# lightec-xyz/bls-verify-gadget

Measured on NVIDIA B200. Metric: bls12_381_verifies_per_sec, higher is better.
Workload: dtype u32 limbs (381-bit modular integer)

## Files before the change

bls_verify_gadget_b200/csrc/blsgpu.cu:

```cuda
#include <cuda_runtime.h>
#include <cstdio>
#include <cstring>
#include <cstdarg>
#include <new>
#include <vector>
#include "stages.cuh"
#include "coop.cuh"
#include "../../include/blsgpu.h"

using namespace bls;

#ifndef BLS_TPB
#define BLS_TPB 128
#endif
#define TPB BLS_TPB
#define VERIFY_CHUNK_DEFAULT ((size_t)1 << 20)
#ifndef VERIFY_COOP_BELOW
#define VERIFY_COOP_BELOW 4096
#endif
#ifndef BLS_MINB
#define BLS_MINB 2
#endif
static inline unsigned nblk(size_t n, unsigned tpb = TPB) { return (unsigned)((n + tpb - 1) / tpb); }

#ifndef BLS_MINB_DG1
#define BLS_MINB_DG1 4
#endif
#ifndef BLS_MINB_DG2
#define BLS_MINB_DG2 4
#endif
#ifndef BLS_MINB_HASH
#define BLS_MINB_HASH BLS_MINB
#endif
#ifndef BLS_MINB_SQR
#define BLS_MINB_SQR 3
#endif
#ifndef BLS_MINB_HFIELD
#define BLS_MINB_HFIELD 4
#endif
#ifndef BLS_MINB_HMAP
#define BLS_MINB_HMAP 3
#endif
#ifndef BLS_MINB_LINES
#define BLS_MINB_LINES BLS_MINB
#endif
#ifndef BLS_MINB_HCLEAR
#define BLS_MINB_HCLEAR BLS_MINB
#endif
#ifndef BLS_MINB_ACCUM
#define BLS_MINB_ACCUM BLS_MINB
#endif
#ifndef MILLER_LINE_ITERS
#define MILLER_LINE_ITERS 8
#define MILLER_LINE_STEPS 11
#endif

#ifndef BLS_F_IN_SMEM
#define BLS_F_IN_SMEM 0
#endif
#ifndef BLS_SKEW
#define BLS_SKEW 0
#endif
__device__ __forceinline__ void phase_skew() {
#if BLS_SKEW > 0
    if ((threadIdx.x >> 5) & 4) { long long t0 = clock64(); while (clock64() - t0 < BLS_SKEW) { } }
#endif
}
__global__ void __launch_bounds__(TPB, BLS_MINB) k_fp_mul_raw(const fp* a, const fp* b, fp* out, size_t n, int reps) {
    size_t i = blockIdx.x * (size_t)blockDim.x + threadIdx.x; if (i >= n) return;
    fp x = a[i], y = b[i];
    fp r = fp_mul(x, y);
    for (int k = 1; k < reps; k++) r = fp_mul(r, y);
    out[i] = r;
}
__global__ void __launch_bounds__(256) k_imad_peak(uint32_t* sink, int iters, int mode) {
    uint32_t a = threadIdx.x * 2654435761u + 12345u, b = blockIdx.x * 40503u + 977u;
    if (mode == 0) {
        unsigned long long acc[16];
#pragma unroll
        for (int j = 0; j < 16; j++) acc[j] = (unsigned long long)j * 0x9e3779b97f4a7c15ull + a;
        for (int it = 0; it < iters; it++) {
#pragma unroll
            for (int j = 0; j < 16; j++)
                asm volatile("mad.wide.u32 %0, %1, %2, %0;" : "+l"(acc[j]) : "r"((uint32_t)acc[(j + 5) & 15]), "r"(b));
        }
        unsigned long long s = 0;
#pragma unroll
        for (int j = 0; j < 16; j++) s ^= acc[j];
        if (s == 0x1234567ull) sink[0] = (uint32_t)s;
    } else {
        uint32_t e[16], o[16];
#pragma unroll
        for (int j = 0; j < 16; j++) { e[j] = a + j; o[j] = b + j; }
        for (int it = 0; it < iters; it++) {
            asm volatile(
                "mad.lo.cc.u32 %0, %16, %24, %0;\n\tmadc.hi.cc.u32 %1, %16, %24, %1;\n\tmadc.lo.cc.u32 %2, %17, %24, %2;\n\tmadc.hi.cc.u32 %3, %17, %24, %3;\n\t"
                "madc.lo.cc.u32 %4, %18, %24, %4;\n\tmadc.hi.cc.u32 %5, %18, %24, %5;\n\tmadc.lo.cc.u32 %6, %19, %24, %6;\n\tmadc.hi.cc.u32 %7, %19, %24, %7;\n\t"
                "madc.lo.cc.u32 %8, %20, %24, %8;\n\tmadc.hi.cc.u32 %9, %20, %24, %9;\n\tmadc.lo.cc.u32 %10, %21, %24, %10;\n\tmadc.hi.cc.u32 %11, %21, %24, %11;\n\t"
                "madc.lo.cc.u32 %12, %22, %24, %12;\n\tmadc.hi.cc.u32 %13, %22, %24, %13;\n\tmadc.lo.cc.u32 %14, %23, %24, %14;\n\tmadc.hi.u32 %15, %23, %24, %15;"
                : "+r"(e[0]), "+r"(e[1]), "+r"(e[2]), "+r"(e[3]), "+r"(e[4]), "+r"(e[5]), "+r"(e[6]), "+r"(e[7]), "+r"(e[8]), "+r"(e[9]), "+r"(e[10]), "+r"(e[11]), "+r"(e[12]), "+r"(e[13]), "+r"(e[14]), "+r"(e[15])
                : "r"(a), "r"(a + 1), "r"(a + 2), "r"(a + 3), "r"(a + 4), "r"(a + 5), "r"(a + 6), "r"(a + 7), "r"(o[3]));
            asm volatile(
                "mad.lo.cc.u32 %0, %16, %24, %0;\n\tmadc.hi.cc.u32 %1, %16, %24, %1;\n\tmadc.lo.cc.u32 %2, %17, %24, %2;\n\tmadc.hi.cc.u32 %3, %17, %24, %3;\n\t"
                "madc.lo.cc.u32 %4, %18, %24, %4;\n\tmadc.hi.cc.u32 %5, %18, %24, %5;\n\tmadc.lo.cc.u32 %6, %19, %24, %6;\n\tmadc.hi.cc.u32 %7, %19, %24, %7;\n\t"
                "madc.lo.cc.u32 %8, %20, %24, %8;\n\tmadc.hi.cc.u32 %9, %20, %24, %9;\n\tmadc.lo.cc.u32 %10, %21, %24, %10;\n\tmadc.hi.cc.u32 %11, %21, %24, %11;\n\t"
                "madc.lo.cc.u32 %12, %22, %24, %12;\n\tmadc.hi.cc.u32 %13, %22, %24, %13;\n\tmadc.lo.cc.u32 %14, %23, %24, %14;\n\tmadc.hi.u32 %15, %23, %24, %15;"
                : "+r"(o[0]), "+r"(o[1]), "+r"(o[2]), "+r"(o[3]), "+r"(o[4]), "+r"(o[5]), "+r"(o[6]), "+r"(o[7]), "+r"(o[8]), "+r"(o[9]), "+r"(o[10]), "+r"(o[11]), "+r"(o[12]), "+r"(o[13]), "+r"(o[14]), "+r"(o[15])
                : "r"(b), "r"(b + 1), "r"(b + 2), "r"(b + 3), "r"(b + 4), "r"(b + 5), "r"(b + 6), "r"(b + 7), "r"(e[5]));
        }
        uint32_t s = 0;
#pragma unroll
        for (int j = 0; j < 16; j++) s ^= e[j] ^ o[j];
        if (s == 0x12345u) sink[0] = s;
    }
}

__global__ void __launch_bounds__(TPB, BLS_MINB_DG1) k_decode_g1(const uint8_t* in48, size_t n, u32x4* soa, uint8_t* code) {
    phase_skew();
    size_t i = blockIdx.x * (size_t)blockDim.x + threadIdx.x; if (i >= n) return;
    g1_aff p; int rc = g1_decode(p, in48 + 48 * i);
    if (soa) soa_store_g1(soa, n, i, p);
    code[i] = (uint8_t)rc;
}
__global__ void __launch_bounds__(TPB, BLS_MINB_DG2) k_decode_g2(const uint8_t* in96, size_t n, u32x4* soa, uint8_t* code) {
    phase_skew();
    size_t i = blockIdx.x * (size_t)blockDim.x + threadIdx.x; if (i >= n) return;
    g2_aff p; int rc = g2_decode(p, in96 + 96 * i);
    if (soa) soa_store_g2(soa, n, i, p);
    code[i] = (uint8_t)rc;
}
__global__ void __launch_bounds__(TPB, BLS_MINB_HASH) k_hash_to_g2(const uint8_t* msg, const uint32_t* off, size_t n, const uint8_t* code_pk, const uint8_t* code_sig,
                                                    u32x4* hm_soa, uint8_t* flags, uint8_t* status) {
    phase_skew();
    size_t i = blockIdx.x * (size_t)blockDim.x + threadIdx.x; if (i >= n) return;
    uint8_t st = ST_OK, fl = 0;
    if (code_pk) {
        if (code_pk[i] != DEC_OK) st = ST_BAD_PK;
        else if (code_sig[i] != DEC_OK && code_sig[i] != DEC_INF) st = ST_BAD_SIG;
        else if (code_sig[i] == DEC_INF) fl = FL_SIG_INF;
    }
    if (st == ST_OK) {
        const uint8_t* m; uint32_t len;
        if (off) { m = msg + off[i]; len = off[i + 1] - off[i]; } else { m = msg + 32 * i; len = 32; }
        g2_aff hm; uint8_t f2; stage_hash(hm, f2, m, len);
        soa_store_g2(hm_soa, n, i, hm); fl |= f2;
    }
    flags[i] = fl; if (status) status[i] = st;
}
__global__ void __launch_bounds__(TPB, BLS_MINB_HFIELD) k_hash_field(const uint8_t* msg, const uint32_t* off, size_t n, const uint8_t* code_pk, const uint8_t* code_sig,
                                                               u32x4* u_soa, uint8_t* flags, uint8_t* status) {
    size_t i = blockIdx.x * (size_t)blockDim.x + threadIdx.x; if (i >= n) return;
    uint8_t st = ST_OK, fl = 0;
    if (code_pk) {
        if (code_pk[i] != DEC_OK) st = ST_BAD_PK;
        else if (code_sig[i] != DEC_OK && code_sig[i] != DEC_INF) st = ST_BAD_SIG;
        else if (code_sig[i] == DEC_INF) fl = FL_SIG_INF;
    }
    if (st == ST_OK) {
        const uint8_t* m; uint32_t len;
        if (off) { m = msg + off[i]; len = off[i + 1] - off[i]; } else { m = msg + 32 * i; len = 32; }
        fp2 u0, u1; hash_to_field(u0, u1, m, len);
        soa_store_fp2(u_soa, n, i, 0, u0); soa_store_fp2(u_soa, n, i, 1, u1);
    }
    flags[i] = fl; if (status) status[i] = st;
}
__global__ void k_status_merge(const uint8_t* code_pk, const uint8_t* code_sig, size_t n, uint8_t* flags, uint8_t* status) {
    size_t i = blockIdx.x * (size_t)blockDim.x + threadIdx.x; if (i >= n) return;
    uint8_t st = ST_OK, fl = 0;
    if (code_pk[i] != DEC_OK) st = ST_BAD_PK;
    else if (code_sig[i] != DEC_OK && code_sig[i] != DEC_INF) st = ST_BAD_SIG;
    else if (code_sig[i] == DEC_INF) fl = FL_SIG_INF;
    flags[i] = (uint8_t)((flags[i] & FL_HM_INF) | fl); status[i] = st;
}
__global__ void __launch_bounds__(TPB, BLS_MINB_HMAP) k_hash_map(const u32x4* u_soa, const uint8_t* status, size_t n, u32x4* q_soa) {
    size_t t = blockIdx.x * (size_t)blockDim.x + threadIdx.x; if (t >= 2 * n) return;
    int j = t >= n; size_t i = t - (j ? n : 0);
    if (status && status[i] != ST_OK) return;
    fp2 u = soa_load_fp2(u_soa, n, i, j), xn, xd, y; g2_jac q;
    sswu_map(xn, xd, y, u); iso3_map(q, xn, xd, y);
    soa_store_fp2(q_soa, n, i, 3 * j, q.X); soa_store_fp2(q_soa, n, i, 3 * j + 1, q.Y); soa_store_fp2(q_soa, n, i, 3 * j + 2, q.Z);
}
__global__ void __launch_bounds__(TPB, BLS_MINB_HCLEAR) k_hash_clear(const u32x4* q_soa, const uint8_t* status, size_t n, u32x4* hm_soa, uint8_t* flags) {
    size_t i = blockIdx.x * (size_t)blockDim.x + threadIdx.x; if (i >= n) return;
    if (status && status[i] != ST_OK) return;
    g2_jac q0, q1, h; g2_aff hm;
    q0.X = soa_load_fp2(q_soa, n, i, 0); q0.Y = soa_load_fp2(q_soa, n, i, 1); q0.Z = soa_load_fp2(q_soa, n, i, 2);
    q1.X = soa_load_fp2(q_soa, n, i, 3); q1.Y = soa_load_fp2(q_soa, n, i, 4); q1.Z = soa_load_fp2(q_soa, n, i, 5);
    jac_add(q0, q0, q1); g2_clear_cofactor(h, q0);
    if (!jac_to_aff(hm, h)) flags[i] |= FL_HM_INF;
    soa_store_g2(hm_soa, n, i, hm);
}
__global__ void __launch_bounds__(TPB, BLS_MINB) k_miller(const u32x4* pk_soa, const u32x4* hm_soa, const u32x4* sig_soa, const uint8_t* flags,
                                                const uint8_t* status, size_t n, u32x4* f_soa) {
    phase_skew();
    size_t i = blockIdx.x * (size_t)blockDim.x + threadIdx.x; if (i >= n) return;
    if (status[i] != ST_OK) return;
    g1_aff pk; g2_aff hm, sig;
    soa_load_g1(pk, pk_soa, n, i); soa_load_g2(hm, hm_soa, n, i); soa_load_g2(sig, sig_soa, n, i);
#if BLS_F_IN_SMEM
    extern __shared__ uint4 f_smem[];
    fp12& f = *reinterpret_cast<fp12*>(f_smem + threadIdx.x * 37);
#else
    fp12 f;
#endif
    stage_miller(f, pk, hm, sig, flags[i]);
    soa_store_fp12(f_soa, n, i, f);
}
__global__ void __launch_bounds__(TPB, BLS_MINB_LINES) k_miller_lines(const u32x4* pk_soa, const u32x4* hm_soa, const u32x4* sig_soa, const uint8_t* flags, const uint8_t* status,
                                                                size_t n, u32x4* t_soa, u32x4* lines, int i_hi, int i_lo) {
    size_t t = blockIdx.x * (size_t)blockDim.x + threadIdx.x; if (t >= 2 * n) return;
    int j = t >= n; size_t i = t - (j ? n : 0);
    if (status[i] != ST_OK) return;
    if (flags[i] & (j ? FL_HM_INF : FL_SIG_INF)) return;
    g1_aff p; g2_aff q; g2_proj r;
    if (j) { soa_load_g1(p, pk_soa, n, i); soa_load_g2(q, hm_soa, n, i); } else { p.x = fp_const(C_G1X); p.y = fp_const(C_G1Y_NEG); soa_load_g2(q, sig_soa, n, i); }
    if (i_hi == 62) { r.x = q.x; r.y = q.y; r.z = fp2_one(); }
    else { r.x = soa_load_fp2(t_soa, n, i, 3 * j); r.y = soa_load_fp2(t_soa, n, i, 3 * j + 1); r.z = soa_load_fp2(t_soa, n, i, 3 * j + 2); }
    const uint64_t x = BLS_X_ABS; int s = 0; fp2 c0, c1, c2;
    for (int it = i_hi; it >= i_lo; it--) {
        miller_dbl(r, c0, c1, c2);
        { u32x4* L = lines + (size_t)(2 * s + j) * 18 * n; soa_store_fp2(L, n, i, 0, c0); soa_store_fp2(L, n, i, 1, fp2_mul_fp(c1, p.x)); soa_store_fp2(L, n, i, 2, fp2_mul_fp(c2, p.y)); s++; }
        if ((x >> it) & 1) {
            miller_add(r, q, c0, c1, c2);
            u32x4* L = lines + (size_t)(2 * s + j) * 18 * n; soa_store_fp2(L, n, i, 0, c0); soa_store_fp2(L, n, i, 1, fp2_mul_fp(c1, p.x)); soa_store_fp2(L, n, i, 2, fp2_mul_fp(c2, p.y)); s++;
        }
    }
    if (i_lo != 0) { soa_store_fp2(t_soa, n, i, 3 * j, r.x); soa_store_fp2(t_soa, n, i, 3 * j + 1, r.y); soa_store_fp2(t_soa, n, i, 3 * j + 2, r.z); }
}
__global__ void __launch_bounds__(TPB, BLS_MINB_ACCUM) k_miller_accum(const uint8_t* flags, const uint8_t* status, size_t n, u32x4* f_soa, const u32x4* lines, int i_hi, int i_lo) {
    size_t i = blockIdx.x * (size_t)blockDim.x + threadIdx.x; if (i >= n) return;
    if (status[i] != ST_OK) return;
    uint8_t fl = flags[i]; bool use0 = !(fl & FL_SIG_INF), use1 = !(fl & FL_HM_INF);
    fp12 f; if (i_hi == 62) fp12_one(f); else soa_load_fp12(f, f_soa, n, i);
    const uint64_t x = BLS_X_ABS; int s = 0;
    for (int it = i_hi; it >= i_lo; it--) {
        if (it != 62) fp12_sqr(f, f);
        int steps = 1 + (int)((x >> it) & 1);
        for (int a = 0; a < steps; a++, s++) {
            if (use0) { const u32x4* L = lines + (size_t)(2 * s) * 18 * n; fp12_mul_by_014(f, soa_load_fp2(L, n, i, 0), soa_load_fp2(L, n, i, 1), soa_load_fp2(L, n, i, 2)); }
            if (use1) { const u32x4* L = lines + (size_t)(2 * s + 1) * 18 * n; fp12_mul_by_014(f, soa_load_fp2(L, n, i, 0), soa_load_fp2(L, n, i, 1), soa_load_fp2(L, n, i, 2)); }
        }
    }
    if (i_lo == 0) fp12_conj(f, f);
    soa_store_fp12(f_soa, n, i, f);
}
__global__ void __launch_bounds__(TPB, BLS_MINB_SQR) k_final_squarings(const u32x4* in_soa, u32x4* snap_soa, const uint8_t* status, size_t n) {
    size_t i = blockIdx.x * (size_t)blockDim.x + threadIdx.x; if (i >= n) return;
    if (status[i] != ST_OK) return;
    fp12c c;
    c.g2 = soa_load_fp2(in_soa, n, i, 3); c.g3 = soa_load_fp2(in_soa, n, i, 2); c.g4 = soa_load_fp2(in_soa, n, i, 1); c.g5 = soa_load_fp2(in_soa, n, i, 5);
    const uint64_t x = BLS_X_ABS; int k = 0;
    for (int j = 1; j <= 63; j++) {
        fp12c_sqr(c, c);
        if ((x >> j) & 1) {
            soa_store_fp2(snap_soa, n, i, 4 * k, c.g2); soa_store_fp2(snap_soa, n, i, 4 * k + 1, c.g3); soa_store_fp2(snap_soa, n, i, 4 * k + 2, c.g4); soa_store_fp2(snap_soa, n, i, 4 * k + 3, c.g5);
            k++;
        }
    }
}
template <int STEP> __global__ void __launch_bounds__(TPB, BLS_MINB) k_final_step(u32x4* f_soa, u32x4* y1_soa, u32x4* y2_soa, const u32x4* snap_soa, const uint8_t* status_in, uint8_t* status_out, size_t n) {
    size_t i = blockIdx.x * (size_t)blockDim.x + threadIdx.x; if (i >= n) return;
    if (status_in[i] != ST_OK) { if (STEP == 5) status_out[i] = status_in[i]; return; }
    fp12 r, y1, y2, e;
    if (STEP >= 1) {
        fp12_decompress_product_from(e, [&](int k) { fp12c c; c.g2 = soa_load_fp2(snap_soa, n, i, 4 * k); c.g3 = soa_load_fp2(snap_soa, n, i, 4 * k + 1);
                                                     c.g4 = soa_load_fp2(snap_soa, n, i, 4 * k + 2); c.g5 = soa_load_fp2(snap_soa, n, i, 4 * k + 3); return c; }, 6);
        fp12_conj(e, e);
    }
    if (STEP == 0 || STEP == 1 || STEP == 3 || STEP == 5) soa_load_fp12(r, f_soa, n, i);
    if (STEP == 2 || STEP == 3 || STEP == 5) soa_load_fp12(y1, y1_soa, n, i);
    final_exponentiation_step<STEP>(r, y1, y2, e);
    if (STEP == 0 || STEP == 3 || STEP == 5) soa_store_fp12(f_soa, n, i, r);
    if (STEP >= 1 && STEP <= 3) soa_store_fp12(y1_soa, n, i, y1);
    if (STEP == 4) soa_store_fp12(y2_soa, n, i, y2);
    if (STEP == 5) status_out[i] = fp12_is_one(r) ? ST_OK : ST_FALSE;
}
__global__ void __launch_bounds__(TPB, BLS_MINB) k_miller_pairs(const u32x4* g1_soa, const u32x4* g2_soa, const uint8_t* c1, const uint8_t* c2, size_t npairs, size_t nprod,
                                                      u32x4* f_soa, uint8_t* status) {
    size_t i = blockIdx.x * (size_t)blockDim.x + threadIdx.x; if (i >= nprod) return;
    size_t tot = npairs * nprod;
    g1_aff p[2]; g2_aff q[2]; bool use[2] = {false, false}; uint8_t st = ST_OK;
    for (size_t k = 0; k < npairs; k++) {
        size_t j = i * npairs + k;
        soa_load_g1(p[k], g1_soa, tot, j); soa_load_g2(q[k], g2_soa, tot, j);
        if (c1[j] > DEC_INF) st = ST_BAD_PK; else if (c2[j] > DEC_INF && st == ST_OK) st = ST_BAD_SIG;
        use[k] = c1[j] == DEC_OK && c2[j] == DEC_OK;
    }
    if (npairs < 2) { p[1] = p[0]; q[1] = q[0]; }
    status[i] = st;
    if (st != ST_OK) return;
    fp12 f; miller_loop2(f, p[0], q[0], use[0], p[1], q[1], use[1]);
    soa_store_fp12(f_soa, nprod, i, f);
}
__global__ void __launch_bounds__(TPB, BLS_MINB) k_final_exp(u32x4* f_soa, const uint8_t* status_in, uint8_t* status_out, size_t n) {
    phase_skew();
    size_t i = blockIdx.x * (size_t)blockDim.x + threadIdx.x; if (i >= n) return;
    if (status_in[i] != ST_OK) { status_out[i] = status_in[i]; return; }
    fp12 f, gt; soa_load_fp12(f, f_soa, n, i);
    status_out[i] = stage_final(gt, f);
    soa_store_fp12(f_soa, n, i, gt);
}
__global__ void __launch_bounds__(TPB, BLS_MINB) k_final_easy(u32x4* f_soa, const uint8_t* status, size_t n) {
    size_t i = blockIdx.x * (size_t)blockDim.x + threadIdx.x; if (i >= n) return;
    if (status[i] != ST_OK) return;
    fp12 f, t, r; soa_load_fp12(f, f_soa, n, i);
    fp12_conj(t, f); fp12_inv(r, f); fp12_mul(r, t, r);
    fp12_frob2(t, r); fp12_mul(r, t, r);
    soa_store_fp12(f_soa, n, i, r);
}
__global__ void __launch_bounds__(128, 2) k_final_hard_coop(u32x4* f_soa, const uint8_t* status_in, uint8_t* status_out, size_t n) {
    __shared__ coop_smem sm[4];
    int warp = threadIdx.x >> 5, lane = threadIdx.x & 31, g = lane / 6;
    coop_lane c = coop_init(&sm[warp]);
    size_t item = (blockIdx.x * (size_t)4 + warp) * 5 + g;
    bool in_range = g < 5 && item < n;
    uint8_t st = in_range ? status_in[item] : (uint8_t)ST_BAD_PK;
    bool active = in_range && st == ST_OK;
    fp2 r = c.k == 0 ? fp2_one() : fp2_zero();
    if (active) r = soa_load_fp2(f_soa, n, item, COOP_TOWER_POS[c.k]);
    r = coop_final_exp_hard(c, r);
    bool mine = c.k == 0 ? fp2_eq(r, fp2_one()) : fp2_is_zero(r);
    unsigned ball = __ballot_sync(0xffffffffu, mine);
    if (active) soa_store_fp2(f_soa, n, item, COOP_TOWER_POS[c.k], r);
    if (in_range && c.k == 0) status_out[item] = active ? ((((ball >> (6 * g)) & 63u) == 63u) ? (uint8_t)ST_OK : (uint8_t)ST_FALSE) : st;
}
__global__ void __launch_bounds__(128, 2) k_miller_accum_coop(const uint8_t* flags, const uint8_t* status, size_t n, u32x4* f_soa, const u32x4* lines, int i_hi, int i_lo) {
    __shared__ coop_smem sm[4];
    int warp = threadIdx.x >> 5, lane = threadIdx.x & 31, g = lane / 6;
    coop_lane c = coop_init(&sm[warp]);
    size_t item = (blockIdx.x * (size_t)4 + warp) * 5 + g;
    bool active = g < 5 && item < n && status[item] == ST_OK;
    uint8_t fl = active ? flags[item] : (uint8_t)(FL_SIG_INF | FL_HM_INF);
    bool use[2] = {!(fl & FL_SIG_INF), !(fl & FL_HM_INF)};
    fp2 unit = c.k == 0 ? fp2_one() : fp2_zero();
    fp2 f = (active && i_hi != 62) ? soa_load_fp2(f_soa, n, item, COOP_TOWER_POS[c.k]) : unit;
    int slot = c.k == 0 ? 0 : c.k == 2 ? 1 : c.k == 3 ? 2 : -1;
    const uint64_t x = BLS_X_ABS; int s = 0;
    for (int it = i_hi; it >= i_lo; it--) {
        if (it != 62) f = coop_mul(c, f, f);
        int steps = 1 + (int)((x >> it) & 1);
        for (int a = 0; a < steps; a++, s++)
            for (int j = 0; j < 2; j++) {
                const u32x4* L = lines + (size_t)(2 * s + j) * 18 * n;
                fp2 b = !use[j] ? unit : slot >= 0 ? soa_load_fp2(L, n, item, slot) : fp2_zero();
                f = coop_mul(c, f, b);
            }
    }
    if (i_lo == 0) f = coop_conj(c, f);
    if (active) soa_store_fp2(f_soa, n, item, COOP_TOWER_POS[c.k], f);
}
__global__ void __launch_bounds__(TPB, BLS_MINB) k_gt_reduce(const u32x4* in_soa, const uint8_t* status, size_t n, u32x4* out_soa, size_t T) {
    size_t t = blockIdx.x * (size_t)blockDim.x + threadIdx.x; if (t >= T) return;
    fp12 acc, x; fp12_one(acc);
    for (size_t i = t; i < n; i += T) {
        if (status && status[i] > ST_FALSE) continue;
        soa_load_fp12(x, in_soa, n, i); fp12_mul(acc, acc, x);
    }
    soa_store_fp12(out_soa, T, t, acc);
}
__global__ void k_gt_mul_into(u32x4* acc_soa, const u32x4* x_soa) {
    if (threadIdx.x || blockIdx.x) return;
    fp12 a, x; soa_load_fp12(a, acc_soa, 1, 0); soa_load_fp12(x, x_soa, 1, 0); fp12_mul(a, a, x); soa_store_fp12(acc_soa, 1, 0, a);
}
__global__ void k_gt_set_one(u32x4* acc_soa) { if (threadIdx.x || blockIdx.x) return; fp12 a; fp12_one(a); soa_store_fp12(acc_soa, 1, 0, a); }
__global__ void __launch_bounds__(TPB, BLS_MINB) k_gt_to_bytes(const u32x4* soa, size_t n, uint8_t* out576, const uint8_t* status) {
    size_t i = blockIdx.x * (size_t)blockDim.x + threadIdx.x; if (i >= n) return;
    if (status && status[i] != ST_OK) { for (int k = 0; k < 576; k++) out576[576 * i + k] = 0; return; }
    fp12 a; soa_load_fp12(a, soa, n, i); fp12_to_bytes(out576 + 576 * i, a);
}
__global__ void __launch_bounds__(TPB, BLS_MINB) k_gt_from_bytes(const uint8_t* in576, size_t n, u32x4* soa) {
    size_t i = blockIdx.x * (size_t)blockDim.x + threadIdx.x; if (i >= n) return;
    fp12 a; fp2* c[6] = {&a.c0.c0, &a.c0.c1, &a.c0.c2, &a.c1.c0, &a.c1.c1, &a.c1.c2};
    const uint8_t* b = in576 + 576 * i;
    for (int k = 0; k < 12; k++) {
        fp v;
        for (int w = 0; w < 12; w++) { const uint8_t* q = b + 48 * k + 4 * w; v.l[w] = q[0] | ((uint32_t)q[1] << 8) | ((uint32_t)q[2] << 16) | ((uint32_t)q[3] << 24); }
        v = fp_to_mont(v);
        if (k & 1) c[k >> 1]->c1 = v; else c[k >> 1]->c0 = v;
    }
    soa_store_fp12(soa, n, i, a);
}
__global__ void k_status_bitmap(const uint8_t* status, size_t n, uint32_t* bitmap32) {
    size_t i = blockIdx.x * (size_t)blockDim.x + threadIdx.x;
    bool ok = i < n && status[i] == ST_OK;
    unsigned m = __ballot_sync(0xffffffffu, ok);
    if ((threadIdx.x & 31) == 0 && i < ((n + 31) / 32) * 32) bitmap32[i >> 5] = m;
}
__global__ void __launch_bounds__(TPB, BLS_MINB) k_encode_g1(const u32x4* soa, const uint8_t* inf, size_t n, uint8_t* out48) {
    size_t i = blockIdx.x * (size_t)blockDim.x + threadIdx.x; if (i >= n) return;
    g1_aff p; soa_load_g1(p, soa, n, i); g1_encode(out48 + 48 * i, p, inf && inf[i]);
}
__global__ void __launch_bounds__(TPB, BLS_MINB) k_encode_g2(const u32x4* soa, const uint8_t* flags, uint8_t mask, size_t n, uint8_t* out96) {
    size_t i = blockIdx.x * (size_t)blockDim.x + threadIdx.x; if (i >= n) return;
    g2_aff p; soa_load_g2(p, soa, n, i); g2_encode(out96 + 96 * i, p, flags && (flags[i] & mask));
}
__device__ __forceinline__ bool load_scalar(uint32_t* k, const uint8_t* sk) {
    const uint32_t R[8] = BLS_C_R_ORDER;
    for (int w = 0; w < 8; w++) k[w] = sk[4 * w] | ((uint32_t)sk[4 * w + 1] << 8) | ((uint32_t)sk[4 * w + 2] << 16) | ((uint32_t)sk[4 * w + 3] << 24);
    for (int w = 7; w >= 0; w--) { if (k[w] != R[w]) return k[w] < R[w]; }
    return false;
}
__global__ void __launch_bounds__(TPB, BLS_MINB) k_scalar_mul_g1(const uint8_t* sk32, size_t n, uint8_t* pk48, uint8_t* status) {
    size_t i = blockIdx.x * (size_t)blockDim.x + threadIdx.x; if (i >= n) return;
    uint32_t k[8]; bool canon = load_scalar(k, sk32 + 32 * i);
    if (status) status[i] = canon ? ST_OK : ST_BAD_SK;
    g1_aff g; g.x = fp_const(C_G1X); g.y = fp_const(C_G1Y);
    g1_jac r; jac_mul_scalar(r, g, k);
    g1_aff a; bool ok = jac_to_aff(a, r); g1_encode(pk48 + 48 * i, a, !ok || !canon);
}
__global__ void __launch_bounds__(TPB, BLS_MINB) k_scalar_mul_g2(const uint8_t* sk32, const u32x4* hm_soa, const uint8_t* flags, size_t n, uint8_t* sig96, uint8_t* status) {
    size_t i = blockIdx.x * (size_t)blockDim.x + threadIdx.x; if (i >= n) return;
    uint32_t k[8]; bool canon = load_scalar(k, sk32 + 32 * i);
    uint32_t nz = 0; for (int w = 0; w < 8; w++) nz |= k[w];
    if (!canon || !nz) { status[i] = ST_BAD_SK; for (int b = 0; b < 96; b++) sig96[96 * i + b] = 0; return; }
    status[i] = ST_OK;
    g2_aff hm; soa_load_g2(hm, hm_soa, n, i);
    g2_jac r;
    if (flags[i] & FL_HM_INF) jac_set_identity(r); else jac_mul_scalar(r, hm, k);
    g2_aff a; bool ok = jac_to_aff(a, r); g2_encode(sig96 + 96 * i, a, !ok);
}

template <class F> struct segsum_traits;
template <> struct segsum_traits<fp>  { enum { K = 2 }; static __device__ __forceinline__ void load(aff<fp>& p, const u32x4* s, size_t n, size_t i) { soa_load_g1(p, s, n, i); }
                                        static __device__ __forceinline__ void store(u32x4* s, size_t n, size_t i, const aff<fp>& p) { soa_store_g1(s, n, i, p); }
                                        static __device__ __forceinline__ void storej(u32x4* s, size_t n, size_t i, const jac<fp>& p) { soa_store_fp(s, n, i, 0, p.X); soa_store_fp(s, n, i, 1, p.Y); soa_store_fp(s, n, i, 2, p.Z); }
                                        static __device__ __forceinline__ void loadj(jac<fp>& p, const u32x4* s, size_t n, size_t i) { p.X = soa_load_fp(s, n, i, 0); p.Y = soa_load_fp(s, n, i, 1); p.Z = soa_load_fp(s, n, i, 2); } };
template <> struct segsum_traits<fp2> { enum { K = 4 }; static __device__ __forceinline__ void load(aff<fp2>& p, const u32x4* s, size_t n, size_t i) { soa_load_g2(p, s, n, i); }
                                        static __device__ __forceinline__ void store(u32x4* s, size_t n, size_t i, const aff<fp2>& p) { soa_store_g2(s, n, i, p); }
                                        static __device__ __forceinline__ void storej(u32x4* s, size_t n, size_t i, const jac<fp2>& p) { soa_store_fp2(s, n, i, 0, p.X); soa_store_fp2(s, n, i, 1, p.Y); soa_store_fp2(s, n, i, 2, p.Z); }
                                        static __device__ __forceinline__ void loadj(jac<fp2>& p, const u32x4* s, size_t n, size_t i) { p.X = soa_load_fp2(s, n, i, 0); p.Y = soa_load_fp2(s, n, i, 1); p.Z = soa_load_fp2(s, n, i, 2); } };
#define SEG_WARPS 4
template <class F> __global__ void __launch_bounds__(32 * SEG_WARPS) k_segsum(const u32x4* pts_soa, const uint8_t* code, size_t npts, const uint32_t* seg_off, size_t seg_stride,
                                                                            const uint64_t* bitmap, size_t nseg, u32x4* out_jac, uint8_t* status, uint8_t bad_code,
                                                                            const uint32_t* idx , int L) {
    __shared__ jac<F> sm[SEG_WARPS][32];
    int warp = threadIdx.x >> 5, lane = threadIdx.x & 31, sub = lane / L, sl = lane % L, per_warp = 32 / L;
    size_t s = (blockIdx.x * (size_t)SEG_WARPS + warp) * per_warp + sub;
    bool active = s < nseg;
    size_t lo = 0, hi = 0;
    if (active) { if (seg_off) { lo = seg_off[s]; hi = seg_off[s + 1]; } else { lo = s * seg_stride; hi = lo + seg_stride; } }
    jac<F> acc; jac_set_identity(acc);
    unsigned bad = 0, cnt = 0;
    for (size_t i = lo + sl; i < hi; i += L) {
        if (bitmap && !((bitmap[i >> 6] >> (i & 63)) & 1)) continue;
        cnt++;
        size_t pi = idx ? (size_t)idx[i] : i;
        if (pi >= npts) { bad = 1; continue; }
        uint8_t c = code[pi];
        if (c > DEC_INF) { bad = 1; continue; }
        if (c == DEC_INF) continue;
        aff<F> p; segsum_traits<F>::load(p, pts_soa, npts, pi);
        jac_add_mixed(acc, acc, p);
    }
    sm[warp][lane] = acc;
    __syncwarp();
    for (int w = L >> 1; w >= 1; w >>= 1) {
        if (sl < w) { jac<F> o = sm[warp][lane + w]; jac_add(acc, acc, o); sm[warp][lane] = acc; }
        __syncwarp();
        bad |= __shfl_down_sync(0xffffffffu, bad, w); cnt += __shfl_down_sync(0xffffffffu, cnt, w);
    }
    if (active && sl == 0) {
        segsum_traits<F>::storej(out_jac, nseg, s, acc);
        status[s] = bad ? bad_code : (cnt == 0 ? ST_EMPTY : ST_OK);
    }
}
template <class F> __global__ void __launch_bounds__(TPB, BLS_MINB) k_jac_to_aff(const u32x4* jac_soa, size_t n, u32x4* aff_soa, uint8_t* inf) {
    size_t i = blockIdx.x * (size_t)blockDim.x + threadIdx.x; if (i >= n) return;
    jac<F> p; segsum_traits<F>::loadj(p, jac_soa, n, i);
    aff<F> a; bool ok = jac_to_aff(a, p);
    segsum_traits<F>::store(aff_soa, n, i, a); inf[i] = ok ? 0 : 1;
}
static int seg_lanes(size_t avg_len) { int L = 32; while (L > 1 && avg_len / L < 64) L >>= 1; return L; }
__global__ void k_fav_status(const uint8_t* agg_status, const uint8_t* agg_inf, const uint8_t* code_sig, size_t n, uint8_t* code_pk_out) {
    size_t i = blockIdx.x * (size_t)blockDim.x + threadIdx.x; if (i >= n) return;
    code_pk_out[i] = (agg_status[i] != ST_OK || agg_inf[i]) ? DEC_BAD_FLAGS : DEC_OK;
}

__device__ __forceinline__ uint64_t rlc_scalar(const uint8_t* seed16, uint64_t idx) {
    sha256_ctx c; sha256_init(c);
    for (int i = 0; i < 16; i++) sha256_put(c, seed16[i]);
    for (int i = 0; i < 8; i++) sha256_put(c, (uint32_t)(idx >> (8 * i)) & 0xffu);
    uint32_t d[8]; sha256_final(c, d);
    uint64_t r = ((uint64_t)d[0] << 32) | d[1];
    return r ? r : 1;
}
template <class F> __device__ __forceinline__ void jac_mul_u64(jac<F>& r, const aff<F>& p, uint64_t k) {
    jac_set_identity(r);
    for (int i = 63; i >= 0; i--) { jac_dbl(r, r); if ((k >> i) & 1) jac_add_mixed(r, r, p); }
}
__global__ void __launch_bounds__(TPB, BLS_MINB) k_rlc_scale(u32x4* pk_soa, const u32x4* sig_soa, uint8_t* flags, const uint8_t* status, size_t n, size_t idx0,
                                                              const uint8_t* seed16, u32x4* rsig_jac) {
    size_t i = blockIdx.x * (size_t)blockDim.x + threadIdx.x; if (i >= n) return;
    g2_jac rs; jac_set_identity(rs);
    if (status[i] == ST_OK) {
        uint64_t r = rlc_scalar(seed16, idx0 + i);
        g1_aff pk; soa_load_g1(pk, pk_soa, n, i);
        g1_jac rp; jac_mul_u64(rp, pk, r);
        g1_aff a; jac_to_aff(a, rp); soa_store_g1(pk_soa, n, i, a);
        if (!(flags[i] & FL_SIG_INF)) { g2_aff sg; soa_load_g2(sg, sig_soa, n, i); jac_mul_u64(rs, sg, r); }
        flags[i] |= FL_SIG_INF;
    }
    segsum_traits<fp2>::storej(rsig_jac, n, i, rs);
}
__global__ void __launch_bounds__(TPB, BLS_MINB) k_g2_jac_reduce(const u32x4* in_jac, size_t n, u32x4* out_jac, size_t T) {
    size_t t = blockIdx.x * (size_t)blockDim.x + threadIdx.x; if (t >= T) return;
    g2_jac acc, x; jac_set_identity(acc);
    for (size_t i = t; i < n; i += T) { segsum_traits<fp2>::loadj(x, in_jac, n, i); jac_add(acc, acc, x); }
    segsum_traits<fp2>::storej(out_jac, T, t, acc);
}
__global__ void k_g2_jac_add_into(u32x4* acc_jac, const u32x4* x_jac) {
    if (threadIdx.x || blockIdx.x) return;
    g2_jac a, x; segsum_traits<fp2>::loadj(a, acc_jac, 1, 0); segsum_traits<fp2>::loadj(x, x_jac, 1, 0); jac_add(a, a, x); segsum_traits<fp2>::storej(acc_jac, 1, 0, a);
}
__global__ void k_g2_jac_set_identity(u32x4* acc_jac) { if (threadIdx.x || blockIdx.x) return; g2_jac a; jac_set_identity(a); segsum_traits<fp2>::storej(acc_jac, 1, 0, a); }
__global__ void k_any_bad(const uint8_t* status, size_t n, uint32_t* bad) {
    size_t i = blockIdx.x * (size_t)blockDim.x + threadIdx.x;
    bool b = i < n && status[i] != ST_OK;
    if (__any_sync(0xffffffffu, b) && (threadIdx.x & 31) == 0) atomicOr(bad, 1u);
}
__global__ void __launch_bounds__(32, 1) k_rlc_finish(const u32x4* f_acc, const u32x4* s_jac, const uint32_t* bad, uint8_t* all_ok) {
    if (threadIdx.x || blockIdx.x) return;
    fp12 F, f2, gt; soa_load_fp12(F, f_acc, 1, 0);
    g2_jac S; segsum_traits<fp2>::loadj(S, s_jac, 1, 0);
    g2_aff sa; bool have = jac_to_aff(sa, S);
    g1_aff ng; ng.x = fp_const(C_G1X); ng.y = fp_const(C_G1Y_NEG);
    miller_loop2(f2, ng, sa, have, ng, sa, false);
    fp12_mul(F, F, f2);
    final_exponentiation(gt, F);
    all_ok[0] = (fp12_is_one(gt) && !bad[0]) ? 1 : 0;
}

__global__ void __launch_bounds__(TPB, BLS_MINB) k_gt_reduce_seg(const u32x4* in_soa, const uint8_t* status, size_t n, size_t L, u32x4* out_soa, size_t T, size_t P) {
    size_t t = blockIdx.x * (size_t)blockDim.x + threadIdx.x, p = blockIdx.y; if (t >= T) return;
    size_t lo = p * L, hi = lo + L < n ? lo + L : n;
    fp12 acc, x; fp12_one(acc);
    for (size_t i = lo + t; i < hi; i += T) {
        if (status && status[i] > ST_FALSE) continue;
        soa_load_fp12(x, in_soa, n, i); fp12_mul(acc, acc, x);
    }
    soa_store_fp12(out_soa, P * T, p * T + t, acc);
}
__global__ void __launch_bounds__(TPB, BLS_MINB) k_g2_jac_reduce_seg(const u32x4* in_jac, size_t n, size_t L, u32x4* out_jac, size_t T, size_t P) {
    size_t t = blockIdx.x * (size_t)blockDim.x + threadIdx.x, p = blockIdx.y; if (t >= T) return;
    size_t lo = p * L, hi = lo + L < n ? lo + L : n;
    g2_jac acc, x; jac_set_identity(acc);
    for (size_t i = lo + t; i < hi; i += T) { segsum_traits<fp2>::loadj(x, in_jac, n, i); jac_add(acc, acc, x); }
    segsum_traits<fp2>::storej(out_jac, P * T, p * T + t, acc);
}
__global__ void __launch_bounds__(32, 1) k_rlc_finish_seg(const u32x4* f_piece, const u32x4* s_piece, size_t P, uint8_t* ok) {
    size_t p = blockIdx.x; if (threadIdx.x || p >= P) return;
    fp12 F, f2, gt; soa_load_fp12(F, f_piece, P, p);
    g2_jac S; segsum_traits<fp2>::loadj(S, s_piece, P, p);
    g2_aff sa; bool have = jac_to_aff(sa, S);
    g1_aff ng; ng.x = fp_const(C_G1X); ng.y = fp_const(C_G1Y_NEG);
    miller_loop2(f2, ng, sa, have, ng, sa, false);
    fp12_mul(F, F, f2);
    final_exponentiation(gt, F);
    ok[p] = fp12_is_one(gt) ? 1 : 0;
}

__global__ void __launch_bounds__(TPB, BLS_MINB) k_g1_recode(const uint8_t* in, size_t n, uint8_t* out, uint8_t* code, int to_uncompressed) {
    size_t i = blockIdx.x * (size_t)blockDim.x + threadIdx.x; if (i >= n) return;
    g1_aff p; int rc = to_uncompressed ? g1_decode(p, in + 48 * i) : g1_decode_uncompressed(p, in + 96 * i);
    uint8_t* o = out + (to_uncompressed ? 96 : 48) * i;
    if (rc > DEC_INF) { for (int k = 0; k < (to_uncompressed ? 96 : 48); k++) o[k] = 0; }
    else if (to_uncompressed) g1_encode_uncompressed(o, p, rc == DEC_INF); else g1_encode(o, p, rc == DEC_INF);
    if (code) code[i] = (uint8_t)rc;
}
__global__ void __launch_bounds__(TPB, BLS_MINB) k_g2_recode(const uint8_t* in, size_t n, uint8_t* out, uint8_t* code, int to_uncompressed) {
    size_t i = blockIdx.x * (size_t)blockDim.x + threadIdx.x; if (i >= n) return;
    g2_aff p; int rc = to_uncompressed ? g2_decode(p, in + 96 * i) : g2_decode_uncompressed(p, in + 192 * i);
    uint8_t* o = out + (to_uncompressed ? 192 : 96) * i;
    if (rc > DEC_INF) { for (int k = 0; k < (to_uncompressed ? 192 : 96); k++) o[k] = 0; }
    else if (to_uncompressed) g2_encode_uncompressed(o, p, rc == DEC_INF); else g2_encode(o, p, rc == DEC_INF);
    if (code) code[i] = (uint8_t)rc;
}
__global__ void k_aggv_sig_status(const uint8_t* code_sig, size_t nsig, uint8_t* st, uint8_t* flags) {
    size_t s = blockIdx.x * (size_t)blockDim.x + threadIdx.x; if (s >= nsig) return;
    st[s] = (code_sig[s] == DEC_OK || code_sig[s] == DEC_INF) ? ST_OK : ST_BAD_SIG;
    flags[s] = FL_HM_INF | (code_sig[s] == DEC_INF ? FL_SIG_INF : 0);
}
__global__ void __launch_bounds__(TPB, BLS_MINB) k_aggv_combine(const u32x4* f_pair, const uint8_t* pair_status, size_t npairs, const uint32_t* pair_off,
                                                                 u32x4* f_sig, const uint8_t* sig_status, size_t nsig, uint8_t* status) {
    size_t s = blockIdx.x * (size_t)blockDim.x + threadIdx.x; if (s >= nsig) return;
    uint32_t lo = pair_off[s], hi = pair_off[s + 1];
    uint8_t st = sig_status[s];
    for (uint32_t j = lo; j < hi; j++) if (pair_status[j] != ST_OK) { st = ST_BAD_PK; break; }
    if (st == ST_OK && lo == hi) st = ST_EMPTY;
    status[s] = st;
    if (st != ST_OK) return;
    fp12 acc, x; soa_load_fp12(acc, f_sig, nsig, s);
    for (uint32_t j = lo; j < hi; j++) { soa_load_fp12(x, f_pair, npairs, j); fp12_mul(acc, acc, x); }
    soa_store_fp12(f_sig, nsig, s, acc);
}

struct blsgpu_ctx {
    int device; cudaStream_t own_stream, stream; int ptr_mode; char err[512];
    uint8_t* ws; size_t ws_bytes, ws_used; unsigned long long launches;
    struct r1cs_sys* r1cs[16]; struct wit_prog* wit[4];
    uint8_t* rlc_acc;
    struct { u32x4* soa; uint8_t* code; size_t n; } pool[16];
    int coop;
    int wit_cluster;
    int lanes; cudaStream_t lane_stream[4]; cudaEvent_t lane_done[4], fork;
    int split;
    size_t chunk;
    int prof; cudaEvent_t ev[8];
};
struct dev_guard { int prev; dev_guard() : prev(-1) { if (cudaGetDevice(&prev) != cudaSuccess) { cudaGetLastError(); prev = -1; } } ~dev_guard() { if (prev >= 0) cudaSetDevice(prev); } };
#define STAGE_MARK(k) do { if (ctx->prof) CU(cudaEventRecord(ctx->ev[k], ctx->stream)); } while (0)
static int fail(blsgpu_ctx* c, int code, const char* fmt, ...) {
    if (c) { va_list ap; va_start(ap, fmt); vsnprintf(c->err, sizeof c->err, fmt, ap); va_end(ap); }
    return code;
}
#define CU(call) do { cudaError_t e_ = (call); if (e_ != cudaSuccess) return fail(ctx, BLSGPU_ERR_CUDA, "%s failed: %s (%s:%d)", #call, cudaGetErrorString(e_), __FILE__, __LINE__); } while (0)
#define LAUNCH(kern, grid, block, ...) do { kern<<<(grid), (block), 0, ctx->stream>>>(__VA_ARGS__); ctx->launches++; CU(cudaGetLastError()); } while (0)

static int ws_reserve(blsgpu_ctx* ctx, size_t bytes) {
    if (bytes <= ctx->ws_bytes) { ctx->ws_used = 0; return 0; }
    CU(cudaStreamSynchronize(ctx->stream));
    if (ctx->ws) { cudaFree(ctx->ws); ctx->ws = nullptr; ctx->ws_bytes = 0; }
    size_t want = bytes + (bytes >> 3);
    if (cudaMalloc(&ctx->ws, want) != cudaSuccess) { cudaGetLastError(); return fail(ctx, BLSGPU_ERR_ALLOC, "cudaMalloc of %zu workspace bytes failed", want); }
    ctx->ws_bytes = want; ctx->ws_used = 0; return 0;
}
template <class T> static T* ws_take(blsgpu_ctx* ctx, size_t count) {
    size_t off = (ctx->ws_used + 255) & ~(size_t)255; ctx->ws_used = off + count * sizeof(T);
    return reinterpret_cast<T*>(ctx->ws + off);
}
static inline size_t al(size_t b) { return (b + 255) & ~(size_t)255; }
template <class T> static int stage_in(blsgpu_ctx* ctx, const T*& dev, const T* user, size_t count) {
    if (!user) { dev = nullptr; return 0; }
    if (ctx->ptr_mode == BLSGPU_DEVICE) { dev = user; return 0; }
    T* d = ws_take<T>(ctx, count ? count : 1);
    if (count) CU(cudaMemcpyAsync(d, user, count * sizeof(T), cudaMemcpyHostToDevice, ctx->stream));
    dev = d; return 0;
}
template <class T> static T* stage_out(blsgpu_ctx* ctx, T* user, size_t count) {
    if (!user) return nullptr;
    return ctx->ptr_mode == BLSGPU_DEVICE ? user : ws_take<T>(ctx, count ? count : 1);
}
template <class T> static int finish_out(blsgpu_ctx* ctx, T* user, const T* dev, size_t count) {
    if (!user || ctx->ptr_mode == BLSGPU_DEVICE || !count) return 0;
    CU(cudaMemcpyAsync(user, dev, count * sizeof(T), cudaMemcpyDeviceToHost, ctx->stream));
    return 0;
}
static int finish_call(blsgpu_ctx* ctx) {
    if (ctx->ptr_mode == BLSGPU_HOST) CU(cudaStreamSynchronize(ctx->stream));
    return 0;
}
static size_t msg_bytes_total(blsgpu_ctx* ctx, const uint32_t* off, size_t n, int& rc) {
    rc = 0;
    if (!off) return 32 * n;
    if (ctx->ptr_mode == BLSGPU_HOST) return off[n];
    uint32_t last = 0;
    if (cudaMemcpyAsync(&last, off + n, 4, cudaMemcpyDeviceToHost, ctx->stream) != cudaSuccess || cudaStreamSynchronize(ctx->stream) != cudaSuccess) rc = BLSGPU_ERR_CUDA;
    return last;
}

static int gt_product(blsgpu_ctx* ctx, const u32x4* in_soa, const uint8_t* status, size_t n, u32x4* tmp_a, u32x4* tmp_b, u32x4* dst) {
    const u32x4* cur = in_soa; size_t cnt = n; const uint8_t* st = status; u32x4* bufs[2] = {tmp_a, tmp_b}; int which = 0;
    while (true) {
        size_t T = (cnt + 7) / 8;
        u32x4* out = T == 1 ? dst : bufs[which];
        LAUNCH(k_gt_reduce, nblk(T), TPB, cur, st, cnt, out, T);
        if (T == 1) break;
        cur = out; cnt = T; st = nullptr; which ^= 1;
    }
    return 0;
}

extern "C" {

int blsgpu_create(blsgpu_ctx** out, int device) {
    if (!out) return BLSGPU_ERR_ARG;
    *out = nullptr;
    int ndev = 0;
    if (cudaGetDeviceCount(&ndev) != cudaSuccess || ndev == 0) { cudaGetLastError(); return BLSGPU_ERR_CUDA; }
    if (device < 0) { if (cudaGetDevice(&device) != cudaSuccess) return BLSGPU_ERR_CUDA; }
    if (device >= ndev) return BLSGPU_ERR_ARG;
    dev_guard guard_;
    cudaDeviceProp prop;
    if (cudaGetDeviceProperties(&prop, device) != cudaSuccess) return BLSGPU_ERR_CUDA;
    if (prop.major != 10) return BLSGPU_ERR_CUDA;
    if (cudaSetDevice(device) != cudaSuccess) return BLSGPU_ERR_CUDA;
    blsgpu_ctx* c = new (std::nothrow) blsgpu_ctx(); if (!c) return BLSGPU_ERR_ALLOC;
    memset(c, 0, sizeof *c); c->device = device; c->ptr_mode = BLSGPU_HOST; c->chunk = VERIFY_CHUNK_DEFAULT; c->lanes = 2; c->wit_cluster = 0; c->split = 1; c->coop = 2;
    if (cudaStreamCreateWithFlags(&c->own_stream, cudaStreamNonBlocking) != cudaSuccess) { delete c; return BLSGPU_ERR_CUDA; }
    c->stream = c->own_stream;
    *out = c; return 0;
}
void blsgpu_destroy(blsgpu_ctx* ctx) {
    if (!ctx) return;
    dev_guard guard_; cudaSetDevice(ctx->device);
    cudaStreamSynchronize(ctx->stream);
    for (int i = 0; i < 16; i++) if (ctx->r1cs[i]) blsgpu_r1cs_free(ctx, i);
    for (int i = 0; i < 4; i++) if (ctx->wit[i]) blsgpu_witness_free(ctx, i);
    for (int i = 0; i < 16; i++) if (ctx->pool[i].soa) { cudaFree(ctx->pool[i].soa); cudaFree(ctx->pool[i].code); }
    if (ctx->ws) cudaFree(ctx->ws);
    if (ctx->rlc_acc) cudaFree(ctx->rlc_acc);
    if (ctx->ev[0]) for (int i = 0; i < 8; i++) cudaEventDestroy(ctx->ev[i]);
    if (ctx->lane_stream[0]) { for (int l = 0; l < 4; l++) { cudaStreamDestroy(ctx->lane_stream[l]); cudaEventDestroy(ctx->lane_done[l]); } cudaEventDestroy(ctx->fork); }
    cudaStreamDestroy(ctx->own_stream);
    delete ctx;
}
const char* blsgpu_last_error(blsgpu_ctx* ctx) { return ctx ? ctx->err : "no context (no usable sm_100 CUDA device, or bad device ordinal)"; }
int blsgpu_set_stream(blsgpu_ctx* ctx, void* s, int use_own) { if (!ctx) return BLSGPU_ERR_ARG; ctx->stream = use_own ? ctx->own_stream : (cudaStream_t)s; return 0; }
int blsgpu_set_pointer_mode(blsgpu_ctx* ctx, int mode) { if (!ctx || (mode != BLSGPU_HOST && mode != BLSGPU_DEVICE)) return BLSGPU_ERR_ARG; ctx->ptr_mode = mode; return 0; }
int blsgpu_synchronize(blsgpu_ctx* ctx) { if (!ctx) return BLSGPU_ERR_ARG; dev_guard guard_; CU(cudaSetDevice(ctx->device)); CU(cudaStreamSynchronize(ctx->stream)); return 0; }
uint64_t blsgpu_launch_count(blsgpu_ctx* ctx) { return ctx ? ctx->launches : 0; }
int blsgpu_set_coop(blsgpu_ctx* ctx, int on) { if (!ctx || on < 0 || on > 2) return BLSGPU_ERR_ARG; ctx->coop = on; return 0; }
int blsgpu_set_witness_mode(blsgpu_ctx* ctx, int cluster) { if (!ctx) return BLSGPU_ERR_ARG; ctx->wit_cluster = cluster ? 1 : 0; return 0; }
int blsgpu_set_split(blsgpu_ctx* ctx, int on) { if (!ctx) return BLSGPU_ERR_ARG; ctx->split = on ? 1 : 0; return 0; }
int blsgpu_set_lanes(blsgpu_ctx* ctx, int lanes) { if (!ctx || lanes < 1 || lanes > 4) return BLSGPU_ERR_ARG; ctx->lanes = lanes; return 0; }
int blsgpu_set_chunk(blsgpu_ctx* ctx, size_t items) { if (!ctx || items < 64 || (items & 63)) return BLSGPU_ERR_ARG; ctx->chunk = items; return 0; }
int blsgpu_set_profiling(blsgpu_ctx* ctx, int on) {
    if (!ctx) return BLSGPU_ERR_ARG;
    dev_guard guard_; CU(cudaSetDevice(ctx->device));
    if (on && !ctx->ev[0]) for (int i = 0; i < 8; i++) CU(cudaEventCreate(&ctx->ev[i]));
    ctx->prof = on ? 1 : 0; return 0;
}
int blsgpu_stage_times(blsgpu_ctx* ctx, float* ms6) {
    if (!ctx || !ms6 || !ctx->ev[0]) return BLSGPU_ERR_ARG;
    dev_guard guard_; CU(cudaSetDevice(ctx->device)); CU(cudaStreamSynchronize(ctx->stream));
    for (int i = 0; i < 6; i++) CU(cudaEventElapsedTime(&ms6[i], ctx->ev[i], ctx->ev[i + 1]));
    return 0;
}

#define ENTER() if (!ctx) return BLSGPU_ERR_ARG; dev_guard guard_; CU(cudaSetDevice(ctx->device))

int blsgpu_fp_mul_raw(blsgpu_ctx* ctx, const uint8_t* a48, const uint8_t* b48, size_t n, uint8_t* out48, int reps) {
    ENTER(); if (!a48 || !b48 || !out48) return fail(ctx, BLSGPU_ERR_ARG, "null pointer");
    if (!n) return 0;
    if (int rc = ws_reserve(ctx, 3 * al(48 * n) + 4096)) return rc;
    const uint8_t *da, *db; if (int rc = stage_in(ctx, da, a48, 48 * n)) return rc; if (int rc = stage_in(ctx, db, b48, 48 * n)) return rc;
    uint8_t* dout = stage_out(ctx, out48, 48 * n);
    LAUNCH(k_fp_mul_raw, nblk(n), TPB, (const fp*)da, (const fp*)db, (fp*)dout, n, reps < 1 ? 1 : reps);
    if (int rc = finish_out(ctx, out48, dout, 48 * n)) return rc;
    return finish_call(ctx);
}
int blsgpu_imad_peak(blsgpu_ctx* ctx, int mode, double* mac32_per_sec, double* ms_out) {
    ENTER(); if (!mac32_per_sec) return fail(ctx, BLSGPU_ERR_ARG, "null pointer");
    if (int rc = ws_reserve(ctx, 4096)) return rc;
    uint32_t* sink = ws_take<uint32_t>(ctx, 16);
    int sms = 0; CU(cudaDeviceGetAttribute(&sms, cudaDevAttrMultiProcessorCount, ctx->device));
    const int iters = 8192, blocks = sms * 8, threads = 256;
    cudaEvent_t e0, e1; CU(cudaEventCreate(&e0)); CU(cudaEventCreate(&e1));
    double best = 1e30;
    if (mode == 2) {
        size_t n = (size_t)sms * 128 * 8; const int reps = 2000;
        if (int rc = ws_reserve(ctx, 3 * al(48 * n) + 4096)) return rc;
        fp* a = ws_take<fp>(ctx, n); fp* b = ws_take<fp>(ctx, n); fp* o = ws_take<fp>(ctx, n);
        CU(cudaMemsetAsync(a, 0x5a, 48 * n, ctx->stream)); CU(cudaMemsetAsync(b, 0x13, 48 * n, ctx->stream));
        for (int rep = 0; rep < 4; rep++) {
            CU(cudaEventRecord(e0, ctx->stream));
            LAUNCH(k_fp_mul_raw, nblk(n), TPB, (const fp*)a, (const fp*)b, o, n, reps);
            CU(cudaEventRecord(e1, ctx->stream)); CU(cudaEventSynchronize(e1));
            float ms = 0; CU(cudaEventElapsedTime(&ms, e0, e1));
            if (rep && ms < best) best = ms;
        }
        cudaEventDestroy(e0); cudaEventDestroy(e1);
        *mac32_per_sec = (double)n * reps * 300.0 / (best * 1e-3); if (ms_out) *ms_out = best;
        return 0;
    }
    for (int rep = 0; rep < 6; rep++) {
        CU(cudaEventRecord(e0, ctx->stream));
        LAUNCH(k_imad_peak, blocks, threads, sink, iters, mode);
        CU(cudaEventRecord(e1, ctx->stream)); CU(cudaEventSynchronize(e1));
        float ms = 0; CU(cudaEventElapsedTime(&ms, e0, e1));
        if (rep && ms < best) best = ms;
    }
    cudaEventDestroy(e0); cudaEventDestroy(e1);
    double macs = (double)blocks * threads * (double)iters * 16.0;
    *mac32_per_sec = macs / (best * 1e-3); if (ms_out) *ms_out = best;
    return 0;
}

int blsgpu_deserialize_g1(blsgpu_ctx* ctx, const uint8_t* in48, size_t n, uint8_t* status) {
    ENTER(); if (!in48 || !status) return fail(ctx, BLSGPU_ERR_ARG, "null pointer");
    if (!n) return 0;
    if (int rc = ws_reserve(ctx, al(48 * n) + al(n) + 4096)) return rc;
    const uint8_t* din; if (int rc = stage_in(ctx, din, in48, 48 * n)) return rc;
    uint8_t* dst = stage_out(ctx, status, n);
    LAUNCH(k_decode_g1, nblk(n), TPB, din, n, (u32x4*)nullptr, dst);
    if (int rc = finish_out(ctx, status, dst, n)) return rc;
    return finish_call(ctx);
}
int blsgpu_deserialize_g2(blsgpu_ctx* ctx, const uint8_t* in96, size_t n, uint8_t* status) {
    ENTER(); if (!in96 || !status) return fail(ctx, BLSGPU_ERR_ARG, "null pointer");
    if (!n) return 0;
    if (int rc = ws_reserve(ctx, al(96 * n) + al(n) + 4096)) return rc;
    const uint8_t* din; if (int rc = stage_in(ctx, din, in96, 96 * n)) return rc;
    uint8_t* dst = stage_out(ctx, status, n);
    LAUNCH(k_decode_g2, nblk(n), TPB, din, n, (u32x4*)nullptr, dst);
    if (int rc = finish_out(ctx, status, dst, n)) return rc;
    return finish_call(ctx);
}

static int hash_stage(blsgpu_ctx* ctx, const uint8_t* dmsg, const uint32_t* doff, size_t n, const uint8_t* code_pk, const uint8_t* code_sig, u32x4* hm_soa, u32x4* scratch36,
                      uint8_t* flags, uint8_t* dstatus);
int blsgpu_hash_to_g2_batch(blsgpu_ctx* ctx, const uint8_t* msg, const uint32_t* msg_off, size_t n, uint8_t* out96) {
    ENTER(); if (!msg || !out96) return fail(ctx, BLSGPU_ERR_ARG, "null pointer");
    if (!n) return 0;
    int rc; size_t mb = msg_bytes_total(ctx, msg_off, n, rc); if (rc) return fail(ctx, rc, "reading msg_off failed");
    if ((rc = ws_reserve(ctx, al(mb + 1) + al(4 * (n + 1)) + al(192 * n) + al(96 * n) + al(n) + (ctx->split ? al(576 * n) : 0) + 8192))) return rc;
    const uint8_t* dmsg; const uint32_t* doff;
    if ((rc = stage_in(ctx, dmsg, msg, mb ? mb : 1))) return rc; if ((rc = stage_in(ctx, doff, msg_off, n + 1))) return rc;
    u32x4* hm = ws_take<u32x4>(ctx, 12 * n); uint8_t* flags = ws_take<uint8_t>(ctx, n);
    uint8_t* dout = stage_out(ctx, out96, 96 * n);
    u32x4* scratch = ctx->split ? ws_take<u32x4>(ctx, 36 * n) : nullptr;
    if ((rc = hash_stage(ctx, dmsg, doff, n, nullptr, nullptr, hm, scratch, flags, nullptr))) return rc;
    LAUNCH(k_encode_g2, nblk(n), TPB, hm, flags, (uint8_t)FL_HM_INF, n, dout);
    if ((rc = finish_out(ctx, out96, dout, 96 * n))) return rc;
    return finish_call(ctx);
}

static int hash_stage(blsgpu_ctx* ctx, const uint8_t* dmsg, const uint32_t* doff, size_t n, const uint8_t* code_pk, const uint8_t* code_sig, u32x4* hm_soa, u32x4* scratch36,
                      uint8_t* flags, uint8_t* dstatus) {
    if (ctx->split) {
        LAUNCH(k_hash_field, nblk(n), TPB, dmsg, doff, n, code_pk, code_sig, hm_soa, flags, dstatus);
        LAUNCH(k_hash_map, nblk(2 * n), TPB, (const u32x4*)hm_soa, (const uint8_t*)dstatus, n, scratch36);
        LAUNCH(k_hash_clear, nblk(n), TPB, (const u32x4*)scratch36, (const uint8_t*)dstatus, n, hm_soa, flags);
    } else LAUNCH(k_hash_to_g2, nblk(n), TPB, dmsg, doff, n, code_pk, code_sig, hm_soa, flags, dstatus);
    return 0;
}
static int miller_stage_split(blsgpu_ctx* ctx, const u32x4* pk_soa, const u32x4* hm_soa, const u32x4* sig_soa, const uint8_t* flags, const uint8_t* dstatus, size_t n,
                              u32x4* f_soa, u32x4* t_soa , u32x4* lines , bool coop = false) {
    for (int hi = 62; hi >= 0; hi -= MILLER_LINE_ITERS) {
        int lo = hi - MILLER_LINE_ITERS + 1 < 0 ? 0 : hi - MILLER_LINE_ITERS + 1;
        LAUNCH(k_miller_lines, nblk(2 * n), TPB, pk_soa, hm_soa, sig_soa, flags, dstatus, n, t_soa, lines, hi, lo);
        if (coop) LAUNCH(k_miller_accum_coop, nblk(n, 20), 128, flags, dstatus, n, f_soa, (const u32x4*)lines, hi, lo);
        else LAUNCH(k_miller_accum, nblk(n), TPB, flags, dstatus, n, f_soa, (const u32x4*)lines, hi, lo);
    }
    return 0;
}
static int verify_core(blsgpu_ctx* ctx, const u32x4* pk_soa, const uint8_t* code_pk, const uint8_t* dmsg, const uint32_t* doff, const uint8_t* dsig, size_t n,
                       uint8_t* dstatus, uint32_t* dbitmap, u32x4* gt_acc , bool forked = false) {
    u32x4* sig_soa = ws_take<u32x4>(ctx, 12 * n); u32x4* hm_soa = ws_take<u32x4>(ctx, 12 * n); u32x4* f_soa = ws_take<u32x4>(ctx, 36 * n);
    uint8_t* code_sig = ws_take<uint8_t>(ctx, n); uint8_t* flags = ws_take<uint8_t>(ctx, n);
    if (forked) {
        cudaStream_t main_stream = ctx->stream; int rc = 0;
        ctx->stream = ctx->lane_stream[0]; cudaStreamWaitEvent(ctx->stream, ctx->fork, 0);
        k_decode_g2<<<nblk(n), TPB, 0, ctx->stream>>>(dsig, n, sig_soa, code_sig); ctx->launches++; cudaEventRecord(ctx->lane_done[0], ctx->stream);
        ctx->stream = ctx->lane_stream[1]; cudaStreamWaitEvent(ctx->stream, ctx->fork, 0);
        rc = hash_stage(ctx, dmsg, doff, n, nullptr, nullptr, hm_soa, f_soa, flags, nullptr); cudaEventRecord(ctx->lane_done[1], ctx->stream);
        ctx->stream = main_stream;
        CU(cudaStreamWaitEvent(main_stream, ctx->lane_done[0], 0)); CU(cudaStreamWaitEvent(main_stream, ctx->lane_done[1], 0));
        if (rc) return rc;
        CU(cudaGetLastError());
        LAUNCH(k_status_merge, nblk(n, 256), 256, code_pk, (const uint8_t*)code_sig, n, flags, dstatus);
    } else {
    STAGE_MARK(1);
    LAUNCH(k_decode_g2, nblk(n), TPB, dsig, n, sig_soa, code_sig);
    STAGE_MARK(2);
    if (int rc = hash_stage(ctx, dmsg, doff, n, code_pk, code_sig, hm_soa, f_soa, flags, dstatus)) return rc;
    }
    STAGE_MARK(3);
    bool coop = ctx->coop == 1 || (ctx->coop == 2 && n <= VERIFY_COOP_BELOW);
    u32x4 *y1_soa = nullptr, *y2_soa = nullptr, *snap_soa = nullptr;
    if (ctx->split) {
        u32x4* t_soa = ws_take<u32x4>(ctx, 36 * n); y1_soa = t_soa; y2_soa = ws_take<u32x4>(ctx, 36 * n);
        u32x4* lines = ws_take<u32x4>(ctx, (size_t)MILLER_LINE_STEPS * 2 * 18 * n);
        if (int rc = miller_stage_split(ctx, pk_soa, hm_soa, sig_soa, flags, dstatus, n, f_soa, t_soa, lines, coop)) return rc;
        snap_soa = lines;
    } else {
#if BLS_F_IN_SMEM
    { static bool attr_set = false; if (!attr_set) { cudaFuncSetAttribute(k_miller, cudaFuncAttributeMaxDynamicSharedMemorySize, TPB * 592); attr_set = true; }
      k_miller<<<nblk(n), TPB, TPB * 592, ctx->stream>>>(pk_soa, (const u32x4*)hm_soa, (const u32x4*)sig_soa, (const uint8_t*)flags, (const uint8_t*)dstatus, n, f_soa); ctx->launches++; CU(cudaGetLastError()); }
#else
    LAUNCH(k_miller, nblk(n), TPB, pk_soa, (const u32x4*)hm_soa, (const u32x4*)sig_soa, (const uint8_t*)flags, (const uint8_t*)dstatus, n, f_soa);
#endif
    }
    STAGE_MARK(4);
    if (coop) {
        LAUNCH(k_final_easy, nblk(n), TPB, f_soa, (const uint8_t*)dstatus, n);
        LAUNCH(k_final_hard_coop, nblk(n, 20), 128, f_soa, (const uint8_t*)dstatus, dstatus, n);
    } else if (ctx->split) {
        const uint8_t* cst = dstatus;
        LAUNCH(k_final_step<0>, nblk(n), TPB, f_soa, y1_soa, y2_soa, (const u32x4*)snap_soa, cst, dstatus, n);
        LAUNCH(k_final_squarings, nblk(n), TPB, (const u32x4*)f_soa, snap_soa, cst, n);
        LAUNCH(k_final_step<1>, nblk(n), TPB, f_soa, y1_soa, y2_soa, (const u32x4*)snap_soa, cst, dstatus, n);
        LAUNCH(k_final_squarings, nblk(n), TPB, (const u32x4*)y1_soa, snap_soa, cst, n);
        LAUNCH(k_final_step<2>, nblk(n), TPB, f_soa, y1_soa, y2_soa, (const u32x4*)snap_soa, cst, dstatus, n);
        LAUNCH(k_final_squarings, nblk(n), TPB, (const u32x4*)y1_soa, snap_soa, cst, n);
        LAUNCH(k_final_step<3>, nblk(n), TPB, f_soa, y1_soa, y2_soa, (const u32x4*)snap_soa, cst, dstatus, n);
        LAUNCH(k_final_squarings, nblk(n), TPB, (const u32x4*)y1_soa, snap_soa, cst, n);
        LAUNCH(k_final_step<4>, nblk(n), TPB, f_soa, y1_soa, y2_soa, (const u32x4*)snap_soa, cst, dstatus, n);
        LAUNCH(k_final_squarings, nblk(n), TPB, (const u32x4*)y2_soa, snap_soa, cst, n);
        LAUNCH(k_final_step<5>, nblk(n), TPB, f_soa, y1_soa, y2_soa, (const u32x4*)snap_soa, cst, dstatus, n);
    } else LAUNCH(k_final_exp, nblk(n), TPB, f_soa, (const uint8_t*)dstatus, dstatus, n);
    STAGE_MARK(5);
    if (dbitmap) LAUNCH(k_status_bitmap, nblk(((n + 31) / 32) * 32, 256), 256, (const uint8_t*)dstatus, n, dbitmap);
    if (gt_acc) {
        u32x4* ta = ws_take<u32x4>(ctx, 36 * ((n + 7) / 8)); u32x4* tb = ws_take<u32x4>(ctx, 36 * ((n + 63) / 64)); u32x4* one = ws_take<u32x4>(ctx, 36);
        if (int rc = gt_product(ctx, f_soa, dstatus, n, ta, tb, one)) return rc;
        LAUNCH(k_gt_mul_into, 1, 32, gt_acc, (const u32x4*)one);
    }
    STAGE_MARK(6);
    return 0;
}
static size_t verify_ws_bytes(size_t n, size_t mb) {
    return 2 * al(576 * n) + al((size_t)MILLER_LINE_STEPS * 2 * 288 * n)  + al(48 * n) + al(96 * n) + al(mb + 1) + al(4 * (n + 1)) + al(n) * 6 + al(96 * n) + 2 * al(192 * n) + al(576 * n) + al(8 * ((n + 63) / 64)) +
           al(576 * ((n + 7) / 8)) + al(576 * ((n + 63) / 64)) + 3 * al(576) + 65536;
}
static int ensure_lanes(blsgpu_ctx* ctx);
static int verify_range(blsgpu_ctx* ctx, const uint8_t* pk48, const uint8_t* msg, const uint32_t* msg_off, const uint8_t* sig96, size_t base, size_t m,
                        uint8_t* status, uint64_t* ok_bitmap, u32x4* gt_acc, size_t mb0, size_t mb) {
    int rc = 0;
    const uint8_t *dpk, *dsig, *dmsg; const uint32_t* doff;
    if ((rc = stage_in(ctx, dpk, pk48 + 48 * base, 48 * m))) return rc;
    if ((rc = stage_in(ctx, dsig, sig96 + 96 * base, 96 * m))) return rc;
    if (ctx->ptr_mode == BLSGPU_HOST) {
        if ((rc = stage_in(ctx, dmsg, msg + mb0, mb ? mb : 1))) return rc;
        dmsg -= msg_off ? mb0 : 0;
    } else dmsg = msg_off ? msg : msg + mb0;
    if ((rc = stage_in(ctx, doff, msg_off ? msg_off + base : nullptr, m + 1))) return rc;
    uint8_t* dstatus = stage_out(ctx, status + base, m);
    uint32_t* dbitmap = (uint32_t*)stage_out(ctx, ok_bitmap ? ok_bitmap + base / 64 : nullptr, (m + 63) / 64);
    u32x4* pk_soa = ws_take<u32x4>(ctx, 6 * m); uint8_t* code_pk = ws_take<uint8_t>(ctx, m);
    if (gt_acc) LAUNCH(k_gt_set_one, 1, 32, gt_acc);
    if (dbitmap) CU(cudaMemsetAsync(dbitmap, 0, 8 * ((m + 63) / 64), ctx->stream));
    STAGE_MARK(0);
    bool forked = ctx->coop == 2 && m <= VERIFY_COOP_BELOW && !ctx->prof && ctx->split && ctx->stream != ctx->lane_stream[0] && ctx->stream != ctx->lane_stream[1];
    if (forked) { if ((rc = ensure_lanes(ctx))) return rc; forked = ctx->stream != ctx->lane_stream[0] && ctx->stream != ctx->lane_stream[1]; }
    if (forked) CU(cudaEventRecord(ctx->fork, ctx->stream));
    LAUNCH(k_decode_g1, nblk(m), TPB, dpk, m, pk_soa, code_pk);
    if ((rc = verify_core(ctx, pk_soa, code_pk, dmsg, doff, dsig, m, dstatus, dbitmap, gt_acc, forked))) return rc;
    if ((rc = finish_out(ctx, status + base, dstatus, m))) return rc;
    if (ok_bitmap && (rc = finish_out(ctx, ok_bitmap + base / 64, (uint64_t*)dbitmap, (m + 63) / 64))) return rc;
    return 0;
}
#define MAX_LANES 4
static int ensure_lanes(blsgpu_ctx* ctx) {
    if (ctx->lane_stream[0]) return 0;
    for (int l = 0; l < MAX_LANES; l++) { CU(cudaStreamCreateWithFlags(&ctx->lane_stream[l], cudaStreamNonBlocking)); CU(cudaEventCreateWithFlags(&ctx->lane_done[l], cudaEventDisableTiming)); }
    CU(cudaEventCreateWithFlags(&ctx->fork, cudaEventDisableTiming));
    return 0;
}

int blsgpu_verify_batch(blsgpu_ctx* ctx, const uint8_t* pk48, const uint8_t* msg, const uint32_t* msg_off, const uint8_t* sig96, size_t n,
                        uint8_t* status, uint64_t* ok_bitmap, uint8_t* gt_acc_le576) {
    ENTER(); if (!pk48 || !msg || !sig96 || !status) return fail(ctx, BLSGPU_ERR_ARG, "null pointer");
    int rc = 0;
    uint8_t gt_host[576];
    const uint32_t* off_host = ctx->ptr_mode == BLSGPU_HOST ? msg_off : nullptr;
    size_t total_mb = 0;
    if (msg_off && !off_host) { total_mb = msg_bytes_total(ctx, msg_off, n, rc); if (rc) return fail(ctx, rc, "reading msg_off failed"); }
    for (size_t base = 0; base < n; base += ctx->chunk) {
        size_t m = n - base < ctx->chunk ? n - base : ctx->chunk;
        int lanes = ctx->lanes; if (lanes > MAX_LANES) lanes = MAX_LANES;
        while (lanes > 1 && m / lanes < 8192) lanes--;
        size_t per = ((m + lanes - 1) / lanes + 63) & ~(size_t)63;
        size_t ws = 65536;
        for (int l = 0; l < lanes; l++) {
            size_t lo = base + l * per, hi = lo + per < base + m ? lo + per : base + m; if (lo >= hi) break;
            size_t mb = msg_off ? (off_host ? off_host[hi] - off_host[lo] : total_mb) : 32 * (hi - lo);
            ws += verify_ws_bytes(hi - lo, ctx->ptr_mode == BLSGPU_HOST ? mb : 0) + 4096;
        }
        if ((rc = ws_reserve(ctx, ws))) return rc;
        u32x4* gt_lane[MAX_LANES] = {nullptr, nullptr, nullptr, nullptr};
        cudaStream_t main_stream = ctx->stream;
        if (lanes > 1) { if ((rc = ensure_lanes(ctx))) return rc; CU(cudaEventRecord(ctx->fork, main_stream)); }
        int used = 0;
        for (int l = 0; l < lanes; l++) {
            size_t lo = base + l * per, hi = lo + per < base + m ? lo + per : base + m; if (lo >= hi) break;
            size_t mb0 = msg_off ? (off_host ? off_host[lo] : 0) : 32 * lo;
            size_t mb = msg_off ? (off_host ? off_host[hi] - off_host[lo] : 0) : 32 * (hi - lo);
            if (gt_acc_le576) gt_lane[l] = ws_take<u32x4>(ctx, 36);
            if (lanes > 1) { ctx->stream = ctx->lane_stream[l]; cudaStreamWaitEvent(ctx->stream, ctx->fork, 0); }
            rc = verify_range(ctx, pk48, msg, msg_off, sig96, lo, hi - lo, status, ok_bitmap, gt_lane[l], mb0, mb);
            if (lanes > 1) { if (!rc) cudaEventRecord(ctx->lane_done[l], ctx->stream); ctx->stream = main_stream; }
            if (rc) return rc;
            used = l + 1;
        }
        if (lanes > 1) for (int l = 0; l < used; l++) CU(cudaStreamWaitEvent(main_stream, ctx->lane_done[l], 0));
        if (gt_acc_le576) {
            for (int l = 1; l < used; l++) LAUNCH(k_gt_mul_into, 1, 32, gt_lane[0], (const u32x4*)gt_lane[l]);
            uint8_t* dgt = ws_take<uint8_t>(ctx, 576);
            LAUNCH(k_gt_to_bytes, 1, TPB, (const u32x4*)gt_lane[0], (size_t)1, dgt, (const uint8_t*)nullptr);
            if (n <= ctx->chunk) {
                CU(cudaMemcpyAsync(gt_acc_le576, dgt, 576, ctx->ptr_mode == BLSGPU_DEVICE ? cudaMemcpyDeviceToDevice : cudaMemcpyDeviceToHost, ctx->stream));
            } else {
                uint8_t part[2][576];
                CU(cudaMemcpyAsync(part[1], dgt, 576, cudaMemcpyDeviceToHost, ctx->stream)); CU(cudaStreamSynchronize(ctx->stream));
                if (base == 0) memcpy(gt_host, part[1], 576);
                else {
                    memcpy(part[0], gt_host, 576);
                    int saved = ctx->ptr_mode; ctx->ptr_mode = BLSGPU_HOST;
                    rc = blsgpu_gt_fold(ctx, &part[0][0], 2, gt_host); ctx->ptr_mode = saved; if (rc) return rc;
                }
                if (base + m >= n) {
                    if (ctx->ptr_mode == BLSGPU_DEVICE) { CU(cudaMemcpyAsync(gt_acc_le576, gt_host, 576, cudaMemcpyHostToDevice, ctx->stream)); CU(cudaStreamSynchronize(ctx->stream)); }
                    else memcpy(gt_acc_le576, gt_host, 576);
                }
            }
        }
        if (ctx->ptr_mode == BLSGPU_HOST || n > ctx->chunk) CU(cudaStreamSynchronize(ctx->stream));
    }
    return 0;
}

int blsgpu_verify_batch_rlc(blsgpu_ctx* ctx, const uint8_t* pk48, const uint8_t* msg, const uint32_t* msg_off, const uint8_t* sig96, size_t n,
                            const uint8_t seed16[16], uint8_t* status, uint8_t* all_ok) {
    ENTER(); if (!pk48 || !msg || !sig96 || !seed16 || !all_ok) return fail(ctx, BLSGPU_ERR_ARG, "null pointer");
    int rc = 0;
    const uint32_t* off_host = ctx->ptr_mode == BLSGPU_HOST ? msg_off : nullptr;
    size_t total_mb = 0;
    if (msg_off && !off_host) { total_mb = msg_bytes_total(ctx, msg_off, n, rc); if (rc) return fail(ctx, rc, "reading msg_off failed"); }
    if (!ctx->rlc_acc) CU(cudaMalloc(&ctx->rlc_acc, 2048));
    u32x4* f_acc = reinterpret_cast<u32x4*>(ctx->rlc_acc); u32x4* s_acc = f_acc + 36; uint32_t* bad = reinterpret_cast<uint32_t*>(ctx->rlc_acc + 1024);
    uint8_t* dseed = ctx->rlc_acc + 1040; uint8_t* dok = ctx->rlc_acc + 1056;
    auto release = [&]() {};
    cudaMemcpyKind in_kind = ctx->ptr_mode == BLSGPU_DEVICE ? cudaMemcpyDeviceToDevice : cudaMemcpyHostToDevice;
    CU(cudaMemcpyAsync(dseed, seed16, 16, in_kind, ctx->stream)); CU(cudaMemsetAsync(bad, 0, 4, ctx->stream));
    LAUNCH(k_gt_set_one, 1, 32, f_acc); LAUNCH(k_g2_jac_set_identity, 1, 32, s_acc);
    for (size_t base = 0; base < n && !rc; base += ctx->chunk) {
        size_t m = n - base < ctx->chunk ? n - base : ctx->chunk;
        size_t mb0 = msg_off ? (off_host ? off_host[base] : 0) : 32 * base;
        size_t mb = msg_off ? (off_host ? off_host[base + m] - off_host[base] : total_mb) : 32 * m;
        if ((rc = ws_reserve(ctx, verify_ws_bytes(m, ctx->ptr_mode == BLSGPU_HOST ? mb : 0) + al(288 * m) + al(288 * ((m + 7) / 8)) + al(288 * ((m + 63) / 64)) + al(288) + 65536))) break;
        const uint8_t *dpk, *dsig, *dmsg; const uint32_t* doff;
        if ((rc = stage_in(ctx, dpk, pk48 + 48 * base, 48 * m))) break;
        if ((rc = stage_in(ctx, dsig, sig96 + 96 * base, 96 * m))) break;
        if (ctx->ptr_mode == BLSGPU_HOST) { if ((rc = stage_in(ctx, dmsg, msg + mb0, mb ? mb : 1))) break; dmsg -= msg_off ? mb0 : 0; }
        else dmsg = msg_off ? msg : msg + mb0;
        if ((rc = stage_in(ctx, doff, msg_off ? msg_off + base : nullptr, m + 1))) break;
        uint8_t* dstatus = status ? stage_out(ctx, status + base, m) : ws_take<uint8_t>(ctx, m);
        u32x4* pk_soa = ws_take<u32x4>(ctx, 6 * m); uint8_t* code_pk = ws_take<uint8_t>(ctx, m);
        u32x4* sig_soa = ws_take<u32x4>(ctx, 12 * m); u32x4* hm_soa = ws_take<u32x4>(ctx, 12 * m); u32x4* f_soa = ws_take<u32x4>(ctx, 36 * m);
        uint8_t* code_sig = ws_take<uint8_t>(ctx, m); uint8_t* flags = ws_take<uint8_t>(ctx, m);
        u32x4* rs = ws_take<u32x4>(ctx, 18 * m); u32x4* ja = ws_take<u32x4>(ctx, 18 * ((m + 7) / 8)); u32x4* jb = ws_take<u32x4>(ctx, 18 * ((m + 63) / 64)); u32x4* jone = ws_take<u32x4>(ctx, 18);
        u32x4* ta = ws_take<u32x4>(ctx, 36 * ((m + 7) / 8)); u32x4* tb = ws_take<u32x4>(ctx, 36 * ((m + 63) / 64)); u32x4* one = ws_take<u32x4>(ctx, 36);
        LAUNCH(k_decode_g1, nblk(m), TPB, dpk, m, pk_soa, code_pk);
        LAUNCH(k_decode_g2, nblk(m), TPB, dsig, m, sig_soa, code_sig);
        if ((rc = hash_stage(ctx, dmsg, doff, m, code_pk, code_sig, hm_soa, f_soa, flags, dstatus))) break;
        LAUNCH(k_any_bad, nblk(((m + 31) / 32) * 32, 256), 256, (const uint8_t*)dstatus, m, bad);
        LAUNCH(k_rlc_scale, nblk(m), TPB, pk_soa, (const u32x4*)sig_soa, flags, (const uint8_t*)dstatus, m, base, (const uint8_t*)dseed, rs);
        {
            const u32x4* cur = rs; size_t cnt = m; u32x4* bufs[2] = {ja, jb}; int which = 0;
            while (true) {
                size_t T = (cnt + 7) / 8; u32x4* out = T == 1 ? jone : bufs[which];
                LAUNCH(k_g2_jac_reduce, nblk(T), TPB, cur, cnt, out, T);
                if (T == 1) break;
                cur = out; cnt = T; which ^= 1;
            }
            LAUNCH(k_g2_jac_add_into, 1, 32, s_acc, (const u32x4*)jone);
        }
        if (ctx->split) {
            u32x4* t_soa = ws_take<u32x4>(ctx, 36 * m); u32x4* lines = ws_take<u32x4>(ctx, (size_t)MILLER_LINE_STEPS * 2 * 18 * m);
            if ((rc = miller_stage_split(ctx, pk_soa, hm_soa, sig_soa, flags, dstatus, m, f_soa, t_soa, lines))) break;
        } else LAUNCH(k_miller, nblk(m), TPB, (const u32x4*)pk_soa, (const u32x4*)hm_soa, (const u32x4*)sig_soa, (const uint8_t*)flags, (const uint8_t*)dstatus, m, f_soa);
        if ((rc = gt_product(ctx, f_soa, dstatus, m, ta, tb, one))) break;
        LAUNCH(k_gt_mul_into, 1, 32, f_acc, (const u32x4*)one);
        if (status && (rc = finish_out(ctx, status + base, dstatus, m))) break;
        if (ctx->ptr_mode == BLSGPU_HOST || n > ctx->chunk) { cudaError_t e = cudaStreamSynchronize(ctx->stream); if (e != cudaSuccess) { rc = fail(ctx, BLSGPU_ERR_CUDA, "sync failed: %s", cudaGetErrorString(e)); break; } }
    }
    if (!rc) {
        k_rlc_finish<<<1, 32, 0, ctx->stream>>>(f_acc, s_acc, bad, dok); ctx->launches++;
        cudaError_t e = cudaMemcpyAsync(all_ok, dok, 1, ctx->ptr_mode == BLSGPU_DEVICE ? cudaMemcpyDeviceToDevice : cudaMemcpyDeviceToHost, ctx->stream);
        if (e == cudaSuccess && ctx->ptr_mode == BLSGPU_HOST) e = cudaStreamSynchronize(ctx->stream);
        if (e != cudaSuccess) rc = fail(ctx, BLSGPU_ERR_CUDA, "rlc finish failed: %s", cudaGetErrorString(e));
    }
    release();
    return rc;
}

#define RLC_PIECE 4096
int blsgpu_verify_batch_rlc_bisect(blsgpu_ctx* ctx, const uint8_t* pk48, const uint8_t* msg, const uint32_t* msg_off, const uint8_t* sig96, size_t n,
                                   const uint8_t seed16[16], uint8_t* status, uint64_t* ok_bitmap, uint64_t* fallback_items) {
    ENTER(); if (!pk48 || !msg || !sig96 || !seed16 || !status) return fail(ctx, BLSGPU_ERR_ARG, "null pointer");
    if (fallback_items) *fallback_items = 0;
    if (!n) return 0;
    int rc = 0; bool host = ctx->ptr_mode == BLSGPU_HOST;
    const uint32_t* off_host = host ? msg_off : nullptr;
    size_t total_mb = 0;
    if (msg_off && !off_host) { total_mb = msg_bytes_total(ctx, msg_off, n, rc); if (rc) return fail(ctx, rc, "reading msg_off failed"); }
    if (!ctx->rlc_acc) CU(cudaMalloc(&ctx->rlc_acc, 2048));
    uint8_t* dseed = ctx->rlc_acc + 1040;
    CU(cudaMemcpyAsync(dseed, seed16, 16, host ? cudaMemcpyHostToDevice : cudaMemcpyDeviceToDevice, ctx->stream));
    const size_t L = RLC_PIECE;
    std::vector<uint8_t> piece_ok((n + L - 1) / L, 1);
    size_t chunk = ctx->chunk >= L ? ctx->chunk / L * L : L;
    for (size_t base = 0; base < n; base += chunk) {
        size_t m = n - base < chunk ? n - base : chunk, P = (m + L - 1) / L, T0 = (L + 7) / 8;
        size_t mb0 = msg_off ? (off_host ? off_host[base] : 0) : 32 * base;
        size_t mb = msg_off ? (off_host ? off_host[base + m] - off_host[base] : total_mb) : 32 * m;
        if ((rc = ws_reserve(ctx, verify_ws_bytes(m, host ? mb : 0) + al(288 * m) + 2 * al(288 * P * T0) + 2 * al(576 * P * T0) + al(P) + 65536))) return rc;
        const uint8_t *dpk, *dsig, *dmsg; const uint32_t* doff;
        if ((rc = stage_in(ctx, dpk, pk48 + 48 * base, 48 * m))) return rc;
        if ((rc = stage_in(ctx, dsig, sig96 + 96 * base, 96 * m))) return rc;
        if (host) { if ((rc = stage_in(ctx, dmsg, msg + mb0, mb ? mb : 1))) return rc; dmsg -= msg_off ? mb0 : 0; }
        else dmsg = msg_off ? msg : msg + mb0;
        if ((rc = stage_in(ctx, doff, msg_off ? msg_off + base : nullptr, m + 1))) return rc;
        uint8_t* dstatus = stage_out(ctx, status + base, m);
        u32x4* pk_soa = ws_take<u32x4>(ctx, 6 * m); uint8_t* code_pk = ws_take<uint8_t>(ctx, m);
        u32x4* sig_soa = ws_take<u32x4>(ctx, 12 * m); u32x4* hm_soa = ws_take<u32x4>(ctx, 12 * m); u32x4* f_soa = ws_take<u32x4>(ctx, 36 * m);
        uint8_t* code_sig = ws_take<uint8_t>(ctx, m); uint8_t* flags = ws_take<uint8_t>(ctx, m);
        u32x4* rs = ws_take<u32x4>(ctx, 18 * m); u32x4* ja = ws_take<u32x4>(ctx, 18 * P * T0); u32x4* jb = ws_take<u32x4>(ctx, 18 * P * T0);
        u32x4* ta = ws_take<u32x4>(ctx, 36 * P * T0); u32x4* tb = ws_take<u32x4>(ctx, 36 * P * T0); uint8_t* dok = ws_take<uint8_t>(ctx, P);
        LAUNCH(k_decode_g1, nblk(m), TPB, dpk, m, pk_soa, code_pk);
        LAUNCH(k_decode_g2, nblk(m), TPB, dsig, m, sig_soa, code_sig);
        if ((rc = hash_stage(ctx, dmsg, doff, m, code_pk, code_sig, hm_soa, f_soa, flags, dstatus))) return rc;
        LAUNCH(k_rlc_scale, nblk(m), TPB, pk_soa, (const u32x4*)sig_soa, flags, (const uint8_t*)dstatus, m, base, (const uint8_t*)dseed, rs);
        const u32x4* s_piece; const u32x4* f_piece;
        {
            const u32x4* cur = rs; size_t cnt_n = m, len = L; u32x4* bufs[2] = {ja, jb}; int which = 0;
            while (true) {
                size_t T = (len + 7) / 8; u32x4* out = bufs[which];
                k_g2_jac_reduce_seg<<<dim3(nblk(T), (unsigned)P), TPB, 0, ctx->stream>>>(cur, cnt_n, len, out, T, P); ctx->launches++; CU(cudaGetLastError());
                cur = out; cnt_n = P * T; len = T; which ^= 1;
                if (T == 1) break;
            }
            s_piece = cur;
        }
        if (ctx->split) {
            u32x4* t_soa = ws_take<u32x4>(ctx, 36 * m); u32x4* lines = ws_take<u32x4>(ctx, (size_t)MILLER_LINE_STEPS * 2 * 18 * m);
            if ((rc = miller_stage_split(ctx, pk_soa, hm_soa, sig_soa, flags, dstatus, m, f_soa, t_soa, lines))) return rc;
        } else LAUNCH(k_miller, nblk(m), TPB, (const u32x4*)pk_soa, (const u32x4*)hm_soa, (const u32x4*)sig_soa, (const uint8_t*)flags, (const uint8_t*)dstatus, m, f_soa);
        {
            const u32x4* cur = f_soa; const uint8_t* st = dstatus; size_t cnt_n = m, len = L; u32x4* bufs[2] = {ta, tb}; int which = 0;
            while (true) {
                size_t T = (len + 7) / 8; u32x4* out = bufs[which];
                k_gt_reduce_seg<<<dim3(nblk(T), (unsigned)P), TPB, 0, ctx->stream>>>(cur, st, cnt_n, len, out, T, P); ctx->launches++; CU(cudaGetLastError());
                cur = out; st = nullptr; cnt_n = P * T; len = T; which ^= 1;
                if (T == 1) break;
            }
            f_piece = cur;
        }
        LAUNCH(k_rlc_finish_seg, (unsigned)P, 32, f_piece, s_piece, P, dok);
        if ((rc = finish_out(ctx, status + base, dstatus, m))) return rc;
        CU(cudaMemcpyAsync(piece_ok.data() + base / L, dok, P, cudaMemcpyDeviceToHost, ctx->stream));
        CU(cudaStreamSynchronize(ctx->stream));
    }
    uint64_t rerun = 0;
    for (size_t p = 0; p < piece_ok.size(); ) {
        if (piece_ok[p]) { p++; continue; }
        size_t q = p; while (q < piece_ok.size() && !piece_ok[q]) q++;
        size_t lo = p * L, hi = q * L < n ? q * L : n;
        const uint8_t* m_ptr; const uint32_t* o_ptr;
        std::vector<uint32_t> rebased;
        if (!msg_off) { m_ptr = msg + 32 * lo; o_ptr = nullptr; }
        else if (host) { rebased.resize(hi - lo + 1); for (size_t i = 0; i <= hi - lo; i++) rebased[i] = msg_off[lo + i] - msg_off[lo]; m_ptr = msg + msg_off[lo]; o_ptr = rebased.data(); }
        else { m_ptr = msg; o_ptr = msg_off + lo; }
        if ((rc = blsgpu_verify_batch(ctx, pk48 + 48 * lo, m_ptr, o_ptr, sig96 + 96 * lo, hi - lo, status + lo, nullptr, nullptr))) return rc;
        if (!host) CU(cudaStreamSynchronize(ctx->stream));
        rerun += hi - lo; p = q;
    }
    if (fallback_items) *fallback_items = rerun;
    if (ok_bitmap) {
        if (host) { size_t words = (n + 63) / 64; for (size_t w = 0; w < words; w++) ok_bitmap[w] = 0; for (size_t i = 0; i < n; i++) if (status[i] == ST_OK) ok_bitmap[i >> 6] |= 1ull << (i & 63); }
        else { CU(cudaMemsetAsync(ok_bitmap, 0, 8 * ((n + 63) / 64), ctx->stream)); LAUNCH(k_status_bitmap, nblk(((n + 31) / 32) * 32, 256), 256, (const uint8_t*)status, n, (uint32_t*)ok_bitmap); }
    }
    return finish_call(ctx);
}

int blsgpu_gt_fold(blsgpu_ctx* ctx, const uint8_t* parts, size_t nparts, uint8_t* out) {
    ENTER(); if (!parts || !out || !nparts) return fail(ctx, BLSGPU_ERR_ARG, "bad argument");
    if (int rc = ws_reserve(ctx, al(576 * nparts) * 2 + al(576 * ((nparts + 7) / 8)) + al(576 * ((nparts + 63) / 64)) + 2 * al(576) + 8192)) return rc;
    const uint8_t* din; if (int rc = stage_in(ctx, din, parts, 576 * nparts)) return rc;
    u32x4* soa = ws_take<u32x4>(ctx, 36 * nparts); u32x4* ta = ws_take<u32x4>(ctx, 36 * ((nparts + 7) / 8)); u32x4* tb = ws_take<u32x4>(ctx, 36 * ((nparts + 63) / 64)); u32x4* one = ws_take<u32x4>(ctx, 36);
    uint8_t* dout = stage_out(ctx, out, 576);
    LAUNCH(k_gt_from_bytes, nblk(nparts), TPB, din, nparts, soa);
    if (int rc = gt_product(ctx, soa, nullptr, nparts, ta, tb, one)) return rc;
    LAUNCH(k_gt_to_bytes, 1, TPB, (const u32x4*)one, (size_t)1, dout, (const uint8_t*)nullptr);
    if (int rc = finish_out(ctx, out, dout, 576)) return rc;
    return finish_call(ctx);
}

int blsgpu_pairing_gt(blsgpu_ctx* ctx, const uint8_t* g1_48, const uint8_t* g2_96, size_t npairs, size_t nprod, uint8_t* gt, uint8_t* status) {
    ENTER(); if (!g1_48 || !g2_96 || !gt || npairs < 1 || npairs > 2) return fail(ctx, BLSGPU_ERR_ARG, "bad argument (npairs must be 1 or 2)");
    if (!nprod) return 0;
    size_t tot = npairs * nprod;
    if (int rc = ws_reserve(ctx, al(48 * tot) + al(96 * tot) + al(96 * tot) + al(192 * tot) + 3 * al(tot) + al(576 * nprod) * 2 + 2 * al(nprod) + 8192)) return rc;
    const uint8_t *d1, *d2; if (int rc = stage_in(ctx, d1, g1_48, 48 * tot)) return rc; if (int rc = stage_in(ctx, d2, g2_96, 96 * tot)) return rc;
    u32x4* s1 = ws_take<u32x4>(ctx, 6 * tot); u32x4* s2 = ws_take<u32x4>(ctx, 12 * tot); uint8_t* c1 = ws_take<uint8_t>(ctx, tot); uint8_t* c2 = ws_take<uint8_t>(ctx, tot);
    u32x4* f = ws_take<u32x4>(ctx, 36 * nprod);
    uint8_t* dst = status && ctx->ptr_mode == BLSGPU_DEVICE ? status : ws_take<uint8_t>(ctx, nprod);
    uint8_t* dgt = stage_out(ctx, gt, 576 * nprod);
    LAUNCH(k_decode_g1, nblk(tot), TPB, d1, tot, s1, c1);
    LAUNCH(k_decode_g2, nblk(tot), TPB, d2, tot, s2, c2);
    LAUNCH(k_miller_pairs, nblk(nprod), TPB, (const u32x4*)s1, (const u32x4*)s2, (const uint8_t*)c1, (const uint8_t*)c2, npairs, nprod, f, dst);
    uint8_t* scratch = ws_take<uint8_t>(ctx, nprod);
    LAUNCH(k_final_exp, nblk(nprod), TPB, f, (const uint8_t*)dst, scratch, nprod);
    LAUNCH(k_gt_to_bytes, nblk(nprod), TPB, (const u32x4*)f, nprod, dgt, (const uint8_t*)dst);
    if (int rc = finish_out(ctx, gt, dgt, 576 * nprod)) return rc;
    if (status) if (int rc = finish_out(ctx, status, dst, nprod)) return rc;
    return finish_call(ctx);
}

int blsgpu_sk_to_pk_batch(blsgpu_ctx* ctx, const uint8_t* sk32, size_t n, uint8_t* pk48, uint8_t* status) {
    ENTER(); if (!sk32 || !pk48) return fail(ctx, BLSGPU_ERR_ARG, "null pointer");
    if (!n) return 0;
    if (int rc = ws_reserve(ctx, al(32 * n) + al(48 * n) + al(n) + 4096)) return rc;
    const uint8_t* dsk; if (int rc = stage_in(ctx, dsk, sk32, 32 * n)) return rc;
    uint8_t* dpk = stage_out(ctx, pk48, 48 * n); uint8_t* dst = stage_out(ctx, status, n);
    LAUNCH(k_scalar_mul_g1, nblk(n), TPB, dsk, n, dpk, dst);
    if (int rc = finish_out(ctx, pk48, dpk, 48 * n)) return rc;
    if (int rc = finish_out(ctx, status, dst, n)) return rc;
    return finish_call(ctx);
}
int blsgpu_sign_batch(blsgpu_ctx* ctx, const uint8_t* sk32, const uint8_t* msg, const uint32_t* msg_off, size_t n, uint8_t* sig96, uint8_t* status) {
    ENTER(); if (!sk32 || !msg || !sig96 || !status) return fail(ctx, BLSGPU_ERR_ARG, "null pointer");
    if (!n) return 0;
    int rc; size_t mb = msg_bytes_total(ctx, msg_off, n, rc); if (rc) return fail(ctx, rc, "reading msg_off failed");
    if ((rc = ws_reserve(ctx, al(32 * n) + al(mb + 1) + al(4 * (n + 1)) + al(192 * n) + al(96 * n) + 2 * al(n) + 8192))) return rc;
    const uint8_t *dsk, *dmsg; const uint32_t* doff;
    if ((rc = stage_in(ctx, dsk, sk32, 32 * n))) return rc; if ((rc = stage_in(ctx, dmsg, msg, mb ? mb : 1))) return rc; if ((rc = stage_in(ctx, doff, msg_off, n + 1))) return rc;
    u32x4* hm = ws_take<u32x4>(ctx, 12 * n); uint8_t* flags = ws_take<uint8_t>(ctx, n);
    uint8_t* dsig = stage_out(ctx, sig96, 96 * n); uint8_t* dst = stage_out(ctx, status, n);
    LAUNCH(k_hash_to_g2, nblk(n), TPB, dmsg, doff, n, (const uint8_t*)nullptr, (const uint8_t*)nullptr, hm, flags, (uint8_t*)nullptr);
    LAUNCH(k_scalar_mul_g2, nblk(n), TPB, dsk, (const u32x4*)hm, (const uint8_t*)flags, n, dsig, dst);
    if ((rc = finish_out(ctx, sig96, dsig, 96 * n))) return rc; if ((rc = finish_out(ctx, status, dst, n))) return rc;
    return finish_call(ctx);
}

static int seg_total(blsgpu_ctx* ctx, const uint32_t* seg_off, size_t nseg, size_t& npts) {
    if (ctx->ptr_mode == BLSGPU_HOST) { npts = seg_off[nseg]; return 0; }
    uint32_t last = 0; CU(cudaMemcpyAsync(&last, seg_off + nseg, 4, cudaMemcpyDeviceToHost, ctx->stream)); CU(cudaStreamSynchronize(ctx->stream)); npts = last; return 0;
}
int blsgpu_g1_aggregate(blsgpu_ctx* ctx, const uint8_t* pts48, const uint32_t* seg_off, size_t nseg, uint8_t* out48, uint8_t* status) {
    ENTER(); if (!seg_off || !out48 || !status) return fail(ctx, BLSGPU_ERR_ARG, "null pointer");
    if (!nseg) return 0;
    size_t npts; if (int rc = seg_total(ctx, seg_off, nseg, npts)) return rc;
    if (npts && !pts48) return fail(ctx, BLSGPU_ERR_ARG, "null pointer");
    if (int rc = ws_reserve(ctx, al(48 * npts + 16) + al(4 * (nseg + 1)) + al(96 * npts + 16) + al(npts + 1) + al(96 * nseg) + al(144 * nseg) + al(48 * nseg) + 3 * al(nseg) + 8192)) return rc;
    const uint8_t* din; const uint32_t* dseg;
    if (int rc = stage_in(ctx, din, pts48, 48 * npts)) return rc; if (int rc = stage_in(ctx, dseg, seg_off, nseg + 1)) return rc;
    u32x4* soa = ws_take<u32x4>(ctx, 6 * npts + 1); uint8_t* code = ws_take<uint8_t>(ctx, npts + 1);
    u32x4* osoa = ws_take<u32x4>(ctx, 6 * nseg); uint8_t* oinf = ws_take<uint8_t>(ctx, nseg);
    uint8_t* dout = stage_out(ctx, out48, 48 * nseg); uint8_t* dst = stage_out(ctx, status, nseg);
    if (npts) LAUNCH(k_decode_g1, nblk(npts), TPB, din, npts, soa, code);
    { int L = seg_lanes(npts / nseg); u32x4* ojac = ws_take<u32x4>(ctx, 9 * nseg);
      LAUNCH(k_segsum<fp>, nblk(nseg, SEG_WARPS * (32 / L)), 32 * SEG_WARPS, (const u32x4*)soa, (const uint8_t*)code, npts, dseg, (size_t)0, (const uint64_t*)nullptr, nseg, ojac, dst, (uint8_t)ST_BAD_PK, (const uint32_t*)nullptr, L);
      LAUNCH(k_jac_to_aff<fp>, nblk(nseg), TPB, (const u32x4*)ojac, nseg, osoa, oinf); }
    LAUNCH(k_encode_g1, nblk(nseg), TPB, (const u32x4*)osoa, (const uint8_t*)oinf, nseg, dout);
    if (int rc = finish_out(ctx, out48, dout, 48 * nseg)) return rc; if (int rc = finish_out(ctx, status, dst, nseg)) return rc;
    return finish_call(ctx);
}
int blsgpu_g2_aggregate(blsgpu_ctx* ctx, const uint8_t* pts96, const uint32_t* seg_off, size_t nseg, uint8_t* out96, uint8_t* status) {
    ENTER(); if (!seg_off || !out96 || !status) return fail(ctx, BLSGPU_ERR_ARG, "null pointer");
    if (!nseg) return 0;
    size_t npts; if (int rc = seg_total(ctx, seg_off, nseg, npts)) return rc;
    if (npts && !pts96) return fail(ctx, BLSGPU_ERR_ARG, "null pointer");
    if (int rc = ws_reserve(ctx, al(96 * npts + 16) + al(4 * (nseg + 1)) + al(192 * npts + 16) + al(npts + 1) + al(192 * nseg) + al(288 * nseg) + al(96 * nseg) + 3 * al(nseg) + 8192)) return rc;
    const uint8_t* din; const uint32_t* dseg;
    if (int rc = stage_in(ctx, din, pts96, 96 * npts)) return rc; if (int rc = stage_in(ctx, dseg, seg_off, nseg + 1)) return rc;
    u32x4* soa = ws_take<u32x4>(ctx, 12 * npts + 1); uint8_t* code = ws_take<uint8_t>(ctx, npts + 1);
    u32x4* osoa = ws_take<u32x4>(ctx, 12 * nseg); uint8_t* oinf = ws_take<uint8_t>(ctx, nseg);
    uint8_t* dout = stage_out(ctx, out96, 96 * nseg); uint8_t* dst = stage_out(ctx, status, nseg);
    if (npts) LAUNCH(k_decode_g2, nblk(npts), TPB, din, npts, soa, code);
    { int L = seg_lanes(npts / nseg); u32x4* ojac = ws_take<u32x4>(ctx, 18 * nseg);
      LAUNCH(k_segsum<fp2>, nblk(nseg, SEG_WARPS * (32 / L)), 32 * SEG_WARPS, (const u32x4*)soa, (const uint8_t*)code, npts, dseg, (size_t)0, (const uint64_t*)nullptr, nseg, ojac, dst, (uint8_t)ST_BAD_SIG, (const uint32_t*)nullptr, L);
      LAUNCH(k_jac_to_aff<fp2>, nblk(nseg), TPB, (const u32x4*)ojac, nseg, osoa, oinf); }
    LAUNCH(k_encode_g2, nblk(nseg), TPB, (const u32x4*)osoa, (const uint8_t*)oinf, (uint8_t)1, nseg, dout);
    if (int rc = finish_out(ctx, out96, dout, 96 * nseg)) return rc; if (int rc = finish_out(ctx, status, dst, nseg)) return rc;
    return finish_call(ctx);
}

int blsgpu_fast_aggregate_verify_batch(blsgpu_ctx* ctx, const uint8_t* pks48, const uint64_t* bitmap, size_t k, const uint8_t* msg32, const uint8_t* sig96, size_t ncomm,
                                       uint8_t* status, uint8_t* agg_pk48_out) {
    ENTER(); if (!msg32 || !sig96 || !status || (k && !pks48)) return fail(ctx, BLSGPU_ERR_ARG, "null pointer");
    if (!ncomm) return 0;
    int rc; size_t npts = ncomm * k;
    size_t need = al(48 * npts + 16) + al(8 * ((npts + 63) / 64 + 1)) + al(96 * npts + 16) + al(npts + 1) + al(96 * ncomm) * 2 + al(144 * ncomm) + al(48 * ncomm) + 4 * al(ncomm) + verify_ws_bytes(ncomm, 32 * ncomm);
    if ((rc = ws_reserve(ctx, need))) return rc;
    const uint8_t *dpks, *dmsg, *dsig; const uint64_t* dbm;
    if ((rc = stage_in(ctx, dpks, pks48, 48 * npts))) return rc; if ((rc = stage_in(ctx, dbm, bitmap, (npts + 63) / 64))) return rc;
    if ((rc = stage_in(ctx, dmsg, msg32, 32 * ncomm))) return rc; if ((rc = stage_in(ctx, dsig, sig96, 96 * ncomm))) return rc;
    u32x4* soa = ws_take<u32x4>(ctx, 6 * npts + 1); uint8_t* code = ws_take<uint8_t>(ctx, npts + 1);
    u32x4* agg_soa = ws_take<u32x4>(ctx, 6 * ncomm); uint8_t* agg_inf = ws_take<uint8_t>(ctx, ncomm); uint8_t* agg_st = ws_take<uint8_t>(ctx, ncomm); uint8_t* code_pk = ws_take<uint8_t>(ctx, ncomm);
    uint8_t* dstatus = stage_out(ctx, status, ncomm); uint8_t* dagg = stage_out(ctx, agg_pk48_out, 48 * ncomm);
    if (npts) LAUNCH(k_decode_g1, nblk(npts), TPB, dpks, npts, soa, code);
    { int L = seg_lanes(k); u32x4* ojac = ws_take<u32x4>(ctx, 9 * ncomm);
      LAUNCH(k_segsum<fp>, nblk(ncomm, SEG_WARPS * (32 / L)), 32 * SEG_WARPS, (const u32x4*)soa, (const uint8_t*)code, npts, (const uint32_t*)nullptr, k, dbm, ncomm, ojac, agg_st, (uint8_t)ST_BAD_PK, (const uint32_t*)nullptr, L);
      LAUNCH(k_jac_to_aff<fp>, nblk(ncomm), TPB, (const u32x4*)ojac, ncomm, agg_soa, agg_inf); }
    if (dagg) LAUNCH(k_encode_g1, nblk(ncomm), TPB, (const u32x4*)agg_soa, (const uint8_t*)agg_inf, ncomm, dagg);
    LAUNCH(k_fav_status, nblk(ncomm), TPB, (const uint8_t*)agg_st, (const uint8_t*)agg_inf, (const uint8_t*)nullptr, ncomm, code_pk);
    if ((rc = verify_core(ctx, agg_soa, code_pk, dmsg, nullptr, dsig, ncomm, dstatus, nullptr, nullptr))) return rc;
    if ((rc = finish_out(ctx, status, dstatus, ncomm))) return rc; if ((rc = finish_out(ctx, agg_pk48_out, dagg, 48 * ncomm))) return rc;
    return finish_call(ctx);
}

int blsgpu_aggregate_verify_batch(blsgpu_ctx* ctx, const uint8_t* pks48, const uint8_t* msg, const uint32_t* msg_off, const uint32_t* pair_off,
                                  const uint8_t* sig96, size_t nsig, uint8_t* status) {
    ENTER(); if (!pair_off || !sig96 || !status) return fail(ctx, BLSGPU_ERR_ARG, "null pointer");
    if (!nsig) return 0;
    int rc; size_t npairs; if ((rc = seg_total(ctx, pair_off, nsig, npairs))) return rc;
    if (npairs && (!pks48 || !msg)) return fail(ctx, BLSGPU_ERR_ARG, "null pointer");
    size_t mb = msg_bytes_total(ctx, msg_off, npairs, rc); if (rc) return fail(ctx, rc, "reading msg_off failed");
    size_t np1 = npairs ? npairs : 1;
    if ((rc = ws_reserve(ctx, al(48 * np1) + al(mb + 1) + al(4 * (np1 + 1)) + al(4 * (nsig + 1)) + al(96 * nsig) + al(96 * np1) + 2 * al(192 * np1) + al(576 * np1) + 5 * al(np1) +
                              al(96 * nsig) + 2 * al(192 * nsig) + al(576 * nsig) + 4 * al(nsig) + 65536))) return rc;
    const uint8_t *dpk, *dmsg, *dsig; const uint32_t *doff, *dpair;
    if ((rc = stage_in(ctx, dpk, pks48, 48 * npairs))) return rc; if ((rc = stage_in(ctx, dmsg, msg, mb ? mb : 1))) return rc;
    if ((rc = stage_in(ctx, doff, msg_off, npairs + 1))) return rc; if ((rc = stage_in(ctx, dpair, pair_off, nsig + 1))) return rc;
    if ((rc = stage_in(ctx, dsig, sig96, 96 * nsig))) return rc;
    u32x4* pk_soa = ws_take<u32x4>(ctx, 6 * np1); u32x4* hm_soa = ws_take<u32x4>(ctx, 12 * np1); u32x4* zero_g2 = ws_take<u32x4>(ctx, 12 * np1); u32x4* f_pair = ws_take<u32x4>(ctx, 36 * np1);
    uint8_t* code_pk = ws_take<uint8_t>(ctx, np1); uint8_t* code_inf = ws_take<uint8_t>(ctx, np1); uint8_t* pflags = ws_take<uint8_t>(ctx, np1); uint8_t* pstatus = ws_take<uint8_t>(ctx, np1);
    u32x4* sig_soa = ws_take<u32x4>(ctx, 12 * nsig); u32x4* zero_g1 = ws_take<u32x4>(ctx, 6 * nsig); u32x4* zero_hm = ws_take<u32x4>(ctx, 12 * nsig); u32x4* f_sig = ws_take<u32x4>(ctx, 36 * nsig);
    uint8_t* code_sig = ws_take<uint8_t>(ctx, nsig); uint8_t* sflags = ws_take<uint8_t>(ctx, nsig); uint8_t* sstatus = ws_take<uint8_t>(ctx, nsig);
    uint8_t* dstatus = stage_out(ctx, status, nsig);
    if (npairs) {
        LAUNCH(k_decode_g1, nblk(npairs), TPB, dpk, npairs, pk_soa, code_pk);
        CU(cudaMemsetAsync(code_inf, DEC_INF, npairs, ctx->stream));
        CU(cudaMemsetAsync(zero_g2, 0, 192 * npairs, ctx->stream));
        LAUNCH(k_hash_to_g2, nblk(npairs), TPB, dmsg, doff, npairs, (const uint8_t*)code_pk, (const uint8_t*)code_inf, hm_soa, pflags, pstatus);
        LAUNCH(k_miller, nblk(npairs), TPB, (const u32x4*)pk_soa, (const u32x4*)hm_soa, (const u32x4*)zero_g2, (const uint8_t*)pflags, (const uint8_t*)pstatus, npairs, f_pair);
    }
    LAUNCH(k_decode_g2, nblk(nsig), TPB, dsig, nsig, sig_soa, code_sig);
    LAUNCH(k_aggv_sig_status, nblk(nsig), TPB, (const uint8_t*)code_sig, nsig, sstatus, sflags);
    CU(cudaMemsetAsync(zero_g1, 0, 96 * nsig, ctx->stream)); CU(cudaMemsetAsync(zero_hm, 0, 192 * nsig, ctx->stream));
    LAUNCH(k_miller, nblk(nsig), TPB, (const u32x4*)zero_g1, (const u32x4*)zero_hm, (const u32x4*)sig_soa, (const uint8_t*)sflags, (const uint8_t*)sstatus, nsig, f_sig);
    LAUNCH(k_aggv_combine, nblk(nsig), TPB, (const u32x4*)f_pair, (const uint8_t*)pstatus, npairs, dpair, f_sig, (const uint8_t*)sstatus, nsig, dstatus);
    LAUNCH(k_final_exp, nblk(nsig), TPB, f_sig, (const uint8_t*)dstatus, dstatus, nsig);
    if ((rc = finish_out(ctx, status, dstatus, nsig))) return rc;
    return finish_call(ctx);
}

static int recode(blsgpu_ctx* ctx, const uint8_t* in, size_t n, uint8_t* out, uint8_t* status, size_t in_sz, size_t out_sz, bool g2, int to_unc) {
    if (!in || !out) return fail(ctx, BLSGPU_ERR_ARG, "null pointer");
    if (!n) return 0;
    if (int rc = ws_reserve(ctx, al(in_sz * n) + al(out_sz * n) + al(n) + 8192)) return rc;
    const uint8_t* din; if (int rc = stage_in(ctx, din, in, in_sz * n)) return rc;
    uint8_t* dout = stage_out(ctx, out, out_sz * n); uint8_t* dst = stage_out(ctx, status, n);
    if (g2) LAUNCH(k_g2_recode, nblk(n), TPB, din, n, dout, dst, to_unc); else LAUNCH(k_g1_recode, nblk(n), TPB, din, n, dout, dst, to_unc);
    if (int rc = finish_out(ctx, out, dout, out_sz * n)) return rc;
    if (int rc = finish_out(ctx, status, dst, n)) return rc;
    return finish_call(ctx);
}
int blsgpu_g1_uncompress(blsgpu_ctx* ctx, const uint8_t* in48, size_t n, uint8_t* out96, uint8_t* status) { ENTER(); return recode(ctx, in48, n, out96, status, 48, 96, false, 1); }
int blsgpu_g1_compress(blsgpu_ctx* ctx, const uint8_t* in96, size_t n, uint8_t* out48, uint8_t* status) { ENTER(); return recode(ctx, in96, n, out48, status, 96, 48, false, 0); }
int blsgpu_g2_uncompress(blsgpu_ctx* ctx, const uint8_t* in96, size_t n, uint8_t* out192, uint8_t* status) { ENTER(); return recode(ctx, in96, n, out192, status, 96, 192, true, 1); }
int blsgpu_g2_compress(blsgpu_ctx* ctx, const uint8_t* in192, size_t n, uint8_t* out96, uint8_t* status) { ENTER(); return recode(ctx, in192, n, out96, status, 192, 96, true, 0); }

int blsgpu_pool_create(blsgpu_ctx* ctx, const uint8_t* pks48, size_t n, int* handle, uint8_t* status) {
    ENTER(); if (!pks48 || !handle || !n) return fail(ctx, BLSGPU_ERR_ARG, "bad argument");
    int h = -1; for (int i = 0; i < 16; i++) if (!ctx->pool[i].soa) { h = i; break; }
    if (h < 0) return fail(ctx, BLSGPU_ERR_ARG, "too many pools");
    if (int rc = ws_reserve(ctx, al(48 * n) + al(n) + 8192)) return rc;
    const uint8_t* din; if (int rc = stage_in(ctx, din, pks48, 48 * n)) return rc;
    u32x4* soa; uint8_t* code;
    if (cudaMalloc(&soa, 96 * n) != cudaSuccess || cudaMalloc(&code, n) != cudaSuccess) { cudaGetLastError(); return fail(ctx, BLSGPU_ERR_ALLOC, "pool allocation failed"); }
    LAUNCH(k_decode_g1, nblk(n), TPB, din, n, soa, code);
    if (status) { if (ctx->ptr_mode == BLSGPU_DEVICE) CU(cudaMemcpyAsync(status, code, n, cudaMemcpyDeviceToDevice, ctx->stream)); else CU(cudaMemcpyAsync(status, code, n, cudaMemcpyDeviceToHost, ctx->stream)); }
    CU(cudaStreamSynchronize(ctx->stream));
    ctx->pool[h].soa = soa; ctx->pool[h].code = code; ctx->pool[h].n = n; *handle = h; return 0;
}
int blsgpu_pool_free(blsgpu_ctx* ctx, int handle) {
    if (!ctx || handle < 0 || handle >= 16 || !ctx->pool[handle].soa) return BLSGPU_ERR_ARG;
    dev_guard guard_; cudaSetDevice(ctx->device); cudaStreamSynchronize(ctx->stream);
    cudaFree(ctx->pool[handle].soa); cudaFree(ctx->pool[handle].code); ctx->pool[handle].soa = nullptr; ctx->pool[handle].code = nullptr; ctx->pool[handle].n = 0; return 0;
}
int blsgpu_pool_fast_aggregate_verify(blsgpu_ctx* ctx, int handle, const uint32_t* idx, const uint64_t* bitmap, size_t k, const uint8_t* msg32, const uint8_t* sig96, size_t ncomm,
                                      uint8_t* status, uint8_t* agg_pk48_out) {
    ENTER(); if (handle < 0 || handle >= 16 || !ctx->pool[handle].soa || !idx || !msg32 || !sig96 || !status) return fail(ctx, BLSGPU_ERR_ARG, "bad argument");
    if (!ncomm) return 0;
    int rc; size_t nm = ncomm * k;
    if ((rc = ws_reserve(ctx, al(4 * nm + 16) + al(8 * ((nm + 63) / 64 + 1)) + al(96 * ncomm) * 2 + al(144 * ncomm) + al(48 * ncomm) + 4 * al(ncomm) + verify_ws_bytes(ncomm, 32 * ncomm)))) return rc;
    const uint32_t* didx; const uint8_t *dmsg, *dsig; const uint64_t* dbm;
    if ((rc = stage_in(ctx, didx, idx, nm))) return rc; if ((rc = stage_in(ctx, dbm, bitmap, (nm + 63) / 64))) return rc;
    if ((rc = stage_in(ctx, dmsg, msg32, 32 * ncomm))) return rc; if ((rc = stage_in(ctx, dsig, sig96, 96 * ncomm))) return rc;
    u32x4* agg_soa = ws_take<u32x4>(ctx, 6 * ncomm); uint8_t* agg_inf = ws_take<uint8_t>(ctx, ncomm); uint8_t* agg_st = ws_take<uint8_t>(ctx, ncomm); uint8_t* code_pk = ws_take<uint8_t>(ctx, ncomm);
    uint8_t* dstatus = stage_out(ctx, status, ncomm); uint8_t* dagg = stage_out(ctx, agg_pk48_out, 48 * ncomm);
    { int L = seg_lanes(k); u32x4* ojac = ws_take<u32x4>(ctx, 9 * ncomm);
      LAUNCH(k_segsum<fp>, nblk(ncomm, SEG_WARPS * (32 / L)), 32 * SEG_WARPS, (const u32x4*)ctx->pool[handle].soa, (const uint8_t*)ctx->pool[handle].code, ctx->pool[handle].n, (const uint32_t*)nullptr, k, dbm, ncomm,
             ojac, agg_st, (uint8_t)ST_BAD_PK, didx, L);
      LAUNCH(k_jac_to_aff<fp>, nblk(ncomm), TPB, (const u32x4*)ojac, ncomm, agg_soa, agg_inf); }
    if (dagg) LAUNCH(k_encode_g1, nblk(ncomm), TPB, (const u32x4*)agg_soa, (const uint8_t*)agg_inf, ncomm, dagg);
    LAUNCH(k_fav_status, nblk(ncomm), TPB, (const uint8_t*)agg_st, (const uint8_t*)agg_inf, (const uint8_t*)nullptr, ncomm, code_pk);
    if ((rc = verify_core(ctx, agg_soa, code_pk, dmsg, nullptr, dsig, ncomm, dstatus, nullptr, nullptr))) return rc;
    if ((rc = finish_out(ctx, status, dstatus, ncomm))) return rc; if ((rc = finish_out(ctx, agg_pk48_out, dagg, 48 * ncomm))) return rc;
    return finish_call(ctx);
}

}

#include "r1cs.cuh"
#include "witness.cuh"
#include "multi.cuh"
```

bls_verify_gadget_b200/csrc/curve.cuh:

```cuda
#pragma once
#include "fp2.cuh"

namespace bls {

BLS_HD fp  f_add(const fp& a, const fp& b) { return fp_add(a, b); }
BLS_HD fp2 f_add(const fp2& a, const fp2& b) { return fp2_add(a, b); }
BLS_HD fp  f_sub(const fp& a, const fp& b) { return fp_sub(a, b); }
BLS_HD fp2 f_sub(const fp2& a, const fp2& b) { return fp2_sub(a, b); }
BLS_HD fp  f_mul(const fp& a, const fp& b) { return fp_mul(a, b); }
BLS_HD fp2 f_mul(const fp2& a, const fp2& b) { return fp2_mul(a, b); }
BLS_HD fp  f_sqr(const fp& a) { return fp_sqr(a); }
BLS_HD fp2 f_sqr(const fp2& a) { return fp2_sqr(a); }
BLS_HD fp  f_neg(const fp& a) { return fp_neg(a); }
BLS_HD fp2 f_neg(const fp2& a) { return fp2_neg(a); }
BLS_HD fp  f_inv(const fp& a) { return fp_inv(a); }
BLS_HD fp2 f_inv(const fp2& a) { return fp2_inv(a); }
BLS_HD bool f_is_zero(const fp& a) { return fp_is_zero(a); }
BLS_HD bool f_is_zero(const fp2& a) { return fp2_is_zero(a); }
BLS_HD bool f_eq(const fp& a, const fp& b) { return fp_eq(a, b); }
BLS_HD bool f_eq(const fp2& a, const fp2& b) { return fp2_eq(a, b); }
BLS_HD void f_set_one(fp& a) { a = fp_one(); }
BLS_HD void f_set_one(fp2& a) { a = fp2_one(); }
BLS_HD void f_set_zero(fp& a) { a = fp_zero(); }
BLS_HD void f_set_zero(fp2& a) { a = fp2_zero(); }

template <class F> struct aff { F x, y; };
template <class F> struct jac { F X, Y, Z; };
typedef aff<fp> g1_aff;  typedef jac<fp> g1_jac;
typedef aff<fp2> g2_aff; typedef jac<fp2> g2_jac;

template <class F> BLS_HD void jac_set_identity(jac<F>& r) { f_set_one(r.X); f_set_one(r.Y); f_set_zero(r.Z); }
template <class F> BLS_HD bool jac_is_identity(const jac<F>& p) { return f_is_zero(p.Z); }
template <class F> BLS_HD void jac_from_aff(jac<F>& r, const aff<F>& a) { r.X = a.x; r.Y = a.y; f_set_one(r.Z); }
template <class F> BLS_HD void jac_neg(jac<F>& r, const jac<F>& p) { r.X = p.X; r.Y = f_neg(p.Y); r.Z = p.Z; }

template <class F> BLS_NOINLINE void jac_dbl(jac<F>& r, const jac<F>& p) {
    F A = f_sqr(p.X), B = f_sqr(p.Y), C = f_sqr(B);
    F D = f_sub(f_sub(f_sqr(f_add(p.X, B)), A), C); D = f_add(D, D);
    F E = f_add(f_add(A, A), A), G = f_sqr(E);
    F Z3 = f_mul(p.Y, p.Z); Z3 = f_add(Z3, Z3);
    F X3 = f_sub(G, f_add(D, D));
    F C8 = f_add(C, C); C8 = f_add(C8, C8); C8 = f_add(C8, C8);
    r.Y = f_sub(f_mul(E, f_sub(D, X3)), C8); r.X = X3; r.Z = Z3;
}
template <class F> BLS_NOINLINE void jac_add_mixed(jac<F>& r, const jac<F>& p, const aff<F>& q) {
    if (f_is_zero(p.Z)) { jac_from_aff(r, q); return; }
    F Z1Z1 = f_sqr(p.Z), U2 = f_mul(q.x, Z1Z1), S2 = f_mul(f_mul(q.y, p.Z), Z1Z1);
    F H = f_sub(U2, p.X), rr = f_sub(S2, p.Y);
    bool h_zero = f_is_zero(H), r_zero = f_is_zero(rr);
    rr = f_add(rr, rr);
    F HH = f_sqr(H), I = f_add(HH, HH); I = f_add(I, I);
    F J = f_mul(H, I), V = f_mul(p.X, I);
    F X3 = f_sub(f_sub(f_sqr(rr), J), f_add(V, V));
    F YJ = f_mul(p.Y, J);
    F Z3 = f_sub(f_sub(f_sqr(f_add(p.Z, H)), Z1Z1), HH);
    F Y3 = f_sub(f_mul(rr, f_sub(V, X3)), f_add(YJ, YJ));
    if (h_zero) {
        if (r_zero) { jac<F> t; jac_from_aff(t, q); jac_dbl(r, t); } else jac_set_identity(r);
    } else { r.X = X3; r.Y = Y3; r.Z = Z3; }
}
template <class F> BLS_NOINLINE void jac_add(jac<F>& r, const jac<F>& p, const jac<F>& q) {
    if (f_is_zero(p.Z)) { r = q; return; }
    if (f_is_zero(q.Z)) { r = p; return; }
    F Z1Z1 = f_sqr(p.Z), Z2Z2 = f_sqr(q.Z);
    F U1 = f_mul(p.X, Z2Z2), U2 = f_mul(q.X, Z1Z1);
    F S1 = f_mul(f_mul(p.Y, q.Z), Z2Z2), S2 = f_mul(f_mul(q.Y, p.Z), Z1Z1);
    F H = f_sub(U2, U1), rr = f_sub(S2, S1);
    bool h_zero = f_is_zero(H), r_zero = f_is_zero(rr);
    rr = f_add(rr, rr);
    F I = f_add(H, H); I = f_sqr(I);
    F J = f_mul(H, I), V = f_mul(U1, I);
    F X3 = f_sub(f_sub(f_sqr(rr), J), f_add(V, V));
    F SJ = f_mul(S1, J);
    F Z3 = f_mul(f_sub(f_sub(f_sqr(f_add(p.Z, q.Z)), Z1Z1), Z2Z2), H);
    F Y3 = f_sub(f_mul(rr, f_sub(V, X3)), f_add(SJ, SJ));
    if (h_zero) {
        if (r_zero) { jac<F> t = p; jac_dbl(r, t); } else jac_set_identity(r);
    } else { r.X = X3; r.Y = Y3; r.Z = Z3; }
}
template <class F> BLS_HD bool jac_to_aff(aff<F>& a, const jac<F>& p) {
    if (f_is_zero(p.Z)) { f_set_zero(a.x); f_set_zero(a.y); return false; }
    F zi = f_inv(p.Z), zi2 = f_sqr(zi);
    a.x = f_mul(p.X, zi2); a.y = f_mul(p.Y, f_mul(zi2, zi));
    return true;
}
template <class F> BLS_HD bool jac_eq_aff(const jac<F>& p, const aff<F>& q) {
    if (f_is_zero(p.Z)) return false;
    F zz = f_sqr(p.Z);
    return f_eq(p.X, f_mul(q.x, zz)) & f_eq(p.Y, f_mul(q.y, f_mul(zz, p.Z)));
}
template <class F> BLS_HD void jac_mul_x_abs(jac<F>& r, const aff<F>& p) {
    jac_from_aff(r, p);
    const uint64_t x = BLS_X_ABS;
    for (int i = 62; i >= 0; i--) {
        jac_dbl(r, r);
        if ((x >> i) & 1) jac_add_mixed(r, r, p);
    }
}
template <class F> BLS_HD void jac_mul_x_abs_j(jac<F>& r, const jac<F>& p) {
    const jac<F> base = p;
    r = base;
    const uint64_t x = BLS_X_ABS;
    for (int i = 62; i >= 0; i--) {
        jac_dbl(r, r);
        if ((x >> i) & 1) jac_add(r, r, base);
    }
}
template <class F> BLS_HD void jac_mul_scalar(jac<F>& r, const aff<F>& p, const uint32_t* k) {
    jac_set_identity(r);
    for (int i = 255; i >= 0; i--) {
        jac_dbl(r, r);
        if ((k[i >> 5] >> (i & 31)) & 1) jac_add_mixed(r, r, p);
    }
}

BLS_HD fp fp_const(const uint32_t (&w)[12]) { fp r;
#pragma unroll
    for (int i = 0; i < 12; i++) r.l[i] = w[i];
    return r; }
BLS_CONST uint32_t C_BETA[12] = BLS_C_BETA;
BLS_CONST uint32_t C_FOUR[12] = BLS_C_FOUR;
BLS_CONST uint32_t C_G1X[12] = BLS_C_G1X;
BLS_CONST uint32_t C_G1Y[12] = BLS_C_G1Y;
BLS_CONST uint32_t C_G1Y_NEG[12] = BLS_C_G1Y_NEG;
BLS_CONST fp2 C_PSI_X = BLS_C_PSI_X;
BLS_CONST fp2 C_PSI_Y = BLS_C_PSI_Y;
BLS_CONST uint32_t C_PSI2_X[12] = BLS_C_PSI2_X;

BLS_HD fp g1_b() { return fp_const(C_FOUR); }
BLS_HD fp2 g2_b() { fp2 r; r.c0 = fp_const(C_FOUR); r.c1 = r.c0; return r; }

BLS_HD void g2_psi(g2_jac& r, const g2_jac& p) {
    r.X = fp2_mul(fp2_conj(p.X), C_PSI_X); r.Y = fp2_mul(fp2_conj(p.Y), C_PSI_Y); r.Z = fp2_conj(p.Z);
}
BLS_HD void g2_psi2(g2_jac& r, const g2_jac& p) {
    r.X = fp2_mul_fp(p.X, fp_const(C_PSI2_X)); r.Y = fp2_neg(p.Y); r.Z = p.Z;
}

BLS_HD bool g1_in_subgroup(const g1_aff& p) {
    g1_jac t; jac_mul_x_abs(t, p);
    g1_jac t2; jac_mul_x_abs_j(t2, t);
    g1_aff s; s.x = fp_mul(p.x, fp_const(C_BETA)); s.y = fp_neg(p.y);
    return jac_eq_aff(t2, s);
}
BLS_HD bool g2_in_subgroup(const g2_aff& p) {
    g2_jac t; jac_mul_x_abs(t, p);
    g2_jac pj; jac_from_aff(pj, p);
    g2_jac ps; g2_psi(ps, pj);
    g2_aff s; s.x = ps.X; s.y = fp2_neg(ps.Y);
    return jac_eq_aff(t, s);
}

enum { DEC_OK = 0, DEC_INF = 1, DEC_BAD_FLAGS = 2, DEC_RANGE = 3, DEC_NOT_ON_CURVE = 4, DEC_NOT_IN_SUBGROUP = 5 };

BLS_HD int g1_decode(g1_aff& out, const uint8_t* b) {
    uint32_t flags = b[0];
    out.x = fp_zero(); out.y = fp_zero();
    if (!(flags & 0x80)) return DEC_BAD_FLAGS;
    if (flags & 0x40) return DEC_INF;
    fp x; if (!fp_from_be48(x, b, 0x1f)) return DEC_RANGE;
    fp y2 = fp_add(fp_mul(fp_sqr(x), x), g1_b());
    fp y = fp_mul(y2, fp_pow_pm3d4(y2));
    if (!fp_eq(fp_sqr(y), y2)) return DEC_NOT_ON_CURVE;
    bool larger = fp_canon_is_larger_half(fp_from_mont(y));
    if (larger != ((flags & 0x20) != 0)) y = fp_neg(y);
    out.x = x; out.y = y;
    if (!g1_in_subgroup(out)) return DEC_NOT_IN_SUBGROUP;
    return DEC_OK;
}
BLS_HD void g1_encode(uint8_t* b, const g1_aff& a, bool inf) {
    if (inf) { for (int i = 0; i < 48; i++) b[i] = 0; b[0] = 0xc0; return; }
    fp_canon_to_be48(b, fp_from_mont(a.x));
    b[0] |= 0x80; if (fp_canon_is_larger_half(fp_from_mont(a.y))) b[0] |= 0x20;
}
BLS_HD int g2_decode(g2_aff& out, const uint8_t* b) {
    uint32_t flags = b[0];
    out.x = fp2_zero(); out.y = fp2_zero();
    if (!(flags & 0x80)) return DEC_BAD_FLAGS;
    if (flags & 0x40) return DEC_INF;
    fp2 x; bool ok1 = fp_from_be48(x.c1, b, 0x1f); bool ok0 = fp_from_be48(x.c0, b + 48);
    if (!(ok0 & ok1)) return DEC_RANGE;
    fp2 y2 = fp2_add(fp2_mul(fp2_sqr(x), x), g2_b());
    fp2 y; if (!fp2_sqrt(y, y2)) return DEC_NOT_ON_CURVE;
    if (fp2_lex_largest(y) != ((flags & 0x20) != 0)) y = fp2_neg(y);
    out.x = x; out.y = y;
    if (!g2_in_subgroup(out)) return DEC_NOT_IN_SUBGROUP;
    return DEC_OK;
}
BLS_HD void g2_encode(uint8_t* b, const g2_aff& a, bool inf) {
    if (inf) { for (int i = 0; i < 96; i++) b[i] = 0; b[0] = 0xc0; return; }
    fp_canon_to_be48(b, fp_from_mont(a.x.c1)); fp_canon_to_be48(b + 48, fp_from_mont(a.x.c0));
    b[0] |= 0x80; if (fp2_lex_largest(a.y)) b[0] |= 0x20;
}

BLS_HD int g1_decode_uncompressed(g1_aff& out, const uint8_t* b) {
    uint32_t flags = b[0];
    out.x = fp_zero(); out.y = fp_zero();
    if (flags & 0x80) return DEC_BAD_FLAGS;
    if (flags & 0x40) return DEC_INF;
    fp x, y; bool okx = fp_from_be48(x, b, 0x1f), oky = fp_from_be48(y, b + 48);
    if (!(okx & oky)) return DEC_RANGE;
    if (!fp_eq(fp_sqr(y), fp_add(fp_mul(fp_sqr(x), x), g1_b()))) return DEC_NOT_ON_CURVE;
    out.x = x; out.y = y;
    if (!g1_in_subgroup(out)) return DEC_NOT_IN_SUBGROUP;
    return DEC_OK;
}
BLS_HD void g1_encode_uncompressed(uint8_t* b, const g1_aff& a, bool inf) {
    if (inf) { for (int i = 0; i < 96; i++) b[i] = 0; b[0] = 0x40; return; }
    fp_canon_to_be48(b, fp_from_mont(a.x)); fp_canon_to_be48(b + 48, fp_from_mont(a.y));
}
BLS_HD int g2_decode_uncompressed(g2_aff& out, const uint8_t* b) {
    uint32_t flags = b[0];
    out.x = fp2_zero(); out.y = fp2_zero();
    if (flags & 0x80) return DEC_BAD_FLAGS;
    if (flags & 0x40) return DEC_INF;
    fp2 x, y; bool ok = fp_from_be48(x.c1, b, 0x1f); ok &= fp_from_be48(x.c0, b + 48); ok &= fp_from_be48(y.c1, b + 96); ok &= fp_from_be48(y.c0, b + 144);
    if (!ok) return DEC_RANGE;
    if (!fp2_eq(fp2_sqr(y), fp2_add(fp2_mul(fp2_sqr(x), x), g2_b()))) return DEC_NOT_ON_CURVE;
    out.x = x; out.y = y;
    if (!g2_in_subgroup(out)) return DEC_NOT_IN_SUBGROUP;
    return DEC_OK;
}
BLS_HD void g2_encode_uncompressed(uint8_t* b, const g2_aff& a, bool inf) {
    if (inf) { for (int i = 0; i < 192; i++) b[i] = 0; b[0] = 0x40; return; }
    fp_canon_to_be48(b, fp_from_mont(a.x.c1)); fp_canon_to_be48(b + 48, fp_from_mont(a.x.c0));
    fp_canon_to_be48(b + 96, fp_from_mont(a.y.c1)); fp_canon_to_be48(b + 144, fp_from_mont(a.y.c0));
}

}
```

bls_verify_gadget_b200/csrc/pairing.cuh:

```cuda
#pragma once
#include "tower.cuh"
#include "curve.cuh"

namespace bls {

struct g2_proj { fp2 x, y, z; };

BLS_NOINLINE void miller_dbl(g2_proj& r, fp2& c0, fp2& c1, fp2& c2) {
    fp2 a = fp2_half(fp2_mul(r.x, r.y));
    fp2 b = fp2_sqr(r.y), c = fp2_sqr(r.z);
    fp2 c3 = fp2_add(fp2_dbl(c), c);
    fp2 e = fp2_mul_xi(fp2_dbl(fp2_dbl(c3)));
    fp2 f = fp2_add(fp2_dbl(e), e);
    fp2 g = fp2_half(fp2_add(b, f));
    fp2 h = fp2_sub(fp2_sqr(fp2_add(r.y, r.z)), fp2_add(b, c));
    fp2 i = fp2_sub(e, b);
    fp2 j = fp2_sqr(r.x);
    fp2 es = fp2_sqr(e);
    r.x = fp2_mul(a, fp2_sub(b, f));
    r.y = fp2_sub(fp2_sqr(g), fp2_add(fp2_dbl(es), es));
    r.z = fp2_mul(b, h);
    c0 = i; c1 = fp2_add(fp2_dbl(j), j); c2 = fp2_neg(h);
}
BLS_NOINLINE void miller_add(g2_proj& r, const g2_aff& q, fp2& c0, fp2& c1, fp2& c2) {
    fp2 theta = fp2_sub(r.y, fp2_mul(q.y, r.z));
    fp2 lambda = fp2_sub(r.x, fp2_mul(q.x, r.z));
    fp2 c = fp2_sqr(theta), d = fp2_sqr(lambda);
    fp2 e = fp2_mul(lambda, d), f = fp2_mul(r.z, c), g = fp2_mul(r.x, d);
    fp2 h = fp2_sub(fp2_add(e, f), fp2_dbl(g));
    r.x = fp2_mul(lambda, h);
    r.y = fp2_sub(fp2_mul(theta, fp2_sub(g, h)), fp2_mul(e, r.y));
    r.z = fp2_mul(r.z, e);
    c0 = fp2_sub(fp2_mul(theta, q.x), fp2_mul(lambda, q.y)); c1 = fp2_neg(theta); c2 = lambda;
}
BLS_HD void miller_ell(fp12& f, const fp2& c0, const fp2& c1, const fp2& c2, const g1_aff& p) {
    fp12_mul_by_014(f, c0, fp2_mul_fp(c1, p.x), fp2_mul_fp(c2, p.y));
}
BLS_NOINLINE void miller_loop2(fp12& f, const g1_aff& p0, const g2_aff& q0, bool use0, const g1_aff& p1, const g2_aff& q1, bool use1) {
    g2_proj r0, r1;
    r0.x = q0.x; r0.y = q0.y; r0.z = fp2_one();
    r1.x = q1.x; r1.y = q1.y; r1.z = fp2_one();
    fp12_one(f);
    fp2 c0, c1, c2;
    const uint64_t x = BLS_X_ABS;
    for (int i = 62; i >= 0; i--) {
        if (i != 62) fp12_sqr(f, f);
        if (use0) { miller_dbl(r0, c0, c1, c2); miller_ell(f, c0, c1, c2, p0); }
        if (use1) { miller_dbl(r1, c0, c1, c2); miller_ell(f, c0, c1, c2, p1); }
        if ((x >> i) & 1) {
            if (use0) { miller_add(r0, q0, c0, c1, c2); miller_ell(f, c0, c1, c2, p0); }
            if (use1) { miller_add(r1, q1, c0, c1, c2); miller_ell(f, c0, c1, c2, p1); }
        }
    }
    fp12_conj(f, f);
}

BLS_NOINLINE void fp12_exp_by_x_gs(fp12& r, const fp12& a) {
    fp12 acc = a;
    const uint64_t x = BLS_X_ABS;
    for (int i = 62; i >= 0; i--) {
        fp12_cyclo_sqr(acc, acc);
        if ((x >> i) & 1) fp12_mul(acc, acc, a);
    }
    fp12_conj(r, acc);
}
struct fp12c { fp2 g2, g3, g4, g5; };
BLS_HD void fp12_compress(fp12c& c, const fp12& a) { c.g2 = a.c1.c0; c.g3 = a.c0.c2; c.g4 = a.c0.c1; c.g5 = a.c1.c2; }
BLS_NOINLINE void fp12c_sqr(fp12c& r, const fp12c& a) {
    fp12c o;
    {
        fp2 ab = fp2_mul(a.g2, a.g3);
        fp2 sm = fp2_mul(fp2_add(a.g2, a.g3), fp2_add(a.g2, fp2_mul_xi(a.g3)));
        fp2 te = fp2_sub(fp2_sub(sm, ab), fp2_mul_xi(ab)), to = fp2_dbl(ab);
        fp2 z = fp2_sub(te, a.g4); z = fp2_dbl(z); o.g4 = fp2_add(z, te);
        z = fp2_add(to, a.g5); z = fp2_dbl(z); o.g5 = fp2_add(z, to);
    }
    {
        fp2 ab = fp2_mul(a.g4, a.g5);
        fp2 sm = fp2_mul(fp2_add(a.g4, a.g5), fp2_add(a.g4, fp2_mul_xi(a.g5)));
        fp2 te = fp2_sub(fp2_sub(sm, ab), fp2_mul_xi(ab)), to = fp2_mul_xi(fp2_dbl(ab));
        fp2 z = fp2_sub(te, a.g3); z = fp2_dbl(z); o.g3 = fp2_add(z, te);
        z = fp2_add(to, a.g2); z = fp2_dbl(z); o.g2 = fp2_add(z, to);
    }
    r = o;
}
BLS_HD void fp12c_g1_fraction(fp2& num, fp2& den, const fp12c& c) {
    if (!fp2_is_zero(c.g2)) {
        fp2 t = fp2_sqr(c.g4);
        num = fp2_sub(fp2_add(fp2_mul_xi(fp2_sqr(c.g5)), fp2_add(fp2_dbl(t), t)), fp2_dbl(c.g3));
        den = fp2_dbl(fp2_dbl(c.g2));
    } else {
        num = fp2_dbl(fp2_mul(c.g4, c.g5));
        den = fp2_is_zero(c.g3) ? fp2_one() : c.g3;
    }
}
BLS_HD void fp12_decompress_with(fp12& r, const fp12c& c, const fp2& g1) {
    fp2 t = fp2_sub(fp2_add(fp2_dbl(fp2_sqr(g1)), fp2_mul(c.g2, c.g5)), fp2_mul(c.g3, c.g4));
    fp2 u = fp2_mul(c.g3, c.g4); t = fp2_sub(t, fp2_dbl(u));
    r.c0.c0 = fp2_add(fp2_mul_xi(t), fp2_one()); r.c1.c1 = g1; r.c1.c0 = c.g2; r.c0.c2 = c.g3; r.c0.c1 = c.g4; r.c1.c2 = c.g5;
}
BLS_NOINLINE void fp12_decompress_product(fp12& r, const fp12c* c, int n) {
    fp2 num[6], den[6], pre[6];
    for (int i = 0; i < n; i++) { fp12c_g1_fraction(num[i], den[i], c[i]); pre[i] = i ? fp2_mul(pre[i - 1], den[i]) : den[i]; }
    fp2 inv = fp2_inv(pre[n - 1]);
    fp12 acc, d;
    for (int i = n - 1; i >= 0; i--) {
        fp2 di = i ? fp2_mul(inv, pre[i - 1]) : inv;
        if (i) inv = fp2_mul(inv, den[i]);
        fp12_decompress_with(d, c[i], fp2_mul(num[i], di));
        if (i == n - 1) acc = d; else fp12_mul(acc, acc, d);
    }
    r = acc;
}
template <class LOAD> BLS_HD void fp12_decompress_product_from(fp12& r, LOAD load, int n) {
    fp2 num[6], den[6], pre[6];
    for (int i = 0; i < n; i++) { fp12c c = load(i); fp12c_g1_fraction(num[i], den[i], c); pre[i] = i ? fp2_mul(pre[i - 1], den[i]) : den[i]; }
    fp2 inv = fp2_inv(pre[n - 1]);
    fp12 acc, d;
    for (int i = n - 1; i >= 0; i--) {
        fp2 di = i ? fp2_mul(inv, pre[i - 1]) : inv;
        if (i) inv = fp2_mul(inv, den[i]);
        fp12c c = load(i);
        fp12_decompress_with(d, c, fp2_mul(num[i], di));
        if (i == n - 1) acc = d; else fp12_mul(acc, acc, d);
    }
    r = acc;
}
#ifndef BLS_KARABINA
#define BLS_KARABINA 1
#endif
BLS_NOINLINE void fp12_exp_by_x(fp12& r, const fp12& a) {
#if BLS_KARABINA
    fp12c c, snap[6]; fp12_compress(c, a);
    const uint64_t x = BLS_X_ABS; int k = 0;
    for (int i = 1; i <= 63; i++) {
        fp12c_sqr(c, c);
        if ((x >> i) & 1) snap[k++] = c;
    }
    fp12 acc; fp12_decompress_product(acc, snap, 6);
    fp12_conj(r, acc);
#else
    fp12_exp_by_x_gs(r, a);
#endif
}
BLS_NOINLINE void final_exponentiation(fp12& r, const fp12& f) {
    fp12 t, y0, y1, y2;
    fp12_conj(t, f); fp12_inv(y0, f); fp12_mul(r, t, y0);
    fp12_frob2(t, r); fp12_mul(r, t, r);
    fp12_cyclo_sqr(y0, r);
    fp12_exp_by_x(y1, r);
    fp12_conj(y2, r);
    fp12_mul(y1, y1, y2);
    fp12_exp_by_x(y2, y1);
    fp12_conj(y1, y1);
    fp12_mul(y1, y1, y2);
    fp12_exp_by_x(y2, y1);
    fp12_frob(y1, y1);
    fp12_mul(y1, y1, y2);
    fp12_mul(r, r, y0);
    fp12_exp_by_x(y0, y1);
    fp12_exp_by_x(y2, y0);
    fp12_frob2(y0, y1);
    fp12_conj(y1, y1);
    fp12_mul(y1, y1, y2);
    fp12_mul(y1, y1, y0);
    fp12_mul(r, r, y1);
}

template <int STEP> BLS_HD void final_exponentiation_step(fp12& r, fp12& y1, fp12& y2, const fp12& e) {
    if (STEP == 0) {
        fp12 t, y0;
        fp12_conj(t, r); fp12_inv(y0, r); fp12_mul(r, t, y0);
        fp12_frob2(t, r); fp12_mul(r, t, r);
    } else if (STEP == 1) {
        fp12_conj(y2, r);
        fp12_mul(y1, e, y2);
    } else if (STEP == 2) {
        fp12_conj(y1, y1);
        fp12_mul(y1, y1, e);
    } else if (STEP == 3) {
        fp12_frob(y1, y1);
        fp12_mul(y1, y1, e);
        fp12 y0; fp12_cyclo_sqr(y0, r); fp12_mul(r, r, y0);
    } else if (STEP == 4) {
        y2 = e;
    } else {
        fp12 y0;
        fp12_frob2(y0, y1);
        fp12_conj(y1, y1);
        fp12_mul(y1, y1, e);
        fp12_mul(y1, y1, y0);
        fp12_mul(r, r, y1);
    }
}

BLS_HD void fp_to_le48(uint8_t* b, const fp& m) {
    fp a = fp_from_mont(m);
    for (int i = 0; i < 12; i++) { uint32_t w = a.l[i]; b[4 * i] = (uint8_t)w; b[4 * i + 1] = (uint8_t)(w >> 8); b[4 * i + 2] = (uint8_t)(w >> 16); b[4 * i + 3] = (uint8_t)(w >> 24); }
}
BLS_HD void fp12_to_bytes(uint8_t* out, const fp12& a) {
    const fp2* c[6] = {&a.c0.c0, &a.c0.c1, &a.c0.c2, &a.c1.c0, &a.c1.c1, &a.c1.c2};
    for (int i = 0; i < 6; i++) { fp_to_le48(out + 96 * i, c[i]->c0); fp_to_le48(out + 96 * i + 48, c[i]->c1); }
}

}
```

bls_verify_gadget_b200/csrc/witness.cuh:

```cuda
#pragma once
#include <cooperative_groups.h>

#ifndef WIT_PF
#define WIT_PF 1
#endif
enum { WR_MULADD = 0, WR_INV = 1, WR_NEQ = 2, WR_NEQMULT = 3, WR_BIT = 4, WR_FP2INV = 5, WR_FP12INV = 6, WR_INPUT = 7 };
struct wit_rule { uint8_t kind, pad; uint16_t aux; uint32_t a, b, d; };
struct wit_xrule { uint8_t kind, pad; uint16_t aux; uint32_t var; uint32_t a_lo, a_hi, b_lo, b_hi, d_lo, d_hi; };
enum { WL_LUT = 0, WL_SUM = 1, WL_BIT = 2, WL_INPUT = 3, WL_ONE = 4 };
#define WL_NO_COL 0xffffffffu
#define WL_INT 0x80000000u
struct wit_lrule { uint8_t kind, flags; uint16_t aux; uint32_t var; uint32_t a[6]; };
struct wit_prog {
    size_t nvars, nout, nlc, nterms, nlevels;
    wit_rule* rules; uint64_t* lc_ptr; uint32_t* col; fp* coeff; fp* coeffc; uint8_t* cls;
    wit_xrule* xrules; uint64_t* level_ptr;
    struct wit_lrule* lrules; uint32_t* llevel_ptr; uint32_t* lt_col; long long* lt_coef; size_t n_light, n_llevels, n_islots, n_lterms;
    size_t msg_len, ninputs, nkeys;
};
#define WIT_POINT_INPUTS 6

__device__ __forceinline__ void wit_store(u32x4* zt, size_t col, int lane, const fp& v) {
    u32x4 a, b, c;
    a.x = v.l[0]; a.y = v.l[1]; a.z = v.l[2]; a.w = v.l[3]; b.x = v.l[4]; b.y = v.l[5]; b.z = v.l[6]; b.w = v.l[7]; c.x = v.l[8]; c.y = v.l[9]; c.z = v.l[10]; c.w = v.l[11];
// ... 210 lines not shown
        }
        pre = level + 1 < p.nlevels && hi + cw < hi_next;
        if (pre) rn = p.xrules[hi + cw];
        cluster.sync();
        lo = hi; hi = hi_next;
    }
}
#define WIT_LIGHT_TPB 1024
__global__ void __launch_bounds__(WIT_LIGHT_TPB, 1) k_witness_light(wit_prog p, const fp* inputs, size_t nwit_padded, u32x4* zt_all, uint2* zbool_all, long long* sint_all) {
    size_t group = blockIdx.x; int tid = threadIdx.x, lane = tid & 31, warp = tid >> 5;
    uint2* zb = zbool_all + group * p.nvars; long long* sint = sint_all + group * p.n_islots * 32; u32x4* zt = zt_all + group * p.nvars * 96;
    uint32_t lut_lo = p.llevel_ptr[0], w_lo = p.llevel_ptr[1], nxt = p.llevel_ptr[2];
    wit_lrule rt, rw; bool pre_t = lut_lo + tid < w_lo, pre_w = w_lo + warp < nxt;
    if (pre_t) rt = p.lrules[lut_lo + tid];
    if (pre_w) rw = p.lrules[w_lo + warp];
    for (size_t L = 0; L < p.n_llevels; L++) {
        for (uint32_t i = lut_lo + tid; i < w_lo; i += WIT_LIGHT_TPB) {
            wit_lrule r = (pre_t && i == lut_lo + tid) ? rt : p.lrules[i];
            uint32_t x0 = zb[r.a[0]].x, x1 = r.a[1] != WL_NO_COL ? zb[r.a[1]].x : 0u, x2 = r.a[2] != WL_NO_COL ? zb[r.a[2]].x : 0u;
            uint32_t out;
            if (r.a[3] != WL_NO_COL) { uint32_t x3 = zb[r.a[3]].x, x4 = r.a[4] != WL_NO_COL ? zb[r.a[4]].x : 0u; out = r1cs_lut5(r.a[5], x0, x1, x2, x3, x4); }
            else out = r1cs_lut3(r.a[5], x0, x1, x2);
            zb[r.var] = make_uint2(out, 1u);
        }
        for (uint32_t i = w_lo + warp; i < nxt; i += WIT_LIGHT_TPB / 32) {
            wit_lrule r = (pre_w && i == w_lo + warp) ? rw : p.lrules[i];
            if (r.kind == WL_ONE) { if (lane == 0) zb[r.var] = make_uint2(0xffffffffu, 1u); continue; }
            if (r.kind == WL_INPUT) {
                uint32_t bit = inputs[(size_t)r.aux * nwit_padded + group * 32 + lane].l[0] & 1u;
                uint32_t pack = __ballot_sync(0xffffffffu, bit); if (lane == 0) zb[r.var] = make_uint2(pack, 1u); continue;
            }
            long long sum = 0;
            for (uint32_t t0 = r.a[0]; t0 < r.a[1]; t0 += 32) {
                uint32_t n = r.a[1] - t0 < 32 ? r.a[1] - t0 : 32u, myc = 0; long long myk = 0;
                if ((uint32_t)lane < n) { myc = p.lt_col[t0 + lane]; myk = p.lt_coef[t0 + lane]; }
                uint32_t myw = ((uint32_t)lane < n && !(myc & WL_INT)) ? zb[myc].x : 0u;
                for (uint32_t t = 0; t < n; t++) {
                    uint32_t c = __shfl_sync(0xffffffffu, myc, t); long long k = __shfl_sync(0xffffffffu, myk, t); uint32_t wd = __shfl_sync(0xffffffffu, myw, t);
                    long long v = (c & WL_INT) ? sint[(size_t)(c & ~WL_INT) * 32 + lane] : (long long)((wd >> lane) & 1u);
                    sum += k * v;
                }
            }
            if (r.kind == WL_BIT || (r.flags & 1)) {
                uint32_t bit = r.kind == WL_BIT ? (uint32_t)((unsigned long long)sum >> (r.aux & 63)) & 1u : (uint32_t)sum & 1u;
                uint32_t pack = __ballot_sync(0xffffffffu, bit); if (lane == 0) zb[r.var] = make_uint2(pack, 1u);
            } else {
                sint[(size_t)r.a[2] * 32 + lane] = sum;
                if (r.flags & 2) {
                    unsigned long long mag = sum < 0 ? (unsigned long long)(-sum) : (unsigned long long)sum;
                    fp v = fp_zero(); v.l[0] = (uint32_t)mag; v.l[1] = (uint32_t)(mag >> 32);
                    if (sum < 0) { fp n; fp_sub_raw(n, fp_modulus(), v); v = n; }
                    wit_store(zt, r.var, lane, v); if (lane == 0) zb[r.var] = make_uint2(0u, 0u);
                }
            }
        }
        lut_lo = nxt; pre_t = pre_w = false;
        if (L + 1 < p.n_llevels) {
            w_lo = p.llevel_ptr[2 * L + 3]; nxt = p.llevel_ptr[2 * L + 4];
            pre_t = lut_lo + tid < w_lo; pre_w = w_lo + warp < nxt;
            if (pre_t) rt = p.lrules[lut_lo + tid];
            if (pre_w) rw = p.lrules[w_lo + warp];
        }
        __syncthreads();
    }
}
__global__ void __launch_bounds__(TPB, BLS_MINB) k_witness_inputs(const u32x4* pk_soa, const uint8_t* code_pk, const u32x4* sig_soa, const uint8_t* code_sig, const uint8_t* msg, size_t msg_len,
                                                                  size_t nwit, size_t nwit_padded, fp* inputs, uint8_t* status) {
    size_t i = blockIdx.x * (size_t)blockDim.x + threadIdx.x; if (i >= nwit_padded) return;
    bool live = i < nwit; uint8_t st = ST_OK;
    if (live) { if (code_pk[i] != DEC_OK) st = ST_BAD_PK; else if (code_sig[i] != DEC_OK) st = ST_BAD_SIG; }
    bool ok = live && st == ST_OK;
    fp zero = fp_zero();
    for (size_t k = 0; k < 8 * msg_len; k++) { fp b = zero; if (ok) b.l[0] = (msg[msg_len * i + (k >> 3)] >> (k & 7)) & 1u; inputs[(size_t)(WIT_POINT_INPUTS + k) * nwit_padded + i] = b; }
    g1_aff pk; g2_aff sg;
    if (ok) { soa_load_g1(pk, pk_soa, nwit, i); soa_load_g2(sg, sig_soa, nwit, i); }
    inputs[(size_t)0 * nwit_padded + i] = ok ? fp_from_mont(pk.x) : zero; inputs[(size_t)1 * nwit_padded + i] = ok ? fp_from_mont(pk.y) : zero;
    inputs[(size_t)2 * nwit_padded + i] = ok ? fp_from_mont(sg.x.c0) : zero; inputs[(size_t)3 * nwit_padded + i] = ok ? fp_from_mont(sg.x.c1) : zero;
    inputs[(size_t)4 * nwit_padded + i] = ok ? fp_from_mont(sg.y.c0) : zero; inputs[(size_t)5 * nwit_padded + i] = ok ? fp_from_mont(sg.y.c1) : zero;
    if (live && status) status[i] = st;
}
__global__ void __launch_bounds__(TPB, BLS_MINB) k_witness_inputs_agg(const u32x4* key_soa, const uint8_t* code_key, size_t n, const uint8_t* bitmap, const u32x4* sig_soa, const uint8_t* code_sig,
                                                                      const uint8_t* msg, size_t msg_len, size_t nwit, size_t nwit_padded, fp* inputs, uint8_t* status) {
    size_t i = blockIdx.x * (size_t)blockDim.x + threadIdx.x; if (i >= nwit_padded) return;
    bool live = i < nwit; uint8_t st = ST_OK;
    if (live) { for (size_t k = 0; k < n; k++) if (code_key[i * n + k] != DEC_OK) { st = ST_BAD_PK; break; } if (st == ST_OK && code_sig[i] != DEC_OK) st = ST_BAD_SIG; }
    bool ok = live && st == ST_OK;
    fp zero = fp_zero();
    for (size_t k = 0; k < n; k++) {
        g1_aff pk; if (ok) soa_load_g1(pk, key_soa, nwit * n, i * n + k);
        inputs[(2 * k) * nwit_padded + i] = ok ? fp_from_mont(pk.x) : zero; inputs[(2 * k + 1) * nwit_padded + i] = ok ? fp_from_mont(pk.y) : zero;
        fp b = zero; if (ok) b.l[0] = bitmap[i * n + k] ? 1u : 0u; inputs[(2 * n + k) * nwit_padded + i] = b;
    }
    g2_aff sg; if (ok) soa_load_g2(sg, sig_soa, nwit, i);
    inputs[(3 * n + 0) * nwit_padded + i] = ok ? fp_from_mont(sg.x.c0) : zero; inputs[(3 * n + 1) * nwit_padded + i] = ok ? fp_from_mont(sg.x.c1) : zero;
    inputs[(3 * n + 2) * nwit_padded + i] = ok ? fp_from_mont(sg.y.c0) : zero; inputs[(3 * n + 3) * nwit_padded + i] = ok ? fp_from_mont(sg.y.c1) : zero;
    for (size_t k = 0; k < 8 * msg_len; k++) { fp b = zero; if (ok) b.l[0] = (msg[msg_len * i + (k >> 3)] >> (k & 7)) & 1u; inputs[(3 * n + 4 + k) * nwit_padded + i] = b; }
    if (live && status) status[i] = st;
}
__global__ void __launch_bounds__(256) k_witness_untranspose(const u32x4* zt_all, const uint2* zbool_all, size_t ncols, size_t nout, size_t nwit, u32x4* z) {
    size_t col = blockIdx.x * (size_t)8 + (threadIdx.x >> 5); int lane = threadIdx.x & 31; size_t group = blockIdx.y;
    size_t w = group * 32 + lane;
    if (col >= nout || w >= nwit) return;
    const u32x4* zt = zt_all + group * ncols * 96;
    u32x4* dst = z + (w * nout + col) * 3;
    if (zbool_all) {
        uint2 f = zbool_all[group * ncols + col];
        if (f.y) { u32x4 v; v.x = (f.x >> lane) & 1u; v.y = v.z = v.w = 0; u32x4 zero; zero.x = zero.y = zero.z = zero.w = 0; dst[0] = v; dst[1] = zero; dst[2] = zero; return; }
    }
    dst[0] = zt[(col * 3) * 32 + lane]; dst[1] = zt[(col * 3 + 1) * 32 + lane]; dst[2] = zt[(col * 3 + 2) * 32 + lane];
}

static void wit_release(wit_prog* p) {
    cudaFree(p->rules); cudaFree(p->lc_ptr); cudaFree(p->col); cudaFree(p->coeff); cudaFree(p->coeffc); cudaFree(p->cls);
    cudaFree(p->xrules); cudaFree(p->level_ptr); cudaFree(p->lrules); cudaFree(p->llevel_ptr); cudaFree(p->lt_col); cudaFree(p->lt_coef);
    delete p;
}

extern "C" {
struct wit_split { std::vector<wit_lrule> lrules; std::vector<uint32_t> llevel_ptr, lt_col; std::vector<long long> lt_coef; size_t n_islots = 0;
                   std::vector<wit_xrule> xrules; std::vector<uint64_t> hlevel_ptr; };
static bool wit_small_coef(const uint8_t* c48, long long& out) {
    static const uint8_t PB[48] = {0xab, 0xaa, 0xff, 0xff, 0xff, 0xff, 0xfe, 0xb9, 0xff, 0xff, 0x53, 0xb1, 0xfe, 0xff, 0xab, 0x1e, 0x24, 0xf6, 0xb0, 0xf6, 0xa0, 0xd2, 0x30, 0x67,
                                   0xbf, 0x12, 0x85, 0xf3, 0x84, 0x4b, 0x77, 0x64, 0xd7, 0xac, 0x4b, 0x43, 0xb6, 0xa7, 0x1b, 0x4b, 0x9a, 0xe6, 0x7f, 0x39, 0xea, 0x11, 0x01, 0x1a};
    bool hi = false; for (int i = 6; i < 48; i++) hi |= c48[i] != 0;
    if (!hi) { long long v = 0; for (int i = 5; i >= 0; i--) v = (v << 8) | c48[i]; out = v; return true; }
    for (int i = 8; i < 48; i++) if (c48[i] != PB[i]) return false;
    unsigned long long lo = 0, pl = 0; for (int i = 7; i >= 0; i--) { lo = (lo << 8) | c48[i]; pl = (pl << 8) | PB[i]; }
    if (lo > pl) return false;
    unsigned long long d = pl - lo; if (d >= (1ull << 48)) return false;
    out = -(long long)d; return true;
}
static void wit_split_program(wit_split& S, const wit_rule* hr, const uint64_t* lc_ptr, const uint32_t* lc_col, const uint8_t* lc_coef48, size_t ncols, size_t nout,
                              const uint32_t* order, size_t nkeys, size_t ninputs) {
    enum : uint8_t { HEAVY = 0, LB = 1, LI = 2 };
    std::vector<uint8_t> state(ncols, HEAVY); std::vector<uint32_t> llev(ncols, 0), hlev(ncols, 0), islot(ncols, 0); std::vector<long long> vmin(ncols, 0), vmax(ncols, 0);
    std::vector<uint8_t> is_small; std::vector<long long> coef;
    auto lo_of = [&](uint32_t id) { return id ? lc_ptr[id - 1] : (uint64_t)0; }; auto hi_of = [&](uint32_t id) { return id ? lc_ptr[id] : (uint64_t)0; };
    size_t nterms = lc_ptr ? 0 : 0; (void)nterms;
    auto bool_input = [&](uint16_t slot) { return nkeys ? ((slot >= 2 * nkeys && slot < 3 * nkeys) || slot >= 3 * nkeys + 4) : slot >= WIT_POINT_INPUTS; };
    struct lrec { wit_lrule r; uint32_t level; }; std::vector<lrec> light; std::vector<uint32_t> heavy_vars;
    const __int128 LIM = (__int128)1 << 62;
    for (size_t oi = 0; oi < ncols; oi++) {
        uint32_t v = order[oi]; const wit_rule& r = hr[v];
        wit_lrule lr; memset(&lr, 0, sizeof lr); lr.var = v; lr.aux = r.aux; for (int k = 0; k < 6; k++) lr.a[k] = WL_NO_COL;
        bool is_light = false; uint32_t level = 0;
        if (r.kind == WR_INPUT) {
            if (r.aux == 0xffff) { lr.kind = WL_ONE; state[v] = LB; is_light = true; }
            else if ((size_t)r.aux < ninputs && bool_input(r.aux)) { lr.kind = WL_INPUT; state[v] = LB; is_light = true; }
        } else if (r.kind == WR_MULADD || r.kind == WR_BIT) {
            uint32_t ids[3] = {r.a, r.kind == WR_BIT ? 0u : r.b, r.kind == WR_BIT ? 0u : r.d}; bool ok = true; uint32_t mx = 0;
            struct term { uint32_t col; long long k; int which; }; std::vector<term> ts;
            for (int q = 0; q < 3 && ok; q++) for (uint64_t t = lo_of(ids[q]); t < hi_of(ids[q]); t++) {
                uint32_t c = lc_col[t]; long long k;
                if (state[c] == HEAVY || !wit_small_coef(lc_coef48 + 48 * t, k)) { ok = false; break; }
                ts.push_back({c, k, q}); if (llev[c] > mx) mx = llev[c];
            }
            if (ok) {
                level = mx + 1;
                if (r.kind == WR_MULADD && !r.a && r.b) ok = false;
                if (!ok) { }
                else if (r.kind == WR_MULADD && r.a) {
                    uint32_t cs[5]; int d = 0; bool fits = true;
                    for (auto& t : ts) { if (state[t.col] != LB) { fits = false; break; } if (t.col == 0) continue;
                                         int j = 0; while (j < d && cs[j] != t.col) j++; if (j == d) { if (d == 5) { fits = false; break; } cs[d++] = t.col; } }
                    if (fits && d == 0) { cs[d++] = 0; }
                    if (fits) {
                        uint32_t table = 0; bool boolean = true;
                        for (uint32_t idx = 0; idx < 32 && boolean; idx++) {
                            __int128 s[3] = {0, 0, 0};
                            for (auto& t : ts) { if (t.col == 0) { s[t.which] += t.k; continue; } int j = 0; while (cs[j] != t.col) j++; if ((idx >> j) & 1) s[t.which] += t.k; }
                            __int128 val = s[0] * s[1] + s[2];
                            if (val == 1) table |= 1u << idx; else if (val != 0) boolean = false;
                        }
                        if (boolean) { lr.kind = WL_LUT; for (int j = 0; j < d; j++) lr.a[j] = cs[j]; lr.a[5] = table; state[v] = LB; is_light = true; }
                    }
                } else {
                    __int128 mn = 0, mxv = 0;
                    for (auto& t : ts) { __int128 a = t.col == 0 ? 1 : state[t.col] == LB ? 0 : vmin[t.col], b = state[t.col] == LB ? 1 : vmax[t.col]; __int128 x = a * t.k, y = b * t.k; mn += x < y ? x : y; mxv += x < y ? y : x; }
                    bool range_ok = mn > -LIM && mxv < LIM && ts.size() < (1u << 20);
                    if (range_ok && (r.kind == WR_MULADD || (mn >= 0 && r.aux < 63))) {
                        lr.kind = r.kind == WR_BIT ? WL_BIT : WL_SUM; lr.a[0] = (uint32_t)S.lt_col.size();
                        for (auto& t : ts) { S.lt_col.push_back(state[t.col] == LI ? (WL_INT | islot[t.col]) : t.col); S.lt_coef.push_back(t.k); }
                        lr.a[1] = (uint32_t)S.lt_col.size(); is_light = true;
                        if (r.kind == WR_BIT || (mn >= 0 && mxv <= 1)) { state[v] = LB; if (r.kind == WR_MULADD) lr.flags |= 1; }
                        else { state[v] = LI; vmin[v] = (long long)mn; vmax[v] = (long long)mxv; islot[v] = (uint32_t)S.n_islots; lr.a[2] = (uint32_t)S.n_islots++; if (v < nout) lr.flags |= 2; }
                    }
                }
            }
        }
        if (is_light) { llev[v] = level; light.push_back({lr, level}); }
        else heavy_vars.push_back(v);
    }
    std::vector<uint8_t> export_int(ncols, 0); uint32_t hmax = 0;
    auto scan = [&](uint32_t id, uint32_t& m) { for (uint64_t t = lo_of(id); t < hi_of(id); t++) { uint32_t c = lc_col[t]; if (state[c] == LI) export_int[c] = 1; if (state[c] == HEAVY && hlev[c] > m) m = hlev[c]; } };
    for (uint32_t v : heavy_vars) {
        const wit_rule& r = hr[v]; uint32_t m = 0;
        if (r.kind == WR_INPUT) { hlev[v] = 0; continue; }
        if (r.kind == WR_FP12INV) { for (uint32_t k = 0; k < 12; k++) scan(r.a + k, m); } else { scan(r.a, m); scan(r.b, m); scan(r.d, m); }
        hlev[v] = m + 1; if (hlev[v] > hmax) hmax = hlev[v];
    }
    for (auto& l : light) if (l.r.kind == WL_SUM && !(l.r.flags & 1) && export_int[l.r.var]) l.r.flags |= 2;
    uint32_t lmax = 0; for (auto& l : light) if (l.level > lmax) lmax = l.level;
    size_t nl = light.empty() ? 0 : (size_t)lmax + 1;
    std::vector<uint32_t> cnt(2 * nl + 1, 0);
    for (auto& l : light) cnt[2 * l.level + (l.r.kind == WL_LUT ? 0 : 1) + 1]++;
    for (size_t i = 0; i < 2 * nl; i++) cnt[i + 1] += cnt[i];
    S.llevel_ptr = cnt; S.lrules.resize(light.size());
    { std::vector<uint32_t> pos(cnt.begin(), cnt.end() - 1); for (auto& l : light) S.lrules[pos[2 * l.level + (l.r.kind == WL_LUT ? 0 : 1)]++] = l.r; }
    size_t nh = (size_t)hmax + 1; std::vector<uint64_t> hc(nh + 1, 0);
    for (uint32_t v : heavy_vars) hc[hlev[v] + 1]++;
    for (size_t i = 0; i < nh; i++) hc[i + 1] += hc[i];
    S.hlevel_ptr = hc; S.xrules.resize(heavy_vars.size());
    { std::vector<uint64_t> pos(hc.begin(), hc.end() - 1);
      for (uint32_t v : heavy_vars) {
          const wit_rule& r = hr[v]; wit_xrule& x = S.xrules[pos[hlev[v]]++];
          x.kind = r.kind; x.pad = 0; x.aux = r.aux; x.var = v;
          if (r.kind == WR_FP12INV) { x.a_lo = r.a; x.a_hi = r.a + 12; x.b_lo = x.b_hi = x.d_lo = x.d_hi = 0; }
          else { x.a_lo = (uint32_t)lo_of(r.a); x.a_hi = (uint32_t)hi_of(r.a); x.b_lo = (uint32_t)lo_of(r.b); x.b_hi = (uint32_t)hi_of(r.b); x.d_lo = (uint32_t)lo_of(r.d); x.d_hi = (uint32_t)hi_of(r.d); }
      } }
}
static int witness_load_impl(blsgpu_ctx* ctx, const uint8_t* rules16, const uint64_t* lc_ptr, const uint32_t* lc_col, const uint8_t* lc_coef48, size_t nvars, size_t nout, size_t nlc, size_t nterms,
                             const uint32_t* order, const uint64_t* level_ptr, size_t nlevels, size_t nkeys, int* handle) {
    if (!rules16 || !lc_ptr || !lc_col || !lc_coef48 || !handle || !nvars || !nout || nout > nvars) return fail(ctx, BLSGPU_ERR_ARG, "bad argument");
    if (ctx->ptr_mode != BLSGPU_HOST) return fail(ctx, BLSGPU_ERR_ARG, "blsgpu_witness_load takes host pointers (the level-ordered rule tables are built on the host)");
    int h = -1; for (int i = 0; i < 4; i++) if (!ctx->wit[i]) { h = i; break; }
    if (h < 0) return fail(ctx, BLSGPU_ERR_ARG, "too many witness programs loaded");
    wit_prog* p = new (std::nothrow) wit_prog(); if (!p) return fail(ctx, BLSGPU_ERR_ALLOC, "out of host memory");
    memset(p, 0, sizeof *p); p->nvars = nvars; p->nout = nout; p->nlc = nlc; p->nterms = nterms;
    struct guard_t { wit_prog* p; ~guard_t() { if (p) wit_release(p); } } undo{p};
    const wit_rule* hr = reinterpret_cast<const wit_rule*>(rules16);
    {
        size_t top = 0;
        for (size_t k = 0; k < nvars; k++) if (hr[k].kind == WR_INPUT && hr[k].aux != 0xffff && (size_t)hr[k].aux + 1 > top) top = (size_t)hr[k].aux + 1;
        size_t fixed = nkeys ? 3 * nkeys + 4 : WIT_POINT_INPUTS;
        if (top < fixed || (top - fixed) % 8) return fail(ctx, BLSGPU_ERR_ARG, "witness program: %zu input slots is not %zu + 8 x message bytes%s", top, fixed, nkeys ? "" : " (an aggregate_verify program is loaded with blsgpu_witness_load_aggregate)");
        p->ninputs = top; p->nkeys = nkeys; p->msg_len = (top - fixed) / 8;
    }
    size_t nt = nterms ? nterms : 1;
    CU(cudaMalloc(&p->rules, 16 * nvars)); CU(cudaMalloc(&p->lc_ptr, 8 * (nlc + 1))); CU(cudaMalloc(&p->col, 4 * nt));
    CU(cudaMalloc(&p->coeff, 48 * nt)); CU(cudaMalloc(&p->coeffc, 48 * nt)); CU(cudaMalloc(&p->cls, nt));
    CU(cudaMemcpyAsync(p->rules, rules16, 16 * nvars, cudaMemcpyHostToDevice, ctx->stream)); CU(cudaMemcpyAsync(p->lc_ptr, lc_ptr, 8 * (nlc + 1), cudaMemcpyHostToDevice, ctx->stream));
    if (nterms) {
        CU(cudaMemcpyAsync(p->col, lc_col, 4 * nterms, cudaMemcpyHostToDevice, ctx->stream));
        dev_tmp raw; CU(cudaMalloc(&raw.p, 48 * nterms));
        CU(cudaMemcpyAsync(raw.p, lc_coef48, 48 * nterms, cudaMemcpyHostToDevice, ctx->stream));
        LAUNCH(k_r1cs_prepare, nblk(nterms), TPB, (const uint8_t*)raw.p, nterms, p->coeff, p->coeffc, p->cls);
        CU(cudaStreamSynchronize(ctx->stream));
    }
    if (order && level_ptr && nlevels) {
        wit_split S; wit_split_program(S, hr, lc_ptr, lc_col, lc_coef48, nvars, nout, order, nkeys, p->ninputs);
        p->nlevels = S.hlevel_ptr.size() - 1; p->n_light = S.lrules.size(); p->n_llevels = S.llevel_ptr.size() / 2; p->n_islots = S.n_islots; p->n_lterms = S.lt_col.size();
        size_t nx = S.xrules.size() ? S.xrules.size() : 1, nlr = S.lrules.size() ? S.lrules.size() : 1, nlt = S.lt_col.size() ? S.lt_col.size() : 1;
        CU(cudaMalloc(&p->xrules, sizeof(wit_xrule) * nx)); CU(cudaMalloc(&p->level_ptr, 8 * S.hlevel_ptr.size()));
        CU(cudaMalloc(&p->lrules, sizeof(wit_lrule) * nlr)); CU(cudaMalloc(&p->llevel_ptr, 4 * (S.llevel_ptr.size() ? S.llevel_ptr.size() : 1)));
        CU(cudaMalloc(&p->lt_col, 4 * nlt)); CU(cudaMalloc(&p->lt_coef, 8 * nlt));
        if (S.xrules.size()) CU(cudaMemcpyAsync(p->xrules, S.xrules.data(), sizeof(wit_xrule) * S.xrules.size(), cudaMemcpyHostToDevice, ctx->stream));
        CU(cudaMemcpyAsync(p->level_ptr, S.hlevel_ptr.data(), 8 * S.hlevel_ptr.size(), cudaMemcpyHostToDevice, ctx->stream));
        if (S.lrules.size()) CU(cudaMemcpyAsync(p->lrules, S.lrules.data(), sizeof(wit_lrule) * S.lrules.size(), cudaMemcpyHostToDevice, ctx->stream));
        if (S.llevel_ptr.size()) CU(cudaMemcpyAsync(p->llevel_ptr, S.llevel_ptr.data(), 4 * S.llevel_ptr.size(), cudaMemcpyHostToDevice, ctx->stream));
        if (S.lt_col.size()) { CU(cudaMemcpyAsync(p->lt_col, S.lt_col.data(), 4 * S.lt_col.size(), cudaMemcpyHostToDevice, ctx->stream)); CU(cudaMemcpyAsync(p->lt_coef, S.lt_coef.data(), 8 * S.lt_coef.size(), cudaMemcpyHostToDevice, ctx->stream)); }
        CU(cudaStreamSynchronize(ctx->stream));
    }
    CU(cudaStreamSynchronize(ctx->stream));
    undo.p = nullptr; ctx->wit[h] = p; *handle = h; return 0;
}
int blsgpu_witness_load(blsgpu_ctx* ctx, const uint8_t* rules16, const uint64_t* lc_ptr, const uint32_t* lc_col, const uint8_t* lc_coef48, size_t nvars, size_t nout, size_t nlc, size_t nterms,
                        const uint32_t* order, const uint64_t* level_ptr, size_t nlevels, int* handle) {
    ENTER(); return witness_load_impl(ctx, rules16, lc_ptr, lc_col, lc_coef48, nvars, nout, nlc, nterms, order, level_ptr, nlevels, 0, handle);
}
int blsgpu_witness_load_aggregate(blsgpu_ctx* ctx, const uint8_t* rules16, const uint64_t* lc_ptr, const uint32_t* lc_col, const uint8_t* lc_coef48, size_t nvars, size_t nout, size_t nlc, size_t nterms,
                                  const uint32_t* order, const uint64_t* level_ptr, size_t nlevels, size_t nkeys, int* handle) {
    ENTER(); if (!nkeys) return fail(ctx, BLSGPU_ERR_ARG, "nkeys must be positive"); return witness_load_impl(ctx, rules16, lc_ptr, lc_col, lc_coef48, nvars, nout, nlc, nterms, order, level_ptr, nlevels, nkeys, handle);
}
long blsgpu_witness_msg_len(blsgpu_ctx* ctx, int handle) { return (!ctx || handle < 0 || handle >= 4 || !ctx->wit[handle]) ? -1 : (long)ctx->wit[handle]->msg_len; }
int blsgpu_witness_shape(blsgpu_ctx* ctx, int handle, uint64_t counts[4]) {
    if (!ctx || handle < 0 || handle >= 4 || !ctx->wit[handle] || !counts) return BLSGPU_ERR_ARG;
    const wit_prog* p = ctx->wit[handle]; counts[0] = p->n_light; counts[1] = p->n_llevels; counts[2] = p->nlevels; counts[3] = p->n_islots; return 0;
}
int blsgpu_witness_free(blsgpu_ctx* ctx, int handle) {
    if (!ctx || handle < 0 || handle >= 4 || !ctx->wit[handle]) return BLSGPU_ERR_ARG;
    dev_guard guard_; cudaSetDevice(ctx->device); cudaStreamSynchronize(ctx->stream);
    wit_release(ctx->wit[handle]); ctx->wit[handle] = nullptr; return 0;
}
}
static int witness_run(blsgpu_ctx* ctx, const wit_prog& p, const uint8_t* pk48, const uint8_t* bitmap, const uint8_t* msg, const uint8_t* sig96, size_t nwit, uint8_t* status, size_t extra,
                       bool want_zbool, u32x4** zt_out, uint2** zbool_out, uint8_t** dstatus_out) {
    if ((bitmap != nullptr) != (p.nkeys != 0)) return fail(ctx, BLSGPU_ERR_ARG, p.nkeys ? "this is an aggregate_verify program: use the _aggregate entry points" : "this is a verify program: use blsgpu_witness_gen / _check");
    size_t groups = (nwit + 31) / 32, np = groups * 32, ninputs = p.ninputs, nk = p.nkeys ? p.nkeys : 1, nkeys_total = nwit * nk;
    if (int rc = ws_reserve(ctx, al(48 * nkeys_total) + al(nkeys_total) + al(96 * nwit) + al(p.msg_len * nwit + 1) + al(96 * nkeys_total) + al(192 * nwit) + 2 * al(np) + al(nkeys_total + np) + al(48 * ninputs * np) + al(groups * p.nvars * 1536) +
                                 (want_zbool ? al(groups * p.nvars * 8) : 0) + al(groups * (p.n_islots + 1) * 256) + extra + 65536)) return rc;
    const uint8_t *dpk, *dsig, *dmsg, *dbm = nullptr;
    if (int rc = stage_in(ctx, dpk, pk48, 48 * nkeys_total)) return rc;
    if (bitmap) { if (int rc = stage_in(ctx, dbm, bitmap, nkeys_total)) return rc; }
    if (int rc = stage_in(ctx, dsig, sig96, 96 * nwit)) return rc;
    if (int rc = stage_in(ctx, dmsg, msg, p.msg_len * nwit ? p.msg_len * nwit : 1)) return rc;
    u32x4* pk_soa = ws_take<u32x4>(ctx, 6 * nkeys_total); u32x4* sig_soa = ws_take<u32x4>(ctx, 12 * nwit);
    uint8_t* code_pk = ws_take<uint8_t>(ctx, nkeys_total + np); uint8_t* code_sig = ws_take<uint8_t>(ctx, np);
    uint8_t* dstatus = status ? stage_out(ctx, status, nwit) : nullptr;
    fp* inputs = ws_take<fp>(ctx, ninputs * np);
    u32x4* zt_all = ws_take<u32x4>(ctx, groups * p.nvars * 96);
    uint2* zbool_all = want_zbool ? ws_take<uint2>(ctx, groups * p.nvars) : nullptr;
    long long* sint_all = ws_take<long long>(ctx, groups * (p.n_islots + 1) * 32);
    LAUNCH(k_decode_g1, nblk(nkeys_total), TPB, dpk, nkeys_total, pk_soa, code_pk);
    LAUNCH(k_decode_g2, nblk(nwit), TPB, dsig, nwit, sig_soa, code_sig);
    if (bitmap) LAUNCH(k_witness_inputs_agg, nblk(np), TPB, (const u32x4*)pk_soa, (const uint8_t*)code_pk, p.nkeys, dbm, (const u32x4*)sig_soa, (const uint8_t*)code_sig, dmsg, p.msg_len, nwit, np, inputs, dstatus);
    else LAUNCH(k_witness_inputs, nblk(np), TPB, (const u32x4*)pk_soa, (const uint8_t*)code_pk, (const u32x4*)sig_soa, (const uint8_t*)code_sig, dmsg, p.msg_len, nwit, np, inputs, dstatus);
    if (p.xrules && !want_zbool) return fail(ctx, BLSGPU_ERR_ARG, "the level-synchronous replay works on the packed 0/1 view");
    if (p.xrules && p.n_light) LAUNCH(k_witness_light, (unsigned)groups, WIT_LIGHT_TPB, p, (const fp*)inputs, np, zt_all, zbool_all, sint_all);
    if (p.xrules && ctx->wit_cluster) {
        cudaLaunchConfig_t cfg; memset(&cfg, 0, sizeof cfg);
        cfg.gridDim = dim3((unsigned)(groups * WIT_CL)); cfg.blockDim = dim3(WIT_CL_TPB); cfg.stream = ctx->stream;
        cudaLaunchAttribute at[1]; at[0].id = cudaLaunchAttributeClusterDimension; at[0].val.clusterDim.x = WIT_CL; at[0].val.clusterDim.y = 1; at[0].val.clusterDim.z = 1;
        cfg.attrs = at; cfg.numAttrs = 1;
        wit_prog pc = p; const fp* in_c = inputs;
        CU(cudaLaunchKernelEx(&cfg, k_witness_cluster, pc, in_c, np, zt_all, groups, zbool_all)); ctx->launches++;
    } else if (p.xrules) {
        int per_sm = 0, sms = 0;
        CU(cudaOccupancyMaxActiveBlocksPerMultiprocessor(&per_sm, k_witness_levels, WIT_TPB, 0)); if (per_sm > WIT_BPS) per_sm = WIT_BPS; CU(cudaDeviceGetAttribute(&sms, cudaDevAttrMultiProcessorCount, ctx->device));
        if (per_sm < 1) return fail(ctx, BLSGPU_ERR_CUDA, "k_witness_levels does not fit on an SM");
        wit_prog pc = p; const fp* in_c = inputs; void* args[] = {(void*)&pc, (void*)&in_c, (void*)&np, (void*)&zt_all, (void*)&groups, (void*)&zbool_all};
        CU(cudaLaunchCooperativeKernel((void*)k_witness_levels, dim3((unsigned)(per_sm * sms)), dim3(WIT_TPB), args, 0, ctx->stream)); ctx->launches++;
    } else {
        if (p.nvars != p.nout || want_zbool) return fail(ctx, BLSGPU_ERR_ARG, "the sequential replay needs a program without scratch columns (load it with its level order)");
        LAUNCH(k_witness_gen, (unsigned)groups, 32, p, (const fp*)inputs, np, zt_all);
    }
    *zt_out = zt_all; if (zbool_out) *zbool_out = zbool_all; *dstatus_out = dstatus;
    return 0;
}
extern "C" {
static int witness_gen_core(blsgpu_ctx* ctx, int handle, const uint8_t* pk48, const uint8_t* bitmap, const uint8_t* msg, const uint8_t* sig96, size_t nwit, uint8_t* z48, uint8_t* status) {
    if (handle < 0 || handle >= 4 || !ctx->wit[handle] || !pk48 || !msg || !sig96 || !z48) return fail(ctx, BLSGPU_ERR_ARG, "bad argument");
    if (!nwit) return 0;
    wit_prog p = *ctx->wit[handle];
    size_t groups = (nwit + 31) / 32;
    bool host = ctx->ptr_mode == BLSGPU_HOST;
    size_t zbytes = nwit * p.nout * 48;
    u32x4* zt_all; uint2* zbool_all = nullptr; uint8_t* dstatus;
    if (int rc = witness_run(ctx, p, pk48, bitmap, msg, sig96, nwit, status, host ? al(zbytes) : 0, p.xrules != nullptr, &zt_all, &zbool_all, &dstatus)) return rc;
    uint8_t* dz = host ? ws_take<uint8_t>(ctx, zbytes) : z48;
    { dim3 grid(nblk(p.nout, 8), (unsigned)groups); k_witness_untranspose<<<grid, 256, 0, ctx->stream>>>((const u32x4*)zt_all, (const uint2*)zbool_all, p.nvars, p.nout, nwit, (u32x4*)dz); ctx->launches++; CU(cudaGetLastError()); }
    if (host) CU(cudaMemcpyAsync(z48, dz, zbytes, cudaMemcpyDeviceToHost, ctx->stream));
    if (status) { if (int rc = finish_out(ctx, status, dstatus, nwit)) return rc; }
    return finish_call(ctx);
}
static int witness_check_core(blsgpu_ctx* ctx, int wit_handle, int r1cs_handle, const uint8_t* pk48, const uint8_t* bitmap, const uint8_t* msg, const uint8_t* sig96, size_t nwit,
                              uint64_t* sat_bits, uint8_t* all_sat, uint8_t* status) {
    if (wit_handle < 0 || wit_handle >= 4 || !ctx->wit[wit_handle] || r1cs_handle < 0 || r1cs_handle >= 16 || !ctx->r1cs[r1cs_handle] || !pk48 || !msg || !sig96 || !sat_bits)
        return fail(ctx, BLSGPU_ERR_ARG, "bad argument");
    if (!nwit) return 0;
    wit_prog p = *ctx->wit[wit_handle]; r1cs_sys s = *ctx->r1cs[r1cs_handle];
    if (p.nout != s.ncols) return fail(ctx, BLSGPU_ERR_ARG, "witness program and R1CS system have different column counts");
    if (!p.xrules) return fail(ctx, BLSGPU_ERR_ARG, "blsgpu_witness_check needs a program loaded with its level order");
    size_t groups = (nwit + 31) / 32, words = (s.nrows + 63) / 64, part_bytes = R1_LONG_ROWS ? 64 : (s.n_seg ? s.n_seg : 1) * 32 * 48;
    bool host = ctx->ptr_mode == BLSGPU_HOST;
    u32x4* zt_all; uint2* zbool_all; uint8_t* dstatus;
    if (int rc = witness_run(ctx, p, pk48, bitmap, msg, sig96, nwit, status, al(part_bytes) + (host ? al(8 * words * nwit) + al(nwit) : 0), true, &zt_all, &zbool_all, &dstatus)) return rc;
    u32x4* part = ws_take<u32x4>(ctx, part_bytes / 16);
    uint64_t* dbits = host ? ws_take<uint64_t>(ctx, words * nwit) : sat_bits;
    uint8_t* dall = all_sat ? (host ? ws_take<uint8_t>(ctx, nwit) : all_sat) : nullptr;
    CU(cudaMemsetAsync(dbits, 0, 8 * words * nwit, ctx->stream));
    for (size_t gi = 0; gi < groups; gi++) {
        size_t w0 = gi * 32, g = nwit - w0 < 32 ? nwit - w0 : 32;
        if (int rc = r1cs_check_group(ctx, s, zt_all + gi * p.nvars * 96, zbool_all + gi * p.nvars, part, w0, g, words, dbits)) return rc;
    }
    if (dall) LAUNCH(k_r1cs_all, nblk(nwit, 8), 256, (const uint64_t*)dbits, nwit, words, s.nrows, dall);
    if (host) {
        CU(cudaMemcpyAsync(sat_bits, dbits, 8 * words * nwit, cudaMemcpyDeviceToHost, ctx->stream));
        if (all_sat) CU(cudaMemcpyAsync(all_sat, dall, nwit, cudaMemcpyDeviceToHost, ctx->stream));
    }
    if (status) { if (int rc = finish_out(ctx, status, dstatus, nwit)) return rc; }
    return finish_call(ctx);
}
int blsgpu_witness_gen(blsgpu_ctx* ctx, int handle, const uint8_t* pk48, const uint8_t* msg, const uint8_t* sig96, size_t nwit, uint8_t* z48, uint8_t* status) {
    ENTER(); return witness_gen_core(ctx, handle, pk48, nullptr, msg, sig96, nwit, z48, status);
}
int blsgpu_witness_check(blsgpu_ctx* ctx, int wit_handle, int r1cs_handle, const uint8_t* pk48, const uint8_t* msg, const uint8_t* sig96, size_t nwit,
                         uint64_t* sat_bits, uint8_t* all_sat, uint8_t* status) {
    ENTER(); return witness_check_core(ctx, wit_handle, r1cs_handle, pk48, nullptr, msg, sig96, nwit, sat_bits, all_sat, status);
}
int blsgpu_witness_gen_aggregate(blsgpu_ctx* ctx, int handle, const uint8_t* pks48, const uint8_t* bitmap, const uint8_t* msg, const uint8_t* sig96, size_t nwit, uint8_t* z48, uint8_t* status) {
    ENTER(); if (!bitmap) return fail(ctx, BLSGPU_ERR_ARG, "null bitmap"); return witness_gen_core(ctx, handle, pks48, bitmap, msg, sig96, nwit, z48, status);
}
int blsgpu_witness_check_aggregate(blsgpu_ctx* ctx, int wit_handle, int r1cs_handle, const uint8_t* pks48, const uint8_t* bitmap, const uint8_t* msg, const uint8_t* sig96, size_t nwit,
                                   uint64_t* sat_bits, uint8_t* all_sat, uint8_t* status) {
    ENTER(); if (!bitmap) return fail(ctx, BLSGPU_ERR_ARG, "null bitmap"); return witness_check_core(ctx, wit_handle, r1cs_handle, pks48, bitmap, msg, sig96, nwit, sat_bits, all_sat, status);
}
}
```

Baseline: 864,200.

## Fuse G2 signature subgroup check into the Miller loop's final point

In the split verify path, signature decoding now skips the standalone G2 subgroup check. Instead, the Miller loop's final accumulated point for the signature pairing, which is |x|·sig, is compared against psi(sig) in projective form, which is the Bowe/Scott-style psi-based membership test. Signatures that fail are marked bad in the accumulate kernel. This removes a separate scalar multiplication per signature by reusing work the Miller loop already does, at the cost of an extra byte array and a check whose correctness depends on the sign conventions of the loop's point arithmetic matching the psi criterion.

```diff
diff --git a/bls_verify_gadget_b200/csrc/blsgpu.cu b/bls_verify_gadget_b200/csrc/blsgpu.cu
--- a/bls_verify_gadget_b200/csrc/blsgpu.cu
+++ b/bls_verify_gadget_b200/csrc/blsgpu.cu
@@ -122,10 +122,10 @@
     if (soa) soa_store_g1(soa, n, i, p);
     code[i] = (uint8_t)rc;
 }
-__global__ void __launch_bounds__(TPB, BLS_MINB_DG2) k_decode_g2(const uint8_t* in96, size_t n, u32x4* soa, uint8_t* code) {
+template <bool SUBGROUP> __global__ void __launch_bounds__(TPB, BLS_MINB_DG2) k_decode_g2(const uint8_t* in96, size_t n, u32x4* soa, uint8_t* code) {
     phase_skew();
     size_t i = blockIdx.x * (size_t)blockDim.x + threadIdx.x; if (i >= n) return;
-    g2_aff p; int rc = g2_decode(p, in96 + 96 * i);
+    g2_aff p; int rc = g2_decode<SUBGROUP>(p, in96 + 96 * i);
     if (soa) soa_store_g2(soa, n, i, p);
     code[i] = (uint8_t)rc;
 }
@@ -207,7 +207,7 @@
     soa_store_fp12(f_soa, n, i, f);
 }
 __global__ void __launch_bounds__(TPB, BLS_MINB_LINES) k_miller_lines(const u32x4* pk_soa, const u32x4* hm_soa, const u32x4* sig_soa, const uint8_t* flags, const uint8_t* status,
-                                                                size_t n, u32x4* t_soa, u32x4* lines, int i_hi, int i_lo) {
+                                                                size_t n, u32x4* t_soa, u32x4* lines, int i_hi, int i_lo, uint8_t* sig_sub) {
     size_t t = blockIdx.x * (size_t)blockDim.x + threadIdx.x; if (t >= 2 * n) return;
     int j = t >= n; size_t i = t - (j ? n : 0);
     if (status[i] != ST_OK) return;
@@ -226,8 +226,10 @@
         }
     }
     if (i_lo != 0) { soa_store_fp2(t_soa, n, i, 3 * j, r.x); soa_store_fp2(t_soa, n, i, 3 * j + 1, r.y); soa_store_fp2(t_soa, n, i, 3 * j + 2, r.z); }
-}
-__global__ void __launch_bounds__(TPB, BLS_MINB_ACCUM) k_miller_accum(const uint8_t* flags, const uint8_t* status, size_t n, u32x4* f_soa, const u32x4* lines, int i_hi, int i_lo) {
+    else if (j == 0 && sig_sub) sig_sub[i] = miller_end_in_subgroup(r, q) ? 1 : 0;
+}
+__global__ void __launch_bounds__(TPB, BLS_MINB_ACCUM) k_miller_accum(const uint8_t* flags, uint8_t* status, size_t n, u32x4* f_soa, const u32x4* lines, int i_hi, int i_lo,
+                                                                const uint8_t* sig_sub) {
     size_t i = blockIdx.x * (size_t)blockDim.x + threadIdx.x; if (i >= n) return;
     if (status[i] != ST_OK) return;
     uint8_t fl = flags[i]; bool use0 = !(fl & FL_SIG_INF), use1 = !(fl & FL_HM_INF);
@@ -242,6 +244,7 @@
         }
     }
     if (i_lo == 0) fp12_conj(f, f);
+    if (i_lo == 0 && sig_sub && use0 && !sig_sub[i]) { status[i] = ST_BAD_SIG; return; }
     soa_store_fp12(f_soa, n, i, f);
 }
 __global__ void __launch_bounds__(TPB, BLS_MINB_SQR) k_final_squarings(const u32x4* in_soa, u32x4* snap_soa, const uint8_t* status, size_t n) {
@@ -324,7 +327,8 @@
     if (active) soa_store_fp2(f_soa, n, item, COOP_TOWER_POS[c.k], r);
     if (in_range && c.k == 0) status_out[item] = active ? ((((ball >> (6 * g)) & 63u) == 63u) ? (uint8_t)ST_OK : (uint8_t)ST_FALSE) : st;
 }
-__global__ void __launch_bounds__(128, 2) k_miller_accum_coop(const uint8_t* flags, const uint8_t* status, size_t n, u32x4* f_soa, const u32x4* lines, int i_hi, int i_lo) {
+__global__ void __launch_bounds__(128, 2) k_miller_accum_coop(const uint8_t* flags, uint8_t* status, size_t n, u32x4* f_soa, const u32x4* lines, int i_hi, int i_lo,
+                                                            const uint8_t* sig_sub) {
     __shared__ coop_smem sm[4];
     int warp = threadIdx.x >> 5, lane = threadIdx.x & 31, g = lane / 6;
     coop_lane c = coop_init(&sm[warp]);
@@ -347,6 +351,7 @@
             }
     }
     if (i_lo == 0) f = coop_conj(c, f);
+    if (active && i_lo == 0 && sig_sub && use[0] && !sig_sub[item]) { if (c.k == 0) status[item] = ST_BAD_SIG; return; }
     if (active) soa_store_fp2(f_soa, n, item, COOP_TOWER_POS[c.k], f);
 }
 __global__ void __launch_bounds__(TPB, BLS_MINB) k_gt_reduce(const u32x4* in_soa, const uint8_t* status, size_t n, u32x4* out_soa, size_t T) {
@@ -792,7 +797,7 @@
     if (int rc = ws_reserve(ctx, al(96 * n) + al(n) + 4096)) return rc;
     const uint8_t* din; if (int rc = stage_in(ctx, din, in96, 96 * n)) return rc;
     uint8_t* dst = stage_out(ctx, status, n);
-    LAUNCH(k_decode_g2, nblk(n), TPB, din, n, (u32x4*)nullptr, dst);
+    LAUNCH(k_decode_g2<true>, nblk(n), TPB, din, n, (u32x4*)nullptr, dst);
     if (int rc = finish_out(ctx, status, dst, n)) return rc;
     return finish_call(ctx);
 }
@@ -824,24 +829,26 @@
     } else LAUNCH(k_hash_to_g2, nblk(n), TPB, dmsg, doff, n, code_pk, code_sig, hm_soa, flags, dstatus);
     return 0;
 }
-static int miller_stage_split(blsgpu_ctx* ctx, const u32x4* pk_soa, const u32x4* hm_soa, const u32x4* sig_soa, const uint8_t* flags, const uint8_t* dstatus, size_t n,
-                              u32x4* f_soa, u32x4* t_soa , u32x4* lines , bool coop = false) {
+static int miller_stage_split(blsgpu_ctx* ctx, const u32x4* pk_soa, const u32x4* hm_soa, const u32x4* sig_soa, const uint8_t* flags, uint8_t* dstatus, size_t n,
+                              u32x4* f_soa, u32x4* t_soa , u32x4* lines , uint8_t* sig_sub, bool coop = false) {
     for (int hi = 62; hi >= 0; hi -= MILLER_LINE_ITERS) {
         int lo = hi - MILLER_LINE_ITERS + 1 < 0 ? 0 : hi - MILLER_LINE_ITERS + 1;
-        LAUNCH(k_miller_lines, nblk(2 * n), TPB, pk_soa, hm_soa, sig_soa, flags, dstatus, n, t_soa, lines, hi, lo);
-        if (coop) LAUNCH(k_miller_accum_coop, nblk(n, 20), 128, flags, dstatus, n, f_soa, (const u32x4*)lines, hi, lo);
-        else LAUNCH(k_miller_accum, nblk(n), TPB, flags, dstatus, n, f_soa, (const u32x4*)lines, hi, lo);
+        LAUNCH(k_miller_lines, nblk(2 * n), TPB, pk_soa, hm_soa, sig_soa, flags, (const uint8_t*)dstatus, n, t_soa, lines, hi, lo, sig_sub);
+        if (coop) LAUNCH(k_miller_accum_coop, nblk(n, 20), 128, flags, dstatus, n, f_soa, (const u32x4*)lines, hi, lo, (const uint8_t*)sig_sub);
+        else LAUNCH(k_miller_accum, nblk(n), TPB, flags, dstatus, n, f_soa, (const u32x4*)lines, hi, lo, (const uint8_t*)sig_sub);
     }
     return 0;
 }
 static int verify_core(blsgpu_ctx* ctx, const u32x4* pk_soa, const uint8_t* code_pk, const uint8_t* dmsg, const uint32_t* doff, const uint8_t* dsig, size_t n,
-                       uint8_t* dstatus, uint32_t* dbitmap, u32x4* gt_acc , bool forked = false) {
+                       uint8_t* dstatus, uint32_t* dbitmap, u32x4* gt_acc , bool forked = false, bool sig_sub_in_miller = false) {
     u32x4* sig_soa = ws_take<u32x4>(ctx, 12 * n); u32x4* hm_soa = ws_take<u32x4>(ctx, 12 * n); u32x4* f_soa = ws_take<u32x4>(ctx, 36 * n);
     uint8_t* code_sig = ws_take<uint8_t>(ctx, n); uint8_t* flags = ws_take<uint8_t>(ctx, n);
+    uint8_t* sig_sub = sig_sub_in_miller && ctx->split ? ws_take<uint8_t>(ctx, n) : nullptr;
+    auto decode_sig = sig_sub ? k_decode_g2<false> : k_decode_g2<true>;
     if (forked) {
         cudaStream_t main_stream = ctx->stream; int rc = 0;
         ctx->stream = ctx->lane_stream[0]; cudaStreamWaitEvent(ctx->stream, ctx->fork, 0);
-        k_decode_g2<<<nblk(n), TPB, 0, ctx->stream>>>(dsig, n, sig_soa, code_sig); ctx->launches++; cudaEventRecord(ctx->lane_done[0], ctx->stream);
+        decode_sig<<<nblk(n), TPB, 0, ctx->stream>>>(dsig, n, sig_soa, code_sig); ctx->launches++; cudaEventRecord(ctx->lane_done[0], ctx->stream);
         ctx->stream = ctx->lane_stream[1]; cudaStreamWaitEvent(ctx->stream, ctx->fork, 0);
         rc = hash_stage(ctx, dmsg, doff, n, nullptr, nullptr, hm_soa, f_soa, flags, nullptr); cudaEventRecord(ctx->lane_done[1], ctx->stream);
         ctx->stream = main_stream;
@@ -851,7 +858,7 @@
         LAUNCH(k_status_merge, nblk(n, 256), 256, code_pk, (const uint8_t*)code_sig, n, flags, dstatus);
     } else {
     STAGE_MARK(1);
-    LAUNCH(k_decode_g2, nblk(n), TPB, dsig, n, sig_soa, code_sig);
+    LAUNCH(decode_sig, nblk(n), TPB, dsig, n, sig_soa, code_sig);
     STAGE_MARK(2);
     if (int rc = hash_stage(ctx, dmsg, doff, n, code_pk, code_sig, hm_soa, f_soa, flags, dstatus)) return rc;
     }
@@ -861,7 +868,7 @@
     if (ctx->split) {
         u32x4* t_soa = ws_take<u32x4>(ctx, 36 * n); y1_soa = t_soa; y2_soa = ws_take<u32x4>(ctx, 36 * n);
         u32x4* lines = ws_take<u32x4>(ctx, (size_t)MILLER_LINE_STEPS * 2 * 18 * n);
-        if (int rc = miller_stage_split(ctx, pk_soa, hm_soa, sig_soa, flags, dstatus, n, f_soa, t_soa, lines, coop)) return rc;
+        if (int rc = miller_stage_split(ctx, pk_soa, hm_soa, sig_soa, flags, dstatus, n, f_soa, t_soa, lines, sig_sub, coop)) return rc;
         snap_soa = lines;
     } else {
 #if BLS_F_IN_SMEM
@@ -900,7 +907,7 @@
     return 0;
 }
 static size_t verify_ws_bytes(size_t n, size_t mb) {
-    return 2 * al(576 * n) + al((size_t)MILLER_LINE_STEPS * 2 * 288 * n)  + al(48 * n) + al(96 * n) + al(mb + 1) + al(4 * (n + 1)) + al(n) * 6 + al(96 * n) + 2 * al(192 * n) + al(576 * n) + al(8 * ((n + 63) / 64)) +
+    return 2 * al(576 * n) + al((size_t)MILLER_LINE_STEPS * 2 * 288 * n)  + al(48 * n) + al(96 * n) + al(mb + 1) + al(4 * (n + 1)) + al(n) * 7 + al(96 * n) + 2 * al(192 * n) + al(576 * n) + al(8 * ((n + 63) / 64)) +
            al(576 * ((n + 7) / 8)) + al(576 * ((n + 63) / 64)) + 3 * al(576) + 65536;
 }
 static int ensure_lanes(blsgpu_ctx* ctx);
@@ -925,7 +932,7 @@
     if (forked) { if ((rc = ensure_lanes(ctx))) return rc; forked = ctx->stream != ctx->lane_stream[0] && ctx->stream != ctx->lane_stream[1]; }
     if (forked) CU(cudaEventRecord(ctx->fork, ctx->stream));
     LAUNCH(k_decode_g1, nblk(m), TPB, dpk, m, pk_soa, code_pk);
-    if ((rc = verify_core(ctx, pk_soa, code_pk, dmsg, doff, dsig, m, dstatus, dbitmap, gt_acc, forked))) return rc;
+    if ((rc = verify_core(ctx, pk_soa, code_pk, dmsg, doff, dsig, m, dstatus, dbitmap, gt_acc, forked, true))) return rc;
     if ((rc = finish_out(ctx, status + base, dstatus, m))) return rc;
     if (ok_bitmap && (rc = finish_out(ctx, ok_bitmap + base / 64, (uint64_t*)dbitmap, (m + 63) / 64))) return rc;
     return 0;
@@ -1032,7 +1039,7 @@
         u32x4* rs = ws_take<u32x4>(ctx, 18 * m); u32x4* ja = ws_take<u32x4>(ctx, 18 * ((m + 7) / 8)); u32x4* jb = ws_take<u32x4>(ctx, 18 * ((m + 63) / 64)); u32x4* jone = ws_take<u32x4>(ctx, 18);
         u32x4* ta = ws_take<u32x4>(ctx, 36 * ((m + 7) / 8)); u32x4* tb = ws_take<u32x4>(ctx, 36 * ((m + 63) / 64)); u32x4* one = ws_take<u32x4>(ctx, 36);
         LAUNCH(k_decode_g1, nblk(m), TPB, dpk, m, pk_soa, code_pk);
-        LAUNCH(k_decode_g2, nblk(m), TPB, dsig, m, sig_soa, code_sig);
+        LAUNCH(k_decode_g2<true>, nblk(m), TPB, dsig, m, sig_soa, code_sig);
         if ((rc = hash_stage(ctx, dmsg, doff, m, code_pk, code_sig, hm_soa, f_soa, flags, dstatus))) break;
         LAUNCH(k_any_bad, nblk(((m + 31) / 32) * 32, 256), 256, (const uint8_t*)dstatus, m, bad);
         LAUNCH(k_rlc_scale, nblk(m), TPB, pk_soa, (const u32x4*)sig_soa, flags, (const uint8_t*)dstatus, m, base, (const uint8_t*)dseed, rs);
@@ -1048,7 +1055,7 @@
         }
         if (ctx->split) {
             u32x4* t_soa = ws_take<u32x4>(ctx, 36 * m); u32x4* lines = ws_take<u32x4>(ctx, (size_t)MILLER_LINE_STEPS * 2 * 18 * m);
-            if ((rc = miller_stage_split(ctx, pk_soa, hm_soa, sig_soa, flags, dstatus, m, f_soa, t_soa, lines))) break;
+            if ((rc = miller_stage_split(ctx, pk_soa, hm_soa, sig_soa, flags, dstatus, m, f_soa, t_soa, lines, nullptr))) break;
         } else LAUNCH(k_miller, nblk(m), TPB, (const u32x4*)pk_soa, (const u32x4*)hm_soa, (const u32x4*)sig_soa, (const uint8_t*)flags, (const uint8_t*)dstatus, m, f_soa);
         if ((rc = gt_product(ctx, f_soa, dstatus, m, ta, tb, one))) break;
         LAUNCH(k_gt_mul_into, 1, 32, f_acc, (const u32x4*)one);
@@ -1099,7 +1106,7 @@
         u32x4* rs = ws_take<u32x4>(ctx, 18 * m); u32x4* ja = ws_take<u32x4>(ctx, 18 * P * T0); u32x4* jb = ws_take<u32x4>(ctx, 18 * P * T0);
         u32x4* ta = ws_take<u32x4>(ctx, 36 * P * T0); u32x4* tb = ws_take<u32x4>(ctx, 36 * P * T0); uint8_t* dok = ws_take<uint8_t>(ctx, P);
         LAUNCH(k_decode_g1, nblk(m), TPB, dpk, m, pk_soa, code_pk);
-        LAUNCH(k_decode_g2, nblk(m), TPB, dsig, m, sig_soa, code_sig);
+        LAUNCH(k_decode_g2<true>, nblk(m), TPB, dsig, m, sig_soa, code_sig);
         if ((rc = hash_stage(ctx, dmsg, doff, m, code_pk, code_sig, hm_soa, f_soa, flags, dstatus))) return rc;
         LAUNCH(k_rlc_scale, nblk(m), TPB, pk_soa, (const u32x4*)sig_soa, flags, (const uint8_t*)dstatus, m, base, (const uint8_t*)dseed, rs);
         const u32x4* s_piece; const u32x4* f_piece;
@@ -1115,7 +1122,7 @@
         }
         if (ctx->split) {
             u32x4* t_soa = ws_take<u32x4>(ctx, 36 * m); u32x4* lines = ws_take<u32x4>(ctx, (size_t)MILLER_LINE_STEPS * 2 * 18 * m);
-            if ((rc = miller_stage_split(ctx, pk_soa, hm_soa, sig_soa, flags, dstatus, m, f_soa, t_soa, lines))) return rc;
+            if ((rc = miller_stage_split(ctx, pk_soa, hm_soa, sig_soa, flags, dstatus, m, f_soa, t_soa, lines, nullptr))) return rc;
         } else LAUNCH(k_miller, nblk(m), TPB, (const u32x4*)pk_soa, (const u32x4*)hm_soa, (const u32x4*)sig_soa, (const uint8_t*)flags, (const uint8_t*)dstatus, m, f_soa);
         {
             const u32x4* cur = f_soa; const uint8_t* st = dstatus; size_t cnt_n = m, len = L; u32x4* bufs[2] = {ta, tb}; int which = 0;
@@ -1178,7 +1185,7 @@
     uint8_t* dst = status && ctx->ptr_mode == BLSGPU_DEVICE ? status : ws_take<uint8_t>(ctx, nprod);
     uint8_t* dgt = stage_out(ctx, gt, 576 * nprod);
     LAUNCH(k_decode_g1, nblk(tot), TPB, d1, tot, s1, c1);
-    LAUNCH(k_decode_g2, nblk(tot), TPB, d2, tot, s2, c2);
+    LAUNCH(k_decode_g2<true>, nblk(tot), TPB, d2, tot, s2, c2);
     LAUNCH(k_miller_pairs, nblk(nprod), TPB, (const u32x4*)s1, (const u32x4*)s2, (const uint8_t*)c1, (const uint8_t*)c2, npairs, nprod, f, dst);
     uint8_t* scratch = ws_take<uint8_t>(ctx, nprod);
     LAUNCH(k_final_exp, nblk(nprod), TPB, f, (const uint8_t*)dst, scratch, nprod);
@@ -1248,7 +1255,7 @@
     u32x4* soa = ws_take<u32x4>(ctx, 12 * npts + 1); uint8_t* code = ws_take<uint8_t>(ctx, npts + 1);
     u32x4* osoa = ws_take<u32x4>(ctx, 12 * nseg); uint8_t* oinf = ws_take<uint8_t>(ctx, nseg);
     uint8_t* dout = stage_out(ctx, out96, 96 * nseg); uint8_t* dst = stage_out(ctx, status, nseg);
-    if (npts) LAUNCH(k_decode_g2, nblk(npts), TPB, din, npts, soa, code);
+    if (npts) LAUNCH(k_decode_g2<true>, nblk(npts), TPB, din, npts, soa, code);
     { int L = seg_lanes(npts / nseg); u32x4* ojac = ws_take<u32x4>(ctx, 18 * nseg);
       LAUNCH(k_segsum<fp2>, nblk(nseg, SEG_WARPS * (32 / L)), 32 * SEG_WARPS, (const u32x4*)soa, (const uint8_t*)code, npts, dseg, (size_t)0, (const uint64_t*)nullptr, nseg, ojac, dst, (uint8_t)ST_BAD_SIG, (const uint32_t*)nullptr, L);
       LAUNCH(k_jac_to_aff<fp2>, nblk(nseg), TPB, (const u32x4*)ojac, nseg, osoa, oinf); }
@@ -1307,7 +1314,7 @@
         LAUNCH(k_hash_to_g2, nblk(npairs), TPB, dmsg, doff, npairs, (const uint8_t*)code_pk, (const uint8_t*)code_inf, hm_soa, pflags, pstatus);
         LAUNCH(k_miller, nblk(npairs), TPB, (const u32x4*)pk_soa, (const u32x4*)hm_soa, (const u32x4*)zero_g2, (const uint8_t*)pflags, (const uint8_t*)pstatus, npairs, f_pair);
     }
-    LAUNCH(k_decode_g2, nblk(nsig), TPB, dsig, nsig, sig_soa, code_sig);
+    LAUNCH(k_decode_g2<true>, nblk(nsig), TPB, dsig, nsig, sig_soa, code_sig);
     LAUNCH(k_aggv_sig_status, nblk(nsig), TPB, (const uint8_t*)code_sig, nsig, sstatus, sflags);
     CU(cudaMemsetAsync(zero_g1, 0, 96 * nsig, ctx->stream)); CU(cudaMemsetAsync(zero_hm, 0, 192 * nsig, ctx->stream));
     LAUNCH(k_miller, nblk(nsig), TPB, (const u32x4*)zero_g1, (const u32x4*)zero_hm, (const u32x4*)sig_soa, (const uint8_t*)sflags, (const uint8_t*)sstatus, nsig, f_sig);
diff --git a/bls_verify_gadget_b200/csrc/curve.cuh b/bls_verify_gadget_b200/csrc/curve.cuh
--- a/bls_verify_gadget_b200/csrc/curve.cuh
+++ b/bls_verify_gadget_b200/csrc/curve.cuh
@@ -173,7 +173,7 @@
     fp_canon_to_be48(b, fp_from_mont(a.x));
     b[0] |= 0x80; if (fp_canon_is_larger_half(fp_from_mont(a.y))) b[0] |= 0x20;
 }
-BLS_HD int g2_decode(g2_aff& out, const uint8_t* b) {
+template <bool SUBGROUP = true> BLS_HD int g2_decode(g2_aff& out, const uint8_t* b) {
     uint32_t flags = b[0];
     out.x = fp2_zero(); out.y = fp2_zero();
     if (!(flags & 0x80)) return DEC_BAD_FLAGS;
@@ -184,7 +184,7 @@
     fp2 y; if (!fp2_sqrt(y, y2)) return DEC_NOT_ON_CURVE;
     if (fp2_lex_largest(y) != ((flags & 0x20) != 0)) y = fp2_neg(y);
     out.x = x; out.y = y;
-    if (!g2_in_subgroup(out)) return DEC_NOT_IN_SUBGROUP;
+    if (SUBGROUP && !g2_in_subgroup(out)) return DEC_NOT_IN_SUBGROUP;
     return DEC_OK;
 }
 BLS_HD void g2_encode(uint8_t* b, const g2_aff& a, bool inf) {
diff --git a/bls_verify_gadget_b200/csrc/pairing.cuh b/bls_verify_gadget_b200/csrc/pairing.cuh
--- a/bls_verify_gadget_b200/csrc/pairing.cuh
+++ b/bls_verify_gadget_b200/csrc/pairing.cuh
@@ -32,6 +32,11 @@
     r.y = fp2_sub(fp2_mul(theta, fp2_sub(g, h)), fp2_mul(e, r.y));
     r.z = fp2_mul(r.z, e);
     c0 = fp2_sub(fp2_mul(theta, q.x), fp2_mul(lambda, q.y)); c1 = fp2_neg(theta); c2 = lambda;
+}
+BLS_NOINLINE bool miller_end_in_subgroup(const g2_proj& r, const g2_aff& sig) {
+    g2_jac sj, ps; jac_from_aff(sj, sig); g2_psi(ps, sj);
+    fp2 px = fp2_mul(ps.X, r.z), py = fp2_mul(ps.Y, r.z);
+    return !fp2_is_zero(r.z) & fp2_eq(r.x, px) & fp2_eq(fp2_neg(r.y), py);
 }
 BLS_HD void miller_ell(fp12& f, const fp2& c0, const fp2& c1, const fp2& c2, const g1_aff& p) {
     fp12_mul_by_014(f, c0, fp2_mul_fp(c1, p.x), fp2_mul_fp(c2, p.y));
diff --git a/bls_verify_gadget_b200/csrc/witness.cuh b/bls_verify_gadget_b200/csrc/witness.cuh
--- a/bls_verify_gadget_b200/csrc/witness.cuh
+++ b/bls_verify_gadget_b200/csrc/witness.cuh
@@ -536,7 +536,7 @@
     uint2* zbool_all = want_zbool ? ws_take<uint2>(ctx, groups * p.nvars) : nullptr;
     long long* sint_all = ws_take<long long>(ctx, groups * (p.n_islots + 1) * 32);
     LAUNCH(k_decode_g1, nblk(nkeys_total), TPB, dpk, nkeys_total, pk_soa, code_pk);
-    LAUNCH(k_decode_g2, nblk(nwit), TPB, dsig, nwit, sig_soa, code_sig);
+    LAUNCH(k_decode_g2<true>, nblk(nwit), TPB, dsig, nwit, sig_soa, code_sig);
     if (bitmap) LAUNCH(k_witness_inputs_agg, nblk(np), TPB, (const u32x4*)pk_soa, (const uint8_t*)code_pk, p.nkeys, dbm, (const u32x4*)sig_soa, (const uint8_t*)code_sig, dmsg, p.msg_len, nwit, np, inputs, dstatus);
     else LAUNCH(k_witness_inputs, nblk(np), TPB, (const u32x4*)pk_soa, (const uint8_t*)code_pk, (const u32x4*)sig_soa, (const uint8_t*)code_sig, dmsg, p.msg_len, nwit, np, inputs, dstatus);
     if (p.xrules && !want_zbool) return fail(ctx, BLSGPU_ERR_ARG, "the level-synchronous replay works on the packed 0/1 view");
```

After: 906,100 (median of 6 runs). +4.8%, better.
